# COx2/docker-nvidia-glx-desktop

Measured on AMD Instinct MI355X. Metric: encoded FPS + p50 end-to-end latency at 1080p60 H.264; concurrent sessions/node, higher is better.
Workload: dtype uint8 video (8-bit 4:2:0), H.264 Constrained Baseline

## Files before the change

### csrc/bindings/module.cpp

```cpp
#include <pybind11/numpy.h>
#include <pybind11/pybind11.h>
#include <pybind11/stl.h>

#include <cstring>

#include "../codec/h264_core.h"
#include "../codec/h264_encoder.h"
#include "../codec/vp8_encoder.h"
#include "../codec/hevc_encoder.h"
#include "../common/hip_check.h"
#include "../common/trace.h"
#include "../kernels/pixel.h"
#include "../runtime/session.h"

namespace py = pybind11;
using namespace mx;

void register_net(py::module& m);
void register_audio(py::module& m);
void register_rfb(py::module& m);

namespace {

template <class T>
T* as_ptr(uintptr_t p) {
    return reinterpret_cast<T*>(p);
}
hipStream_t as_stream(uintptr_t s) { return reinterpret_cast<hipStream_t>(s); }

py::bytes to_bytes(const std::vector<uint8_t>& v) {
    return py::bytes(reinterpret_cast<const char*>(v.data()), v.size());
}

struct PyBits {
    std::vector<uint32_t> words;
    h264::BitWriter w;
    PyBits() : words(4096) { w.init(words.data()); }
    py::tuple finish() {
        const uint32_t bits = w.bits;
        w.flush();
        std::vector<uint8_t> out;
        for (uint32_t i = 0; i < (bits + 7) / 8; ++i) out.push_back((uint8_t)(words[i / 4] >> (24 - 8 * (i % 4))));
        return py::make_tuple(to_bytes(out), bits);
    }
};

py::tuple cavlc_block_py(const std::vector<int>& coef, int nc) {
    PyBits b;
    int16_t c[16] = {0};
    const int n = (int)coef.size();
    if (n != 4 && n != 15 && n != 16) throw std::invalid_argument("block must have 4, 15 or 16 coefficients");
    for (int i = 0; i < n; ++i) c[i] = (int16_t)coef[i];
    h264::cavlc_block(b.w, c, n, nc);
    return b.finish();
}

py::array_t<int> fdct_py(py::array_t<int, py::array::c_style | py::array::forcecast> x) {
    if (x.size() != 16) throw std::invalid_argument("need 16 values");
    py::array_t<int> y(16);
    h264::fdct4x4(x.data(), y.mutable_data());
    return y;
}
py::array_t<int> idct_py(py::array_t<int, py::array::c_style | py::array::forcecast> x) {
    if (x.size() != 16) throw std::invalid_argument("need 16 values");
    py::array_t<int> y(16);
    h264::idct4x4(x.data(), y.mutable_data());
    return y;
}

py::array_t<uint8_t> copy_plane(const uint8_t* dev, int pitch, int w, int h) {
    py::array_t<uint8_t> out({h, w});
    HIP_CHECK(hipDeviceSynchronize());
    HIP_CHECK(hipMemcpy2D(out.mutable_data(), w, dev, pitch, w, h, hipMemcpyDeviceToHost));
    return out;
}

}

PYBIND11_MODULE(_native, m) {
    m.doc() = "mxdesk native runtime: HIP kernels (gfx950), H.264 encoder, session pipeline";

    m.def("device_count", []() {
        int n = 0;
        if (hipGetDeviceCount(&n) != hipSuccess) return 0;
        return n;
    });
    m.def("set_device", [](int d) { HIP_CHECK(hipSetDevice(d)); });
    m.def("device_name", [](int d) {
        hipDeviceProp_t p;
        HIP_CHECK(hipGetDeviceProperties(&p, d));
        return std::string(p.gcnArchName) + " / " + p.name;
    });
    m.def("synchronize", []() { HIP_CHECK(hipDeviceSynchronize()); });
    register_net(m);
    register_audio(m);
    register_rfb(m);
    m.def("now_us", &Session::now_us, "CLOCK_MONOTONIC microseconds (same clock as time.monotonic())");

    py::module h = m.def_submodule("h264", "H.264 building blocks (for tests)");
    h.def("hpel_planes", [](py::array_t<uint8_t, py::array::c_style> ref, int coded_w) {
        if (ref.ndim() != 2 || coded_w % 16 || ref.shape(0) % 16 || ref.shape(1) < coded_w)
            throw std::invalid_argument("ref must be (coded_h, pitch) with 16-aligned coded size");
        int hp = 0;
        auto planes = h264::hpel_planes_for_test(ref.data(), coded_w, (int)ref.shape(0), (int)ref.shape(1), &hp);
        const int rows = (int)ref.shape(0) + 2 * h264::kHpelPad;
        py::list out;
        for (auto& p : planes) {
            py::array_t<uint8_t> a({rows, hp});
            std::memcpy(a.mutable_data(), p.data(), p.size());
            out.append(a);
        }
        return out;
    });
    h.def("mc_luma_gpu", [](py::array_t<uint8_t, py::array::c_style> ref, int coded_w, int x4, int y4) {
        if (ref.ndim() != 2 || coded_w % 16 || ref.shape(0) % 16 || ref.shape(1) < coded_w)
            throw std::invalid_argument("ref must be (coded_h, pitch) with 16-aligned coded size");
        py::array_t<uint8_t> out({16, 16});
        h264::mc_luma_for_test(ref.data(), coded_w, (int)ref.shape(0), (int)ref.shape(1), x4, y4, out.mutable_data());
        return out;
    }, py::arg("ref"), py::arg("coded_w"), py::arg("x4"), py::arg("y4"),
          "16x16 luma prediction at quarter-sample position (x4, y4) by k_inter_encode's interpolation");
    h.def("cavlc_block", &cavlc_block_py, py::arg("coef"), py::arg("nc"));
    h.def("fdct4x4", &fdct_py);
    h.def("idct4x4", &idct_py);
    h.def("ue", [](uint32_t k) {
        PyBits b;
        h264::put_ue(b.w, k);
        return b.finish();
    });
    h.def("se", [](int v) {
        PyBits b;
        h264::put_se(b.w, v);
        return b.finish();
    });
    h.def("luma_qpel", [](py::array_t<uint8_t, py::array::c_style> plane, int x4, int y4) {
        if (plane.ndim() != 2) throw std::invalid_argument("2-D plane");
        const int H = (int)plane.shape(0), W = (int)plane.shape(1);
        return h264::luma_qpel(plane.data(), W, W, H, x4, y4);
    });
    h.def("level_for", &h264::pick_level);

    py::class_<h264::EncoderConfig>(m, "EncoderConfig")
        .def(py::init<>())
        .def_readwrite("width", &h264::EncoderConfig::width)
        .def_readwrite("height", &h264::EncoderConfig::height)
        .def_readwrite("fps", &h264::EncoderConfig::fps)
        .def_readwrite("bitrate_kbps", &h264::EncoderConfig::bitrate_kbps)
        .def_readwrite("qp", &h264::EncoderConfig::qp)
        .def_readwrite("qp_min", &h264::EncoderConfig::qp_min)
        .def_readwrite("qp_max", &h264::EncoderConfig::qp_max)
        .def_readwrite("keyint", &h264::EncoderConfig::keyint)
        .def_readwrite("search_range", &h264::EncoderConfig::search_range)
        .def_readwrite("me_coarse", &h264::EncoderConfig::me_coarse)
        .def_readwrite("intra4x4", &h264::EncoderConfig::intra4x4)
        .def_readwrite("subpel", &h264::EncoderConfig::subpel)
        .def_readwrite("chroma_qp_offset", &h264::EncoderConfig::chroma_qp_offset)
        .def_readwrite("pipeline_depth", &h264::EncoderConfig::pipeline_depth)
        .def_readwrite("aq", &h264::EncoderConfig::aq)
        .def_readwrite("intra_in_p", &h264::EncoderConfig::intra_in_p)
        .def_readwrite("vp8_bpred", &h264::EncoderConfig::vp8_bpred)
        .def_readwrite("vp8_intra", &h264::EncoderConfig::vp8_intra)
        .def_readwrite("mask_x0", &h264::EncoderConfig::mask_x0)
        .def_readwrite("mask_y0", &h264::EncoderConfig::mask_y0)
        .def_readwrite("mask_x1", &h264::EncoderConfig::mask_x1)
        .def_readwrite("mask_y1", &h264::EncoderConfig::mask_y1)
        .def_readwrite("deblock", &h264::EncoderConfig::deblock)
        .def_readwrite("partitions", &h264::EncoderConfig::partitions)
        .def_readwrite("tu_split", &h264::EncoderConfig::tu_split)
        .def_readwrite("hevc_slice_cost", &h264::EncoderConfig::hevc_slice_cost)
        .def_readwrite("hevc_wpp", &h264::EncoderConfig::hevc_wpp)
        .def_readwrite("hevc_wpp_rows", &h264::EncoderConfig::hevc_wpp_rows)
        .def_readwrite("sao", &h264::EncoderConfig::sao)
        .def_readwrite("hevc_chroma_keep", &h264::EncoderConfig::hevc_chroma_keep)
        .def_readwrite("hevc_intra_split", &h264::EncoderConfig::hevc_intra_split);

    py::class_<h264::FrameStats>(m, "FrameStats")
        .def_readonly("frame_index", &h264::FrameStats::frame_index)
        .def_readonly("idr", &h264::FrameStats::idr)
        .def_readonly("qp", &h264::FrameStats::qp)
        .def_readonly("bytes", &h264::FrameStats::bytes)
        .def_readonly("skipped_mbs", &h264::FrameStats::skipped_mbs)
        .def_readonly("encode_ms", &h264::FrameStats::encode_ms)
        .def_property_readonly("sse", [](const h264::FrameStats& s) { return py::make_tuple(s.sse[0], s.sse[1], s.sse[2]); })
        .def_readonly("sse_masked", &h264::FrameStats::sse_masked)
        .def_readonly("masked_pixels", &h264::FrameStats::masked_pixels)
        .def_readonly("deblocked", &h264::FrameStats::deblocked)
        .def_readonly("db_coherent", &h264::FrameStats::db_coherent)
        .def_readonly("db_changed", &h264::FrameStats::db_changed)
        .def_readonly("db_moving", &h264::FrameStats::db_moving);

    py::class_<h264::CpuH264Encoder>(m, "CpuH264Encoder")
        .def(py::init<const h264::EncoderConfig&>())
        .def(
            "encode",
            [](h264::CpuH264Encoder& e, py::array_t<uint8_t, py::array::c_style> y,
               py::array_t<uint8_t, py::array::c_style> uv, bool force_idr) {
                if (y.ndim() != 2 || uv.ndim() != 2 || y.shape(1) != uv.shape(1))
                    throw std::invalid_argument("y (H,P) and uv (H/2,P) planes with equal pitch");
                const int pitch = (int)y.shape(1);
                const int cw = e.coded_pitch();
                const auto& cfg = e.common().config();
                const int ch = e.common().mb_h() * 16;
                if (y.shape(0) < cfg.height || pitch < cfg.width || uv.shape(0) < cfg.height / 2)
                    throw std::invalid_argument("planes smaller than the encoder's configured picture");
                std::vector<uint8_t> py_, puv;
                const uint8_t* yy = y.data();
                const uint8_t* uu = uv.data();
                int p = pitch;
                if (y.shape(0) < ch || pitch < cw) {
                    h264::pad_nv12(yy, uu, cfg.width, cfg.height, pitch, cw, ch, py_, puv);
                    yy = py_.data();
                    uu = puv.data();
                    p = cw;
                }
                const auto& au = e.encode(yy, uu, p, force_idr);
                return to_bytes(au);
            },
            py::arg("y"), py::arg("uv"), py::arg("force_idr") = false)
        .def("recon",
             [](h264::CpuH264Encoder& e) {
                 const int cw = e.coded_pitch(), ch = e.common().mb_h() * 16;
                 py::array_t<uint8_t> y({ch, cw}), uv({ch / 2, cw});
                 std::memcpy(y.mutable_data(), e.recon_y().data(), (size_t)cw * ch);
                 std::memcpy(uv.mutable_data(), e.recon_uv().data(), (size_t)cw * ch / 2);
                 return py::make_tuple(y, uv);
             })
        .def("mb_bits",
             [](h264::CpuH264Encoder& e) {
                 const auto& v = e.mb_bits();
                 py::array_t<uint32_t> a((py::ssize_t)v.size());
                 std::memcpy(a.mutable_data(), v.data(), v.size() * 4);
                 return a.reshape({e.common().mb_h(), e.common().mb_w()});
             })
        .def("mb_info",
             [](h264::CpuH264Encoder& e) {
                 const auto& v = e.mb_info();
                 py::array_t<int32_t> a({(py::ssize_t)v.size(), (py::ssize_t)9});
                 int32_t* d = a.mutable_data();
                 for (size_t i = 0; i < v.size(); ++i) {
                     int nz = 0;
                     for (int k = 0; k < 16; ++k) nz += v[i].nz_luma[k];
                     const int32_t r[9] = {v[i].type, v[i].qp, v[i].cbp, v[i].skip, v[i].mvx, v[i].mvy, nz,
                                           (int32_t)v[i].cost, v[i].part};
                     std::memcpy(d + 9 * i, r, sizeof r);
                 }
                 return a.reshape({e.common().mb_h(), e.common().mb_w(), 9});
             })
        .def("request_idr", [](h264::CpuH264Encoder& e) { e.common().request_idr(); })
        .def("set_bitrate", [](h264::CpuH264Encoder& e, int k) { e.common().set_bitrate(k); })
        .def_property_readonly("stats", &h264::CpuH264Encoder::last_stats);

    py::class_<vp8::CpuVp8Encoder>(m, "CpuVp8Encoder")
        .def(py::init<const h264::EncoderConfig&>())
        .def(
            "encode",
            [](vp8::CpuVp8Encoder& e, py::array_t<uint8_t, py::array::c_style> y,
               py::array_t<uint8_t, py::array::c_style> uv, bool force_idr) {
                if (y.ndim() != 2 || uv.ndim() != 2 || y.shape(1) != uv.shape(1))
                    throw std::invalid_argument("y (H,P) and uv (H/2,P) planes with equal pitch");
                const int pitch = (int)y.shape(1);
                const int cw = e.coded_pitch();
                const auto& cfg = e.common().config();
                const int ch = e.common().mb_h() * 16;
                if (y.shape(0) < cfg.height || pitch < cfg.width || uv.shape(0) < cfg.height / 2)
                    throw std::invalid_argument("planes smaller than the encoder's configured picture");
                std::vector<uint8_t> py_, puv;
                const uint8_t* yy = y.data();
                const uint8_t* uu = uv.data();
                int p = pitch;
                if (y.shape(0) < ch || pitch < cw) {
                    h264::pad_nv12(yy, uu, cfg.width, cfg.height, pitch, cw, ch, py_, puv);
                    yy = py_.data();
                    uu = puv.data();
                    p = cw;
                }
                const auto& au = e.encode(yy, uu, p, force_idr);
                return to_bytes(au);
            },
            py::arg("y"), py::arg("uv"), py::arg("force_idr") = false)
        .def("recon",
             [](vp8::CpuVp8Encoder& e) {
                 const int cw = e.coded_pitch(), ch = e.common().mb_h() * 16;
                 py::array_t<uint8_t> y({ch, cw}), uv({ch / 2, cw});
                 std::memcpy(y.mutable_data(), e.recon_y().data(), (size_t)cw * ch);
                 std::memcpy(uv.mutable_data(), e.recon_uv().data(), (size_t)cw * ch / 2);
                 return py::make_tuple(y, uv);
             })
        .def("mb_info",
             [](vp8::CpuVp8Encoder& e) {
                 const auto& v = e.mb_info();
                 py::array_t<int32_t> a({(py::ssize_t)v.size(), (py::ssize_t)4});
                 int32_t* d = a.mutable_data();
                 for (size_t i = 0; i < v.size(); ++i) {
// ... 509 lines not shown
```

### csrc/codec/h264_encoder.cpp

```cpp
#include "h264_encoder.h"

#include <hip/hip_ext.h>

#include <algorithm>
#include <cmath>
#include <cstring>
#include <stdexcept>
#include <string>

#include "../common/hip_check.h"
#include "h264_mb.h"

namespace mx {
namespace h264 {

EncoderCommon::EncoderCommon(const EncoderConfig& c) : cfg_(c) {
    if (c.width <= 0 || c.height <= 0 || (c.width & 1) || (c.height & 1))
        throw std::invalid_argument("encoder size must be positive and even");
    mb_w_ = (c.width + 15) / 16;
    mb_h_ = (c.height + 15) / 16;
    cur_qp_ = std::clamp(c.qp, 0, 51);
}

double EncoderCommon::frame_budget_bits() const {
// ... 131 lines not shown
    words_to_bytes(words, w.bits + (w.bits % 8 ? 8 - w.bits % 8 : 0), rbsp);
    static const uint8_t sc[4] = {0, 0, 0, 1};
    out.insert(out.end(), sc, sc + 4);
    out.push_back(0x67);
    emulation_prevent(out, rbsp.data(), rbsp.size());
    w.init(words);
    write_pps(w, pic_init_qp(), cfg_.chroma_qp_offset);
    rbsp.clear();
    words_to_bytes(words, w.bits + (w.bits % 8 ? 8 - w.bits % 8 : 0), rbsp);
    out.insert(out.end(), sc, sc + 4);
    out.push_back(0x68);
    emulation_prevent(out, rbsp.data(), rbsp.size());
}

void EncoderCommon::write_slice_nal(std::vector<uint8_t>& out, const uint8_t* rbsp, size_t n, bool idr) const {
    static const uint8_t sc[4] = {0, 0, 0, 1};
    out.insert(out.end(), sc, sc + 4);
    out.push_back(idr ? 0x65 : 0x41);
    emulation_prevent(out, rbsp, n);
}

std::vector<std::vector<uint8_t>> hpel_planes_for_test(const uint8_t* ref, int coded_w, int coded_h, int pitch,
                                                       int* hp_pitch_out) {
    Geometry g{};
    g.width = coded_w;
    g.height = coded_h;
    g.mb_w = coded_w / 16;
    g.mb_h = coded_h / 16;
    g.coded_w = coded_w;
    g.coded_h = coded_h;
    g.pitch = pitch;
    const int hp_pitch = (coded_w + 2 * kHpelPad + 255) & ~255;
    const size_t hp_bytes = (size_t)hp_pitch * (coded_h + 2 * kHpelPad);
    uint8_t* dref = nullptr;
    uint8_t* planes[4];
    FrameState fs{};
    DeviceBuffers b{};
    HIP_CHECK(hipMalloc(&dref, (size_t)pitch * coded_h));
    HIP_CHECK(hipMemcpy(dref, ref, (size_t)pitch * coded_h, hipMemcpyHostToDevice));
    for (auto& p : planes) {
        HIP_CHECK(hipMalloc(&p, hp_bytes));
        HIP_CHECK(hipMemset(p, 0, hp_bytes));
    }
    fs.ref_y = dref;
    HIP_CHECK(hipMalloc(&b.fs, sizeof(FrameState)));
    HIP_CHECK(hipMemcpy(b.fs, &fs, sizeof(FrameState), hipMemcpyHostToDevice));
    launch_hpel(g, b, planes, hp_pitch, nullptr);
    HIP_CHECK(hipGetLastError());
    HIP_CHECK(hipDeviceSynchronize());
    std::vector<std::vector<uint8_t>> out(4, std::vector<uint8_t>(hp_bytes));
    for (int i = 0; i < 4; ++i) {
        HIP_CHECK(hipMemcpy(out[i].data(), planes[i], hp_bytes, hipMemcpyDeviceToHost));
        (void)hipFree(planes[i]);
    }
    (void)hipFree(dref);
    (void)hipFree(b.fs);
    *hp_pitch_out = hp_pitch;
    return out;
}

void mc_luma_for_test(const uint8_t* ref, int coded_w, int coded_h, int pitch, int x4, int y4, uint8_t* out) {
    Geometry g{};
    g.width = g.coded_w = coded_w;
    g.height = g.coded_h = coded_h;
    g.mb_w = coded_w / 16;
    g.mb_h = coded_h / 16;
    g.pitch = pitch;
    uint8_t *dref = nullptr, *dout = nullptr;
    HIP_CHECK(hipMalloc(&dref, (size_t)pitch * coded_h));
    HIP_CHECK(hipMalloc(&dout, 256));
    HIP_CHECK(hipMemcpy(dref, ref, (size_t)pitch * coded_h, hipMemcpyHostToDevice));
    launch_mc_luma_test(g, dref, x4, y4, dout, nullptr);
    const hipError_t e = hipGetLastError();
    if (e == hipSuccess) (void)hipMemcpy(out, dout, 256, hipMemcpyDeviceToHost);
    (void)hipFree(dref);
    (void)hipFree(dout);
    HIP_CHECK(e);
}

constexpr unsigned kDeviceEvent = hipEventDisableTiming | hipEventReleaseToDevice;

void GpuH264Encoder::alloc_slot(FrameSlot& sl) {
    const int nmb = geom_.mb_w * geom_.mb_h;
    DeviceBuffers& b = sl.buf;
    HIP_CHECK(hipMalloc(&b.fs, sizeof(FrameState)));
    HIP_CHECK(hipMalloc(&b.mb, sizeof(MbInfo) * nmb));
    HIP_CHECK(hipMemsetAsync(b.mb, 0, sizeof(MbInfo) * nmb, stream_));
    HIP_CHECK(hipMalloc(&b.coef, sizeof(int16_t) * kCoefStride * nmb));
    HIP_CHECK(hipMalloc(&b.slot, sizeof(uint32_t) * kSlotWords * (size_t)nmb));
    HIP_CHECK(hipMalloc(&b.slot_bits, sizeof(uint32_t) * nmb));
    HIP_CHECK(hipMalloc(&b.row_agg, sizeof(uint4) * (size_t)geom_.mb_h));
    HIP_CHECK(hipMalloc(&b.row_sse, sizeof(unsigned long long) * 4 * 512));
    HIP_CHECK(hipMalloc(&b.coded_info, sizeof(uint4) * nmb));
    HIP_CHECK(hipMalloc(&b.slice_info, sizeof(uint32_t) * kSliceInfo * kMaxSlices));
    HIP_CHECK(hipMemsetAsync(b.slice_info, 0, sizeof(uint32_t) * kSliceInfo * kMaxSlices, stream_));
    b.out_bytes = (size_t)nmb * 768;
    HIP_CHECK(hipMalloc(&b.quad_unit, sizeof(uint32_t) * (b.out_bytes / 16 + 1)));
    HIP_CHECK(hipMalloc(&b.out_hdr, sizeof(OutHeader)));
    HIP_CHECK(hipMalloc(&b.sse_part, 4 * sizeof(unsigned long long) * kSsePartStride));
    HIP_CHECK(hipMalloc(&b.wave_prog, sizeof(int) * 4));
    HIP_CHECK(hipMalloc(&b.mb_sse, sizeof(uint32_t) * 3 * (size_t)nmb));
    HIP_CHECK(hipMalloc(&b.intra_gain, sizeof(int32_t) * (size_t)nmb));
    HIP_CHECK(hipMalloc(&b.intra_cand, sizeof(int) * (size_t)nmb));
    HIP_CHECK(hipMalloc(&b.db_rec, sizeof(uint4) * (size_t)nmb));
    HIP_CHECK(hipMalloc(&b.db_rowq, sizeof(int) * (size_t)geom_.mb_h));
    HIP_CHECK(hipMalloc(&b.db_glb, sizeof(uint64_t) * 2 * 24 * (size_t)nmb));
    HIP_CHECK(hipMemsetAsync(b.db_glb, 0, sizeof(uint64_t) * 2 * 24 * (size_t)nmb, stream_));
    HIP_CHECK(hipMalloc(&b.pack_done, sizeof(uint32_t)));
    HIP_CHECK(hipMemsetAsync(b.pack_done, 0, sizeof(uint32_t), stream_));
    HIP_CHECK(hipMalloc(&b.db_cnt, sizeof(uint32_t) * 4));
    HIP_CHECK(hipMemsetAsync(b.db_cnt, 0, sizeof(uint32_t) * 4, stream_));
    HIP_CHECK(hipHostMalloc(&b.db_err, sizeof(int), hipHostMallocMapped));
    *b.db_err = 0;
    HIP_CHECK(hipHostMalloc(&sl.fs_host, sizeof(FrameState), hipHostMallocDefault));
    HIP_CHECK(hipHostMalloc(&sl.host_out, kOutPayloadOffset + b.out_bytes + 16, hipHostMallocMapped));
    std::memset(sl.host_out, 0, kOutPayloadOffset);
    HIP_CHECK(hipEventCreateWithFlags(&sl.start, hipEventDisableTiming));
    HIP_CHECK(hipEventCreateWithFlags(&sl.analysis_done, kDeviceEvent));
    HIP_CHECK(hipEventCreateWithFlags(&sl.deblock_done, kDeviceEvent));
    HIP_CHECK(hipEventCreateWithFlags(&sl.me_done, kDeviceEvent));
    HIP_CHECK(hipEventCreateWithFlags(&sl.done, hipEventDisableTiming));
}

void GpuH264Encoder::free_slot(FrameSlot& sl) {
    DeviceBuffers& b = sl.buf;
    for (void* p : {(void*)b.fs, (void*)b.mb, (void*)b.coef, (void*)b.slot, (void*)b.slot_bits, (void*)b.row_agg,
                    (void*)b.row_sse, (void*)b.coded_info, (void*)b.slice_info,
                    (void*)b.out_hdr, (void*)b.sse_part, (void*)b.wave_prog, (void*)b.mb_sse, (void*)b.intra_gain, (void*)b.intra_cand, (void*)b.quad_unit,
                    (void*)b.db_rec, (void*)b.db_rowq, (void*)b.db_glb, (void*)b.pack_done, (void*)b.db_cnt})
        if (p) (void)hipFree(p);
    if (b.db_err) (void)hipHostFree(b.db_err);
    if (sl.fs_host) (void)hipHostFree(sl.fs_host);
    if (sl.host_out) (void)hipHostFree(sl.host_out);
    for (hipEvent_t e : {sl.start, sl.analysis_done, sl.deblock_done, sl.done, sl.me_done})
        if (e) (void)hipEventDestroy(e);
}

GpuH264Encoder::GpuH264Encoder(const EncoderConfig& cfg, hipStream_t stream)
    : cfg_(cfg.with_aq_default(4)), common_(cfg), stream_(stream) {
    if (cfg.pipeline_depth < 1 || cfg.pipeline_depth > kMaxInFlight)
        throw std::invalid_argument("pipeline_depth must be 1 to 4");
    depth_ = cfg.pipeline_depth;
    db_lag_.reset(cfg_.h264_deblock_mode());
    geom_.width = cfg.width;
    geom_.height = cfg.height;
    geom_.mb_w = common_.mb_w();
    geom_.mb_h = common_.mb_h();
    geom_.coded_w = geom_.mb_w * 16;
    geom_.coded_h = geom_.mb_h * 16;
    geom_.pitch = (geom_.coded_w + 255) & ~255;
    if (geom_.mb_h > kMaxSlices) throw std::invalid_argument("picture too tall");
    if (geom_.mb_w > 512) throw std::invalid_argument("picture too wide (k_intra_wave stages <= 512 MBs per row)");
    const int nmb = geom_.mb_w * geom_.mb_h;
    if ((nmb + 3) / 4 + geom_.mb_h > kSsePartStride)
        throw std::invalid_argument("frame too large for the distortion partials");
    const size_t ysz = (size_t)geom_.pitch * geom_.coded_h, uvsz = ysz / 2;
    for (int i = 0; i < 2; ++i) {
        HIP_CHECK(hipMalloc(&rec_y_[i], ysz));
        HIP_CHECK(hipMalloc(&rec_uv_[i], uvsz));
        HIP_CHECK(hipMemsetAsync(rec_y_[i], 16, ysz, stream_));
        HIP_CHECK(hipMemsetAsync(rec_uv_[i], 128, uvsz, stream_));
        HIP_CHECK(hipMalloc(&src_keep_[i], ysz));
        HIP_CHECK(hipMemsetAsync(src_keep_[i], 16, ysz, stream_));
    }
    if (cfg.mask_x1 > cfg.mask_x0 && cfg.mask_y1 > cfg.mask_y0) {
        mask_mb_[0] = std::max(0, cfg.mask_x0) / 16;
        mask_mb_[1] = std::max(0, cfg.mask_y0) / 16;
        mask_mb_[2] = std::min(geom_.mb_w, (cfg.mask_x1 + 15) / 16);
        mask_mb_[3] = std::min(geom_.mb_h, (cfg.mask_y1 + 15) / 16);
    }
    masked_pixels_ = (int64_t)cfg.width * cfg.height;
    for (int my = mask_mb_[1]; my < mask_mb_[3]; ++my)
        for (int mx = mask_mb_[0]; mx < mask_mb_[2]; ++mx)
            masked_pixels_ -= (int64_t)std::max(0, std::min(16, cfg.width - 16 * mx)) *
                              std::max(0, std::min(16, cfg.height - 16 * my));
    if (cfg_.h264_deblock()) HIP_CHECK(hipMalloc(&rec_unf_, ysz));
    for (int i = 0; i < depth_; ++i) alloc_slot(slots_[i]);
    clock_khz_ = device_clock_khz();
    if (depth_ > 1) {
        HIP_CHECK(hipStreamCreateWithFlags(&stream_e_, hipStreamNonBlocking));
        if (cfg_.h264_deblock()) {
            HIP_CHECK(hipEventCreateWithFlags(&ev_hpu_, kDeviceEvent));
            HIP_CHECK(hipEventRecord(ev_hpu_, stream_));
        }
    }
    HIP_CHECK(hipStreamSynchronize(stream_));
    const char* et = std::getenv("MXDESK_ENTROPY_THREAD");
    if (stream_e_ && !(et && et[0] == '0')) {
        HIP_CHECK(hipGetDevice(&device_));
        launcher_ = std::thread([this]() { launcher_loop(); });
    }
}

void GpuH264Encoder::ensure_me_stream() {
    if (stream_m_) return;
    e2_retired_ = true;
    if (stream_e2_) {
        drain_launcher();
        HIP_CHECK(hipStreamSynchronize(stream_e2_));
        HIP_CHECK(hipStreamDestroy(stream_e2_));
        stream_e2_ = nullptr;
    }
    const char* rv = std::getenv("MXDESK_ME_CU_RESERVE");
    const int reserve = rv ? std::atoi(rv) : 0;
    int ncu = 0;
    HIP_CHECK(hipDeviceGetAttribute(&ncu, hipDeviceAttributeMultiprocessorCount, 0));
    if (reserve > 0 && reserve < ncu) {
        std::vector<uint32_t> mask((size_t)(ncu + 31) / 32, 0u);
        for (int c = 0; c < ncu - reserve; ++c) mask[(size_t)c / 32] |= 1u << (c % 32);
        HIP_CHECK(hipExtStreamCreateWithCUMask(&stream_m_, (uint32_t)mask.size(), mask.data()));
    } else {
        HIP_CHECK(hipStreamCreateWithFlags(&stream_m_, hipStreamNonBlocking));
    }
}

void GpuH264Encoder::launcher_loop() {
    (void)hipSetDevice(device_);
    for (;;) {
        EntropyJob j;
        {
            std::unique_lock<std::mutex> lk(lmu_);
            lcv_.wait(lk, [&] { return lstop_ || !ljobs_.empty(); });
            if (ljobs_.empty()) return;
            j = ljobs_.front();
            ljobs_.pop_front();
        }
        try {
            FrameSlot& sl = slots_[j.slot];
            HIP_CHECK(hipStreamWaitEvent(j.stream, sl.analysis_done, 0));
            launch_entropy(geom_, sl.buf, sl.host_out, j.stream, j.sse_ready);
            HIP_CHECK(hipGetLastError());
            HIP_CHECK(hipEventRecord(sl.done, j.stream));
        } catch (...) {
            std::lock_guard<std::mutex> lk(lmu_);
            lerr_ = std::current_exception();
        }
        {
            std::lock_guard<std::mutex> lk(lmu_);
            ++l_done_;
        }
        lcv_.notify_all();
    }
}

void GpuH264Encoder::drain_launcher() const {
    if (!launcher_.joinable()) return;
    std::unique_lock<std::mutex> lk(lmu_);
    lcv_.wait(lk, [&] { return l_done_ >= l_pushed_ || lerr_; });
    if (lerr_) std::rethrow_exception(lerr_);
}

void GpuH264Encoder::wait_launched(int slot) const {
    std::unique_lock<std::mutex> lk(lmu_);
    lcv_.wait(lk, [&] { return l_done_ >= slot_job_[slot] || lerr_; });
    if (lerr_) std::rethrow_exception(lerr_);
}

GpuH264Encoder::~GpuH264Encoder() {
    if (launcher_.joinable()) {
        {
            std::lock_guard<std::mutex> lk(lmu_);
            lstop_ = true;
        }
        lcv_.notify_all();
        launcher_.join();
    }
    (void)hipStreamSynchronize(stream_);
    if (stream_e_) {
        (void)hipStreamSynchronize(stream_e_);
        (void)hipStreamDestroy(stream_e_);
    }
    if (stream_e2_) {
        (void)hipStreamSynchronize(stream_e2_);
        (void)hipStreamDestroy(stream_e2_);
    }
    if (stream_m_) {
        (void)hipStreamSynchronize(stream_m_);
        (void)hipStreamDestroy(stream_m_);
    }
    if (ev_hpu_) (void)hipEventDestroy(ev_hpu_);
    if (rec_unf_) (void)hipFree(rec_unf_);
    for (int i = 0; i < 2; ++i) {
        (void)hipFree(rec_y_[i]);
        (void)hipFree(rec_uv_[i]);
        (void)hipFree(src_keep_[i]);
    }
    for (int i = 0; i < depth_; ++i) free_slot(slots_[i]);
}

void GpuH264Encoder::enqueue_analysis_kernels(bool idr, const uint8_t* src_y, const uint8_t* src_uv, bool publish) {
    FrameSlot& sl = slots_[prep_slot_];
    const FrameState* pub = publish ? sl.fs_host : nullptr;
    auto wait_input = [&]() {
        if (!in_ev_) return;
        HIP_CHECK(hipStreamWaitEvent(stream_, in_ev_, 0));
        in_ev_ = nullptr;
    };
    if (idr) {
        wait_input();
        launch_intra(geom_, sl.buf, src_y, src_uv, stream_, pub);
        if (cfg_.aq >= 3)
            launch_save_src(geom_, sl.buf, src_y, stream_);
    } else {
        if (depth_ > 1 && pub && sl.me_unf) ensure_me_stream();
        const bool side_me = stream_m_ && pub && sl.me_unf;
        if (side_me) {
            HIP_CHECK(hipStreamWaitEvent(stream_m_, ev_hpu_, 0));
            if (in_ev_) {
                HIP_CHECK(hipStreamWaitEvent(stream_m_, in_ev_, 0));
                in_ev_ = nullptr;
            }
            launch_me(geom_, sl.buf, src_y, stream_m_, pub, true);
            HIP_CHECK(hipEventRecord(sl.me_done, stream_m_));
            HIP_CHECK(hipStreamWaitEvent(stream_, sl.me_done, 0));
        } else {
            wait_input();
            launch_me(geom_, sl.buf, src_y, stream_, pub);
        }
        launch_inter(geom_, sl.buf, src_y, src_uv, stream_);
        if (cfg_.intra_in_p) launch_intra_in_p(geom_, sl.buf, src_y, src_uv, stream_);
    }
}

void GpuH264Encoder::link_entropy() {
    if (!stream_e_) return;
    drain_launcher();
    FrameSlot& sl = slots_[prep_slot_];
    HIP_CHECK(hipEventRecord(sl.analysis_done, stream_));
    HIP_CHECK(hipStreamWaitEvent(stream_e_, sl.analysis_done, 0));
}

void GpuH264Encoder::enqueue_entropy() {
    drain_launcher();
    FrameSlot& sl = slots_[prep_slot_];
    launch_entropy(geom_, sl.buf, sl.host_out, stream_e_ ? stream_e_ : stream_, nullptr);
}

void GpuH264Encoder::unfiltered_copy(FrameSlot& sl) {
    launch_copy_luma(geom_, sl.fs_host->rec_y, rec_unf_, stream_);
    if (ev_hpu_) HIP_CHECK(hipEventRecord(ev_hpu_, stream_));
}

void GpuH264Encoder::enqueue_kernels(bool idr, const uint8_t* src_y, const uint8_t* src_uv, bool publish) {
    FrameSlot& sl = slots_[prep_slot_];
    enqueue_analysis_kernels(idr, src_y, src_uv, publish);
    async_frame_ = launcher_.joinable() && publish && !sync_launch_;
    if (async_frame_) {
        HIP_CHECK(hipEventRecord(sl.analysis_done, stream_));
        hipEvent_t sse_ready = nullptr;
        if (sl.deblock) {
            unfiltered_copy(sl);
            launch_deblock(geom_, sl.buf, src_y, src_uv, stream_);
            HIP_CHECK(hipEventRecord(sl.deblock_done, stream_));
            sse_ready = sl.deblock_done;
        }
        if (depth_ >= 3 && !stream_e2_ && !e2_retired_ && !stream_m_)
            HIP_CHECK(hipStreamCreateWithFlags(&stream_e2_, hipStreamNonBlocking));
        hipStream_t es = (stream_e2_ && (seq_ & 1)) ? stream_e2_ : stream_e_;
        HIP_CHECK(hipGetLastError());
        {
            std::lock_guard<std::mutex> lk(lmu_);
            if (lerr_) std::rethrow_exception(lerr_);
            ljobs_.push_back(EntropyJob{prep_slot_, sse_ready, es});
            slot_job_[prep_slot_] = ++l_pushed_;
        }
        lcv_.notify_all();
        return;
    }
    link_entropy();
    hipStream_t es = stream_e_ ? stream_e_ : stream_;
    hipEvent_t sse_ready = nullptr;
    if (sl.deblock) {
        unfiltered_copy(sl);
        launch_deblock(geom_, sl.buf, src_y, src_uv, stream_);
        if (stream_e_) {
            HIP_CHECK(hipEventRecord(sl.deblock_done, stream_));
            sse_ready = sl.deblock_done;
        }
    }
    launch_entropy(geom_, sl.buf, sl.host_out, es, sse_ready);
    HIP_CHECK(hipGetLastError());
}

void GpuH264Encoder::fill_state(FrameSlot& sl, bool idr, int qp, int ref, int cur) {
    FrameState& f = *sl.fs_host;
    f.ref_y = rec_y_[ref];
    f.ref_uv = rec_uv_[ref];
    f.rec_y = rec_y_[cur];
    f.rec_uv = rec_uv_[cur];
    f.idr = idr ? 1 : 0;
    f.frame_num = common_.cur_frame_num();
    f.idr_pic_id = common_.cur_idr_pic_id();
    f.qp = qp;
    f.slice_rows = idr ? idr_slice_rows(geom_.mb_h) : geom_.mb_h;
    f.num_slices = (geom_.mb_h + f.slice_rows - 1) / f.slice_rows;
    f.search_range = me_range(cfg_.search_range);
    f.me_coarse = cfg_.me_coarse;
    f.intra4x4 = cfg_.intra4x4;
    f.subpel = cfg_.subpel;
    f.deblock_off = sl.deblock ? 0 : 1;
    if (++db_epoch_ == 0) db_epoch_ = 1;
    f.db_epoch = (int32_t)db_epoch_;
    f.pic_init_qp = common_.pic_init_qp();
    f.chroma_qp_offset = cfg_.chroma_qp_offset;
    f.log2_max_frame_num = common_.log2_max_frame_num();
    f.aq = cfg_.aq;
    f.intra_in_p = cfg_.intra_in_p;
    f.partitions = cfg_.partitions ? 1 : 0;
    f.mask_mx0 = mask_mb_[0];
    f.mask_my0 = mask_mb_[1];
    f.mask_mx1 = mask_mb_[2];
    f.mask_my1 = mask_mb_[3];
    f.me_ref = sl.me_unf ? rec_unf_ : nullptr;
    f.sse_part = sl.buf.sse_part;
    f.prev_src = src_keep_[ref];
    f.save_src = src_keep_[cur];
}

int GpuH264Encoder::probe_bytes(const uint8_t* src_y, const uint8_t* src_uv, int qp) {
    if (!inflight_.empty()) throw std::logic_error("GpuH264Encoder: probe with frames in flight");
    prep_slot_ = 0;
    FrameSlot& sl = slots_[0];
    sl.deblock = cfg_.deblock == 1;
    sl.me_unf = false;
    fill_state(sl, true, qp, cur_ ^ 1, cur_);
    sl.fs_host->frame_num = 0;
    sl.fs_host->idr_pic_id = 0;
    sync_launch_ = true;
    enqueue_kernels(true, src_y, src_uv, true);
    sync_launch_ = false;
    HIP_CHECK(hipStreamSynchronize(stream_));
    if (stream_e_) HIP_CHECK(hipStreamSynchronize(stream_e_));
    const OutHeader hdr = *reinterpret_cast<const OutHeader*>(sl.host_out);
    return hdr.overflow ? (int)sl.buf.out_bytes : (int)(hdr.total_bytes + hdr.num_slices * 6 + 32);
}

bool GpuH264Encoder::prepare(bool force_idr) {
    if ((int)inflight_.size() >= depth_)
        throw std::logic_error("GpuH264Encoder: collect() a frame first (pipeline full)");
    const int s = (depth_ == 1) ? 0 : next_slot_;
    next_slot_ = (next_slot_ + 1) % depth_;
    prep_slot_ = s;
    ++seq_;
    FrameSlot& sl = slots_[s];
    common_.begin_frame(force_idr || !have_ref_);
    have_ref_ = true;
    const bool idr = common_.cur_idr();
    sl.idr = idr;
    sl.qp = common_.cur_qp();
    const int ref = cur_;
    cur_ ^= 1;
    sl.fidx = seq_;
    sl.me_unf = !idr && last_deblock_;
    sl.deblock = db_lag_.decide((long long)seq_, idr);
    last_deblock_ = sl.deblock;
    fill_state(sl, idr, sl.qp, ref, cur_);
    return idr;
}

void GpuH264Encoder::enqueue_body(bool idr, const uint8_t* src_y, const uint8_t* src_uv) {
    drain_launcher();
    FrameSlot& sl = slots_[prep_slot_];
    HIP_CHECK(hipMemcpyAsync(sl.buf.fs, sl.fs_host, sizeof(FrameState), hipMemcpyHostToDevice, stream_));
    enqueue_kernels(idr, src_y, src_uv, false);
}

void GpuH264Encoder::enqueue_analysis(bool idr, const uint8_t* src_y, const uint8_t* src_uv) {
    drain_launcher();
    FrameSlot& sl = slots_[prep_slot_];
    HIP_CHECK(hipMemcpyAsync(sl.buf.fs, sl.fs_host, sizeof(FrameState), hipMemcpyHostToDevice, stream_));
    enqueue_analysis_kernels(idr, src_y, src_uv, false);
}
// ... 75 lines not shown
```

### csrc/codec/h264_gpu.h

```cpp
#pragma once
#include <vector>
#include <hip/hip_runtime.h>
#include <stdint.h>

#define MXHD_GPU __host__ __device__ __forceinline__

namespace mx {
namespace h264 {

constexpr int kSlotWords = 640;
constexpr int kCoefStride = 416;
constexpr int kCoefLuma = 0;
constexpr int kCoefLumaDc = 256;
constexpr int kCoefChromaDc = 272;
constexpr int kCoefChromaAc = 280;

enum MbType : uint8_t { kMbP16x16 = 0, kMbI16x16 = 1, kMbI4x4 = 2 };

struct MbInfo {
    int16_t mvx, mvy;
    uint8_t type;
    uint8_t cbp;
    uint8_t i16_mode;
    uint8_t chroma_mode;
    uint8_t nz_luma[16];
    uint8_t nz_cb[4];
    uint8_t nz_cr[4];
    uint8_t skip;
    uint8_t qp;
    uint8_t cbp_c;
    uint8_t itype;
    uint8_t i4[8];
    uint32_t cost;
    int16_t pmv[4];
    uint8_t part;
    uint8_t pad_[7];
};
static_assert(sizeof(MbInfo) == 64, "MbInfo layout");
enum MbPart : uint8_t { kPart16x16 = 0, kPart16x8 = 1, kPart8x16 = 2 };

MXHD_GPU bool is_intra(const MbInfo& m) { return m.type != kMbP16x16; }
template <class FS>
MXHD_GPU bool mb_unmasked(const FS* fs, int mbx, int mby) {
    return !(mbx >= fs->mask_mx0 && mbx < fs->mask_mx1 && mby >= fs->mask_my0 && mby < fs->mask_my1);
}
MXHD_GPU bool carries_dqp(const MbInfo& m) { return m.type == kMbI16x16 || m.cbp != 0; }

struct FrameState {
    const uint8_t* ref_y;
    const uint8_t* ref_uv;
    uint8_t* rec_y;
    uint8_t* rec_uv;
    int32_t idr;
    int32_t frame_num;
    int32_t idr_pic_id;
    int32_t qp;
    int32_t slice_rows;
    int32_t num_slices;
    int32_t search_range;
    int32_t subpel;
    int32_t me_coarse;
    int32_t intra4x4;
    int32_t deblock_off;
    int32_t db_epoch;
    int32_t pic_init_qp;
    int32_t chroma_qp_offset;
    int32_t log2_max_frame_num;
    int32_t aq;
    int32_t intra_in_p;
    int32_t partitions;
    int32_t mask_mx0, mask_my0, mask_mx1, mask_my1;
    const uint8_t* prev_src;
    uint8_t* save_src;
    const uint8_t* me_ref;
    unsigned long long* sse_part;
};
constexpr int kHpelPad = 48;
constexpr int kSsePartStride = 65536;

struct OutHeader {
    uint32_t total_bytes;
    uint32_t num_slices;
    uint32_t overflow;
    uint32_t deblocked;
    uint64_t sse[3];
    uint64_t sse_masked;
    uint64_t t_start;
    uint64_t t_end;
    uint32_t db_coherent, db_changed, db_moving;
    uint32_t pad;
};
static_assert(sizeof(OutHeader) % 16 == 0, "payload must stay 16-byte aligned");
constexpr int kMaxSlices = 1024;
constexpr int kSliceInfo = 8;
constexpr size_t kOutPayloadOffset = sizeof(OutHeader) + 2 * kMaxSlices * sizeof(uint32_t);

struct Geometry {
    int width, height;
    int mb_w, mb_h;
    int pitch;
    int coded_w, coded_h;
};

struct DeviceBuffers {
    FrameState* fs;
    MbInfo* mb;
    int16_t* coef;
    uint32_t* slot;
    uint32_t* slot_bits;
    uint4* row_agg;
    unsigned long long* row_sse;
    uint4* coded_info;
    uint32_t* quad_unit;
    uint32_t* slice_info;
    size_t out_bytes;
    OutHeader* out_hdr;
    unsigned long long* sse_part;
    int* wave_prog;
    int32_t* intra_gain;
    int* intra_cand;
    uint32_t* mb_sse;
    uint4* db_rec;
    int* db_rowq;
    uint64_t* db_glb;
    int* db_err;
    uint32_t* db_cnt;
    uint32_t* pack_done;
};

void launch_me(const Geometry& g, const DeviceBuffers& b, const uint8_t* src_y, hipStream_t stream,
               const FrameState* publish = nullptr, bool side = false);
void launch_copy_luma(const Geometry& g, const uint8_t* luma, uint8_t* dst, hipStream_t stream);
void launch_mc_luma_test(const Geometry& g, const uint8_t* ref, int x4, int y4, uint8_t* out, hipStream_t stream);
void launch_inter(const Geometry& g, const DeviceBuffers& b, const uint8_t* src_y, const uint8_t* src_uv,
                  hipStream_t stream);
void launch_intra(const Geometry& g, const DeviceBuffers& b, const uint8_t* src_y, const uint8_t* src_uv,
                  hipStream_t stream, const FrameState* publish = nullptr);
void launch_hpel(const Geometry& g, const DeviceBuffers& b, uint8_t* const planes[4], int hp_pitch,
                 hipStream_t stream, const FrameState* publish = nullptr);
std::vector<unsigned long long> deblock_row_stamps(int mb_h);
void launch_deblock(const Geometry& g, const DeviceBuffers& b, const uint8_t* src_y, const uint8_t* src_uv,
                    hipStream_t stream);
void launch_save_src(const Geometry& g, const DeviceBuffers& b, const uint8_t* src_y, hipStream_t stream);
void launch_entropy(const Geometry& g, const DeviceBuffers& b, uint8_t* host_out, hipStream_t stream,
                    hipEvent_t wait_for_sse = nullptr);
void launch_intra_in_p(const Geometry& g, const DeviceBuffers& b, const uint8_t* src_y, const uint8_t* src_uv,
                       hipStream_t stream);

}
}
```

### csrc/codec/h264_kernels.hip

```cpp
#include <hip/hip_runtime.h>

#include <cstddef>

#include "../common/hip_check.h"
#include "h264_core.h"
#include "h264_deblock.h"
#include "h264_gpu.h"
#include "h264_mb.h"

namespace mx {
namespace h264 {

namespace {

__device__ __forceinline__ uint32_t bswap32(uint32_t v) { return __builtin_bswap32(v); }

template <bool kSwap>
struct OrWriter {
    uint32_t* dst;
    uint32_t pos;
    uint64_t acc;
    int nacc;
    uint32_t bits;

// ... 25 lines not shown
            nacc -= 32;
        }
    }
    __device__ __forceinline__ void flush() {
        if (nacc > 0) {
            emit((uint32_t)(acc << (32 - nacc)), nacc);
            nacc = 0;
            acc = 0;
        }
    }
};

__device__ __forceinline__ uint32_t rows_sum(uint32_t v) {
    const auto r16 = __builtin_amdgcn_permlane16_swap(v, v, false, false);
    v = r16[0] + r16[1];
    const auto r32 = __builtin_amdgcn_permlane32_swap(v, v, false, false);
    return r32[0] + r32[1];
}
__device__ __forceinline__ int wave_sum(int v) {
    v += __builtin_amdgcn_mov_dpp(v, 0xB1, 0xF, 0xF, false);
    v += __builtin_amdgcn_mov_dpp(v, 0x4E, 0xF, 0xF, false);
    v += __builtin_amdgcn_mov_dpp(v, 0x124, 0xF, 0xF, false);
    v += __builtin_amdgcn_mov_dpp(v, 0x128, 0xF, 0xF, false);
    return (int)rows_sum((uint32_t)v);
}

constexpr int kHpTW = 128, kHpTH = 16;
constexpr int kHpSW = kHpTW + 8;
__device__ __forceinline__ int byte_of(uint32_t w, int k) { return (int)((w >> (8 * k)) & 0xff); }
__device__ __forceinline__ uint32_t pack4(int a, int b, int c, int d) {
    const uint32_t lo = __builtin_amdgcn_perm((uint32_t)b, (uint32_t)a, 0x0c0c0400u);
    const uint32_t hi = __builtin_amdgcn_perm((uint32_t)d, (uint32_t)c, 0x0c0c0400u);
    return __builtin_amdgcn_perm(hi, lo, 0x05040100u);
}
struct StateArg {
    FrameState v;
    FrameState* dst;
    int publish;
    uint64_t* t_start;
};
__device__ __forceinline__ void publish_state(const StateArg& a) {
    static_assert(sizeof(FrameState) % 4 == 0, "FrameState is copied as dwords");
    if (a.t_start && blockIdx.x == 0 && blockIdx.y == 0 && threadIdx.x == 0) *a.t_start = wall_clock64();
    if (a.publish && blockIdx.x == 0 && blockIdx.y == 0 && threadIdx.x < sizeof(FrameState) / 4)
        reinterpret_cast<uint32_t*>(a.dst)[threadIdx.x] = reinterpret_cast<const uint32_t*>(&a.v)[threadIdx.x];
}
__device__ __forceinline__ const FrameState& state_of(const StateArg& a) { return a.publish ? a.v : *a.dst; }

__global__ __launch_bounds__(256) void k_hpel(Geometry g, StateArg sa, uint8_t* __restrict__ pf,
                                              uint8_t* __restrict__ ph, uint8_t* __restrict__ pv,
                                              uint8_t* __restrict__ pj, int hp_pitch) {
    __shared__ uint32_t smp[kHpTH + 5][kHpSW / 4];
    __shared__ int4 b1[kHpTH + 5][kHpTW / 4];
    publish_state(sa);
    const uint8_t* __restrict__ ref = state_of(sa).ref_y;
    const int px0 = blockIdx.x * kHpTW, py0 = blockIdx.y * kHpTH;
    const int W = g.coded_w + 2 * kHpelPad, H = g.coded_h + 2 * kHpelPad;
    const int tid = threadIdx.x;
    const int xs = px0 - 4 - kHpelPad, ys = py0 - 2 - kHpelPad;
    const bool interior = xs >= 0 && xs + kHpSW <= g.coded_w && ys >= 0 && ys + kHpTH + 5 <= g.coded_h &&
                          (g.pitch & 3) == 0 && (reinterpret_cast<uintptr_t>(ref) & 3) == 0;
    for (int i = tid; i < (kHpTH + 5) * (kHpSW / 4); i += 256) {
        const int r = i / (kHpSW / 4), k4 = i - r * (kHpSW / 4);
        uint32_t w;
        if (interior) {
            w = *reinterpret_cast<const uint32_t*>(ref + (size_t)(ys + r) * g.pitch + xs + 4 * k4);
        } else {
            w = 0;
            for (int k = 0; k < 4; ++k)
                w |= (uint32_t)ref_px(ref, g.pitch, g.coded_w, g.coded_h, xs + 4 * k4 + k, ys + r) << (8 * k);
        }
        smp[r][k4] = w;
    }
    __syncthreads();
    for (int i = tid; i < (kHpTH + 5) * (kHpTW / 4); i += 256) {
        const int r = i / (kHpTW / 4), q = i - r * (kHpTW / 4);
        const uint32_t w0 = smp[r][q], w1 = smp[r][q + 1], w2 = smp[r][q + 2];
        int s[12];
#pragma unroll
        for (int k = 0; k < 4; ++k) {
            s[k] = byte_of(w0, k);
            s[4 + k] = byte_of(w1, k);
            s[8 + k] = byte_of(w2, k);
        }
        int t[4];
#pragma unroll
        for (int j = 0; j < 4; ++j) t[j] = tap6(s[j + 2], s[j + 3], s[j + 4], s[j + 5], s[j + 6], s[j + 7]);
        b1[r][q] = make_int4(t[0], t[1], t[2], t[3]);
    }
    __syncthreads();
    const int q = tid & (kHpTW / 4 - 1), r0 = (tid / (kHpTW / 4)) * 2;
    const int x = px0 + 4 * q;
    if (x >= W) return;
    int sv[7][4], bv[7][4];
#pragma unroll
    for (int k = 0; k < 7; ++k) {
        const uint32_t w = smp[r0 + k][q + 1];
        const int4 bb = b1[r0 + k][q];
#pragma unroll
        for (int j = 0; j < 4; ++j) sv[k][j] = byte_of(w, j);
        bv[k][0] = bb.x;
        bv[k][1] = bb.y;
        bv[k][2] = bb.z;
        bv[k][3] = bb.w;
    }
#pragma unroll
    for (int rr = 0; rr < 2; ++rr) {
        const int y = py0 + r0 + rr;
        if (y >= H) break;
        int Hs[4], Vs[4], Js[4];
#pragma unroll
        for (int j = 0; j < 4; ++j) {
            Hs[j] = clip255((bv[rr + 2][j] + 16) >> 5);
            const int v1 = tap6(sv[rr][j], sv[rr + 1][j], sv[rr + 2][j], sv[rr + 3][j], sv[rr + 4][j], sv[rr + 5][j]);
            Vs[j] = clip255((v1 + 16) >> 5);
            const int j1 = tap6(bv[rr][j], bv[rr + 1][j], bv[rr + 2][j], bv[rr + 3][j], bv[rr + 4][j], bv[rr + 5][j]);
            Js[j] = clip255((j1 + 512) >> 10);
        }
        const size_t o = (size_t)y * hp_pitch + x;
        *reinterpret_cast<uint32_t*>(pf + o) = smp[r0 + rr + 2][q + 1];
        *reinterpret_cast<uint32_t*>(ph + o) = pack4(Hs[0], Hs[1], Hs[2], Hs[3]);
        *reinterpret_cast<uint32_t*>(pv + o) = pack4(Vs[0], Vs[1], Vs[2], Vs[3]);
        *reinterpret_cast<uint32_t*>(pj + o) = pack4(Js[0], Js[1], Js[2], Js[3]);
    }
}

constexpr int kSpW = 20;
__device__ __forceinline__ int qpel_lds(const uint8_t (*sp)[18][kSpW], int x4, int y4) {
    const int xi = x4 >> 2, yi = y4 >> 2, xf = x4 & 3, yf = y4 & 3;
    const int G = sp[0][yi][xi];
    if ((xf | yf) == 0) return G;
    if (yf == 0) {
        const int b = sp[1][yi][xi];
        if (xf == 2) return b;
        return ((xf == 1 ? G : (int)sp[0][yi][xi + 1]) + b + 1) >> 1;
    }
    if (xf == 0) {
        const int hh = sp[2][yi][xi];
        if (yf == 2) return hh;
        return ((yf == 1 ? G : (int)sp[0][yi + 1][xi]) + hh + 1) >> 1;
    }
    if (xf == 2 && yf == 2) return sp[3][yi][xi];
    if (xf == 2) return ((yf == 1 ? (int)sp[1][yi][xi] : (int)sp[1][yi + 1][xi]) + sp[3][yi][xi] + 1) >> 1;
    if (yf == 2) return ((xf == 1 ? (int)sp[2][yi][xi] : (int)sp[2][yi][xi + 1]) + sp[3][yi][xi] + 1) >> 1;
    const int bb = (yf == 1) ? sp[1][yi][xi] : sp[1][yi + 1][xi];
    const int hh = (xf == 1) ? sp[2][yi][xi] : sp[2][yi][xi + 1];
    return (bb + hh + 1) >> 1;
}

constexpr int kMaxRange = 32;
constexpr int kWinPadX = 4, kWinPadY = 3;
constexpr int kWinStride = 16 + 2 * kMaxRange + 8;
constexpr int kWinRows = 16 + 2 * kMaxRange + 7;

constexpr int kMeThreads = 256, kMeWaves = kMeThreads / 64;
constexpr int kFpRows = 18 + 5;
__device__ __forceinline__ void build_footprints(const uint8_t* win, int org0, int org1, int n,
                                                 uint8_t (*sp)[4][18][kSpW], int16_t (*b1)[kFpRows][kSpW], int tid) {
    for (int i = tid; i < n * kFpRows * 18; i += kMeThreads) {
        const int pi = i / (kFpRows * 18), rem = i - pi * (kFpRows * 18), r = rem / 18, c = rem - r * 18;
        const uint8_t* p = win + (pi ? org1 : org0) + (r - 2) * kWinStride + c;
        b1[pi][r][c] = (int16_t)tap6(p[-2], p[-1], p[0], p[1], p[2], p[3]);
    }
    __syncthreads();
    for (int i = tid; i < n * 324; i += kMeThreads) {
        const int pi = i / 324, rem = i - pi * 324, r = rem / 18, c = rem - r * 18;
        const uint8_t* p = win + (pi ? org1 : org0) + r * kWinStride + c;
        const int16_t(*b)[kSpW] = b1[pi];
        const int v1 = tap6(p[-2 * kWinStride], p[-kWinStride], p[0], p[kWinStride], p[2 * kWinStride], p[3 * kWinStride]);
        const int j1 = tap6(b[r][c], b[r + 1][c], b[r + 2][c], b[r + 3][c], b[r + 4][c], b[r + 5][c]);
        sp[pi][0][r][c] = p[0];
        sp[pi][1][r][c] = (uint8_t)clip255((b[r + 2][c] + 16) >> 5);
        sp[pi][2][r][c] = (uint8_t)clip255((v1 + 16) >> 5);
        sp[pi][3][r][c] = (uint8_t)clip255((j1 + 512) >> 10);
    }
}

struct MeState {
    const uint8_t* ref;
    int qp, search_range, subpel, me_coarse, partitions;
};
__device__ __forceinline__ MeState me_state(const FrameState& f) {
    return MeState{f.me_ref ? f.me_ref : f.ref_y, f.qp, f.search_range, f.subpel, f.me_coarse, f.partitions};
}
__device__ __forceinline__ void me_full_body(const Geometry& g, const MeState& st, const uint8_t* __restrict__ src_y,
                                             MbInfo* __restrict__ mbs) {
    __shared__ uint32_t win_lds[kWinRows * kWinStride / 4];
    __shared__ uint8_t sp2[2][4][18][kSpW];
    __shared__ int16_t fp_b1[2][kFpRows][kSpW];
    __shared__ uint32_t srcw[64];
    __shared__ unsigned long long red[kMeWaves];
    __shared__ uint32_t cand_cost[8];
    __shared__ uint32_t s_sad0[4];

    const int mbi = blockIdx.x;
    const int mbx = mbi % g.mb_w, mby = mbi / g.mb_w;
    const int x0 = mbx * 16, y0 = mby * 16;
    const int tid = threadIdx.x, lane = tid & 63;
    const int R = me_range(st.search_range);
    const int W = 16 + 2 * R;
    const uint8_t* __restrict__ ref = st.ref;
    const int lambda = lambda_sad(st.qp);

    constexpr int kWs4 = kWinStride / 4;
    {
        if (tid < 64) {
            const int r = tid >> 2, c4 = (tid & 3) * 4;
            const uint32_t sw = *reinterpret_cast<const uint32_t*>(src_y + (y0 + r) * g.pitch + x0 + c4);
            const uint32_t rw = *reinterpret_cast<const uint32_t*>(ref + (y0 + r) * g.pitch + x0 + c4);
            const int d = wave_sum((int)__builtin_amdgcn_sad_u8(sw, rw, 0u));
            if (tid == 0) s_sad0[0] = (uint32_t)d;
        }
        __syncthreads();
        const uint32_t sad0 = s_sad0[0];
        if (sad0 <= static_sad(st.qp)) {
            if (tid == 0) {
                MbInfo& m = mbs[mbi];
                m.mvx = 0;
                m.mvy = 0;
                m.part = kPart16x16;
                m.pmv[0] = m.pmv[1] = m.pmv[2] = m.pmv[3] = 0;
            }
            return;
        }
    }
    const bool t256 = tid < 256;
    const int wrows = W + 2 * kWinPadY + 1, wx0 = x0 - R - kWinPadX, wy0 = y0 - R - kWinPadY;
    const bool dwords = (g.pitch & 3) == 0 && (reinterpret_cast<uintptr_t>(ref) & 3) == 0;
    for (int i = tid; i < wrows * kWs4; i += kMeThreads) {
        const int wy = i / kWs4, wx4 = (i - wy * kWs4) * 4;
        uint32_t w = 0u;
        if (wx4 < W + 2 * kWinPadX) {
            const int py = min(max(wy0 + wy, 0), g.coded_h - 1), px = wx0 + wx4;
            const uint8_t* row = ref + (size_t)py * g.pitch;
            if (px < 0)
                w = row[0] * 0x01010101u;
            else if (px >= g.coded_w)
                w = row[g.coded_w - 1] * 0x01010101u;
            else if (dwords)
                w = *reinterpret_cast<const uint32_t*>(row + px);
            else
                w = row[px] | ((uint32_t)row[px + 1] << 8) | ((uint32_t)row[px + 2] << 16) | ((uint32_t)row[px + 3] << 24);
        }
        win_lds[i] = w;
    }
    const uint32_t* win32 = win_lds + kWinPadY * kWs4 + kWinPadX / 4;
    auto fp_org = [&](int vx, int vy) {
        return ((vy >> 2) + R + kWinPadY - 1) * kWinStride + (vx >> 2) + R + kWinPadX - 1;
    };
    if (tid < 64) {
        const int r = tid >> 2, c = (tid & 3) * 4;
        srcw[tid] = *reinterpret_cast<const uint32_t*>(src_y + (y0 + r) * g.pitch + x0 + c);
    }
    __syncthreads();

    const int side = 2 * R + 1, gw = (side + 3) >> 2, ngroups = side * gw;
    unsigned long long best = ~0ull;
    const bool coarse = st.me_coarse != 0;
    const bool parts = st.partitions != 0;
    const int ntask = (coarse && !parts) ? (R + 1) * gw : 0;
    auto mkey = [&](uint32_t sad, int dxr, int dyr) {
        const int dx = dxr - R, dy = dyr - R;
        const uint32_t cost = me_cost(sad, lambda, 4 * dx, 4 * dy);
        const uint32_t dist = (uint32_t)(abs(dx) + abs(dy));
        return ((unsigned long long)cost << 32) | (dist << 16) | (uint32_t)(dyr * side + dxr);
    };
    unsigned long long pb[4] = {~0ull, ~0ull, ~0ull, ~0ull};
    auto kmin = [](unsigned long long a, unsigned long long c) { return c < a ? c : a; };
    auto visit_quads = [&](const uint32_t* qd, int dxr, int dyr) {
        best = kmin(best, mkey(qd[0] + qd[1] + qd[2] + qd[3], dxr, dyr));
        pb[0] = kmin(pb[0], mkey(qd[0] + qd[1], dxr, dyr));
        pb[1] = kmin(pb[1], mkey(qd[2] + qd[3], dxr, dyr));
        pb[2] = kmin(pb[2], mkey(qd[0] + qd[2], dxr, dyr));
        pb[3] = kmin(pb[3], mkey(qd[1] + qd[3], dxr, dyr));
    };
    if (parts) {
        const int nsh = coarse ? 2 : 4, ntp = coarse ? (R + 1) * gw : ngroups;
        for (int q = tid; q < ntp; q += kMeThreads) {
            const int dyr = coarse ? 2 * (q / gw) : q / gw, g = q % gw;
            uint32_t acc[4][4];
#pragma unroll
            for (int i = 0; i < 4; ++i) acc[i][0] = acc[i][1] = acc[i][2] = acc[i][3] = 0;
#pragma unroll 2
            for (int r = 0; r < 16; ++r) {
                const int a = (dyr + r) * kWs4 + g, hq = r < 8 ? 0 : 2;
                const uint32_t w0 = win32[a], w1 = win32[a + 1], w2 = win32[a + 2], w3 = win32[a + 3], w4 = win32[a + 4];
                const uint32_t s0 = srcw[r * 4 + 0], s1 = srcw[r * 4 + 1], s2 = srcw[r * 4 + 2], s3 = srcw[r * 4 + 3];
#pragma unroll
                for (int si = 0; si < 4; ++si) {
                    if (si >= nsh) break;
                    const int sh = coarse ? 2 * si : si;
                    const uint32_t a0 = sh ? __builtin_amdgcn_alignbyte(w1, w0, sh) : w0;
                    const uint32_t a1 = sh ? __builtin_amdgcn_alignbyte(w2, w1, sh) : w1;
                    const uint32_t a2 = sh ? __builtin_amdgcn_alignbyte(w3, w2, sh) : w2;
                    const uint32_t a3 = sh ? __builtin_amdgcn_alignbyte(w4, w3, sh) : w3;
                    uint32_t lft = hq ? acc[si][2] : acc[si][0], rgt = hq ? acc[si][3] : acc[si][1];
                    lft = __builtin_amdgcn_sad_u8(a1, s1, __builtin_amdgcn_sad_u8(a0, s0, lft));
                    rgt = __builtin_amdgcn_sad_u8(a3, s3, __builtin_amdgcn_sad_u8(a2, s2, rgt));
                    if (hq) {
                        acc[si][2] = lft;
                        acc[si][3] = rgt;
                    } else {
                        acc[si][0] = lft;
                        acc[si][1] = rgt;
                    }
                }
            }
#pragma unroll
            for (int si = 0; si < 4; ++si) {
                if (si >= nsh) break;
                const int dxr = 4 * g + (coarse ? 2 * si : si);
                if (dxr >= side) break;
                visit_quads(acc[si], dxr, dyr);
            }
        }
    }
    for (int q = tid; q < ntask; q += kMeThreads) {
        const int dyr = 2 * (q / gw), g = q % gw;
        uint32_t s0a = 0, s2a = 0;
#pragma unroll 4
        for (int r = 0; r < 16; ++r) {
            const int a = (dyr + r) * kWs4 + g;
            const uint32_t w0 = win32[a], w1 = win32[a + 1], w2 = win32[a + 2], w3 = win32[a + 3], w4 = win32[a + 4];
            const uint32_t s0 = srcw[r * 4 + 0], s1 = srcw[r * 4 + 1], s2 = srcw[r * 4 + 2], s3 = srcw[r * 4 + 3];
            s0a = __builtin_amdgcn_sad_u8(w0, s0, s0a);
            s0a = __builtin_amdgcn_sad_u8(w1, s1, s0a);
            s0a = __builtin_amdgcn_sad_u8(w2, s2, s0a);
            s0a = __builtin_amdgcn_sad_u8(w3, s3, s0a);
            s2a = __builtin_amdgcn_sad_u8(__builtin_amdgcn_alignbyte(w1, w0, 2), s0, s2a);
            s2a = __builtin_amdgcn_sad_u8(__builtin_amdgcn_alignbyte(w2, w1, 2), s1, s2a);
            s2a = __builtin_amdgcn_sad_u8(__builtin_amdgcn_alignbyte(w3, w2, 2), s2, s2a);
            s2a = __builtin_amdgcn_sad_u8(__builtin_amdgcn_alignbyte(w4, w3, 2), s3, s2a);
        }
#pragma unroll
        for (int h2 = 0; h2 < 2; ++h2) {
            const int dxr = 4 * g + 2 * h2;
            if (dxr >= side) break;
            const int dx = dxr - R, dy = dyr - R, c = dyr * side + dxr;
            const uint32_t cost = me_cost(h2 ? s2a : s0a, lambda, 4 * dx, 4 * dy);
            const uint32_t dist = (uint32_t)(abs(dx) + abs(dy));
            const unsigned long long key = ((unsigned long long)cost << 32) | (dist << 16) | (uint32_t)c;
            best = key < best ? key : best;
        }
    }
    for (int q = tid; q < ((coarse || parts) ? 0 : ngroups); q += kMeThreads) {
        const int dyr = q / gw, g = q - dyr * gw;
        uint32_t sad[4] = {0, 0, 0, 0};
#pragma unroll 2
        for (int r = 0; r < 16; ++r) {
            const int a = (dyr + r) * kWs4 + g;
            const uint32_t w0 = win32[a], w1 = win32[a + 1], w2 = win32[a + 2], w3 = win32[a + 3], w4 = win32[a + 4];
            const uint32_t s0 = srcw[r * 4 + 0], s1 = srcw[r * 4 + 1], s2 = srcw[r * 4 + 2], s3 = srcw[r * 4 + 3];
            sad[0] = __builtin_amdgcn_sad_u8(w0, s0, sad[0]);
            sad[0] = __builtin_amdgcn_sad_u8(w1, s1, sad[0]);
            sad[0] = __builtin_amdgcn_sad_u8(w2, s2, sad[0]);
            sad[0] = __builtin_amdgcn_sad_u8(w3, s3, sad[0]);
#pragma unroll
            for (int sh = 1; sh < 4; ++sh) {
                uint32_t t = sad[sh];
                t = __builtin_amdgcn_sad_u8(__builtin_amdgcn_alignbyte(w1, w0, sh), s0, t);
                t = __builtin_amdgcn_sad_u8(__builtin_amdgcn_alignbyte(w2, w1, sh), s1, t);
                t = __builtin_amdgcn_sad_u8(__builtin_amdgcn_alignbyte(w3, w2, sh), s2, t);
                t = __builtin_amdgcn_sad_u8(__builtin_amdgcn_alignbyte(w4, w3, sh), s3, t);
                sad[sh] = t;
            }
        }
#pragma unroll
        for (int sh = 0; sh < 4; ++sh) {
            const int dxr = 4 * g + sh;
            if (dxr >= side) break;
            const int dx = dxr - R, dy = dyr - R, c = dyr * side + dxr;
            const uint32_t cost = me_cost(sad[sh], lambda, 4 * dx, 4 * dy);
            const uint32_t dist = (uint32_t)(abs(dx) + abs(dy));
            const unsigned long long key = ((unsigned long long)cost << 32) | (dist << 16) | (uint32_t)c;
            best = key < best ? key : best;
        }
    }
    for (int o = 32; o > 0; o >>= 1) {
        unsigned long long other = __shfl_xor(best, o, 64);
        best = other < best ? other : best;
    }
    if (lane == 0) red[tid >> 6] = best;
    __shared__ unsigned long long pred4[4][kMeWaves];
    if (parts) {
#pragma unroll
        for (int sh = 0; sh < 4; ++sh) {
            unsigned long long v = pb[sh];
            for (int o = 32; o > 0; o >>= 1) {
                const unsigned long long other = __shfl_xor(v, o, 64);
                v = other < v ? other : v;
            }
            if (lane == 0) pred4[sh][tid >> 6] = v;
        }
    }
    __syncthreads();
    unsigned long long b = red[0];
    for (int i = 1; i < kMeWaves; ++i) b = red[i] < b ? red[i] : b;
    unsigned long long pbest[4] = {~0ull, ~0ull, ~0ull, ~0ull};
    if (parts)
        for (int sh = 0; sh < 4; ++sh)
            for (int i = 0; i < kMeWaves; ++i) pbest[sh] = pred4[sh][i] < pbest[sh] ? pred4[sh][i] : pbest[sh];
    if (parts && coarse) {
        __shared__ unsigned long long pnkey[4][8];
        const int ev = (tid & 255) >> 3, sub = tid & 7, sh = ev >> 3, k = ev & 7;
        const int cb0 = (int)(pbest[sh] & 0xffff), bxr = cb0 % side, byr = cb0 / side;
        int ddx, ddy;
        subpel_offset(k, &ddx, &ddy);
        const int nxr = bxr + ddx, nyr = byr + ddy;
        const bool inside = t256 && nxr >= 0 && nxr < side && nyr >= 0 && nyr < side;
        int d = 0;
        if (inside) {
            const uint8_t* wb = reinterpret_cast<const uint8_t*>(win32);
            const uint8_t* sb = reinterpret_cast<const uint8_t*>(srcw);
            for (int part_row = 0; part_row < 2; ++part_row) {
                const int rr = sh < 2 ? (sh == 0 ? sub : 8 + sub) : 2 * sub + part_row;
                const int c0 = sh < 2 ? 8 * part_row : (sh == 2 ? 0 : 8);
#pragma unroll
                for (int j = 0; j < 8; ++j)
                    d += abs((int)sb[rr * 16 + c0 + j] - (int)wb[(nyr + rr) * kWinStride + nxr + c0 + j]);
            }
        }
        for (int o = 4; o > 0; o >>= 1) d += __shfl_xor(d, o, 64);
        if (t256 && sub == 0) pnkey[sh][k] = inside ? mkey((uint32_t)d, nxr, nyr) : ~0ull;
        __syncthreads();
        for (int s2 = 0; s2 < 4; ++s2)
            for (int i = 0; i < 8; ++i) pbest[s2] = pnkey[s2][i] < pbest[s2] ? pnkey[s2][i] : pbest[s2];
    }
    if (coarse) {
        __shared__ unsigned long long nkey[8];
        const int cb0 = (int)(b & 0xffff), bxr = cb0 % side, byr = cb0 / side;
        const int k = (tid & 255) >> 5, sub = tid & 31, py = sub >> 1, px0 = (sub & 1) * 8;
        int ddx, ddy;
        subpel_offset(k, &ddx, &ddy);
        const int nxr = bxr + ddx, nyr = byr + ddy;
        const bool inside = t256 && nxr >= 0 && nxr < side && nyr >= 0 && nyr < side;
        int d = 0;
        if (inside) {
            const uint8_t* wrow = reinterpret_cast<const uint8_t*>(win32) + (nyr + py) * kWinStride + nxr + px0;
            const uint32_t s0 = srcw[py * 4 + (px0 >> 2)], s1 = srcw[py * 4 + (px0 >> 2) + 1];
#pragma unroll
            for (int j = 0; j < 8; ++j) d += abs((int)(((j < 4 ? s0 : s1) >> (8 * (j & 3))) & 0xff) - (int)wrow[j]);
        }
        for (int o = 16; o > 0; o >>= 1) d += __shfl_xor(d, o, 64);
        if (t256 && sub == 0) {
            const int dx = nxr - R, dy = nyr - R;
            const uint32_t cost = me_cost((uint32_t)d, lambda, 4 * dx, 4 * dy);
            const uint32_t dist = (uint32_t)(abs(dx) + abs(dy));
            nkey[k] = inside ? (((unsigned long long)cost << 32) | (dist << 16) | (uint32_t)(nyr * side + nxr)) : ~0ull;
        }
        __syncthreads();
        for (int i = 0; i < 8; ++i) b = nkey[i] < b ? nkey[i] : b;
    }
    const int cbest = (int)(b & 0xffff);
    int mvx = 4 * ((cbest % side) - R), mvy = 4 * ((cbest / side) - R);

    if (parts) {
        const uint32_t c16 = (uint32_t)(b >> 32);
        const uint32_t chz = (uint32_t)(pbest[0] >> 32) + (uint32_t)(pbest[1] >> 32) + 2u * (uint32_t)lambda;
        const uint32_t cvt = (uint32_t)(pbest[2] >> 32) + (uint32_t)(pbest[3] >> 32) + 2u * (uint32_t)lambda;
        const int part = (c16 <= chz && c16 <= cvt) ? kPart16x16 : (chz <= cvt ? kPart16x8 : kPart8x16);
        if (part != kPart16x16) {
            const int s0 = part == kPart16x8 ? 0 : 2;
            int pvx[2], pvy[2];
            uint32_t pcost[2];
            for (int i = 0; i < 2; ++i) {
                const int cb = (int)(pbest[s0 + i] & 0xffff);
                pvx[i] = 4 * ((cb % side) - R);
                pvy[i] = 4 * ((cb / side) - R);
                pcost[i] = (uint32_t)(pbest[s0 + i] >> 32);
            }
            if (st.subpel) {
                uint8_t(*psp)[4][18][kSpW] = sp2;
                __shared__ uint32_t pcand[2][8];
                build_footprints(reinterpret_cast<const uint8_t*>(win_lds), fp_org(pvx[0], pvy[0]),
                                 fp_org(pvx[1], pvy[1]), 2, sp2, fp_b1, tid);
                __syncthreads();
                const int pi = (tid & 255) >> 7, k = (tid >> 4) & 7, sub = tid & 15;
                const int rx = part == kPart8x16 ? 8 * pi : 0, ry = part == kPart16x8 ? 8 * pi : 0;
                const int prow = part == kPart16x8 ? (sub >> 1) : sub, pcol = part == kPart16x8 ? (sub & 1) * 8 : 0;
                const int yy = ry + prow, xx = rx + pcol;
                const uint32_t s0w = srcw[yy * 4 + (xx >> 2)], s1w = srcw[yy * 4 + (xx >> 2) + 1];
                const int ivx = pvx[pi], ivy = pvy[pi];
                const int base_x4 = xx * 4 + 4 - ivx, base_y4 = yy * 4 + 4 - ivy;
                for (int step = 2; step >= 1; step >>= 1) {
                    int ddx, ddy;
                    subpel_offset(k, &ddx, &ddy);
                    const int cx = pvx[pi] + ddx * step, cy = pvy[pi] + ddy * step;
                    int d = 0;
#pragma unroll
                    for (int j = 0; j < 8; ++j) {
                        const int sv = (int)(((j < 4 ? s0w : s1w) >> (8 * (j & 3))) & 0xff);
                        d += abs(sv - qpel_lds(psp[pi], base_x4 + 4 * j + cx, base_y4 + cy));
                    }
                    for (int o = 8; o > 0; o >>= 1) d += __shfl_xor(d, o, 64);
                    __syncthreads();
                    if (t256 && sub == 0) pcand[pi][k] = me_cost((uint32_t)d, lambda, cx, cy);
                    __syncthreads();
                    for (int q = 0; q < 2; ++q) {
                        int bdx = 0, bdy = 0;
                        uint32_t bcost = pcost[q];
                        for (int kk = 0; kk < 8; ++kk) {
                            const uint32_t cc = pcand[q][kk];
                            if (cc < bcost) {
                                int ex, ey;
                                subpel_offset(kk, &ex, &ey);
                                bcost = cc;
                                bdx = ex * step;
                                bdy = ey * step;
                            }
                        }
                        pvx[q] += bdx;
                        pvy[q] += bdy;
                        pcost[q] = bcost;
                    }
                }
            }
            if (tid == 0) {
                MbInfo& m = mbs[mbi];
                m.mvx = (int16_t)mvx;
                m.mvy = (int16_t)mvy;
                m.part = (uint8_t)part;
                m.pmv[0] = (int16_t)pvx[0];
                m.pmv[1] = (int16_t)pvy[0];
                m.pmv[2] = (int16_t)pvx[1];
                m.pmv[3] = (int16_t)pvy[1];
            }
            return;
        }
    }

    if (st.subpel) {
        uint8_t(*sp)[18][kSpW] = sp2[0];
        build_footprints(reinterpret_cast<const uint8_t*>(win_lds), fp_org(mvx, mvy), 0, 1, sp2, fp_b1, tid);
        __syncthreads();
        uint32_t cur_cost = (uint32_t)(b >> 32);
        const int k = (tid & 255) >> 5, sub = tid & 31;
        const int py = sub >> 1, px0 = (sub & 1) * 8;
        const uint32_t s0 = srcw[py * 4 + (px0 >> 2)], s1 = srcw[py * 4 + (px0 >> 2) + 1];
        const int base_x4 = px0 * 4 + 4 - mvx, base_y4 = py * 4 + 4 - mvy;
        for (int step = 2; step >= 1; step >>= 1) {
            int ddx, ddy;
            subpel_offset(k, &ddx, &ddy);
            const int cx = mvx + ddx * step, cy = mvy + ddy * step;
            int d = 0;
#pragma unroll
            for (int j = 0; j < 8; ++j) {
                const int sv = (int)(((j < 4 ? s0 : s1) >> (8 * (j & 3))) & 0xff);
                d += abs(sv - qpel_lds(sp, base_x4 + 4 * j + cx, base_y4 + cy));
            }
            for (int o = 16; o > 0; o >>= 1) d += __shfl_xor(d, o, 64);
            __syncthreads();
            if (t256 && sub == 0) cand_cost[k] = me_cost((uint32_t)d, lambda, cx, cy);
            __syncthreads();
            int bdx = 0, bdy = 0;
            uint32_t bcost = cur_cost;
            for (int kk = 0; kk < 8; ++kk) {
                const uint32_t cc = cand_cost[kk];
                if (cc < bcost) {
                    int ex, ey;
                    subpel_offset(kk, &ex, &ey);
                    bcost = cc;
                    bdx = ex * step;
                    bdy = ey * step;
                }
            }
            mvx += bdx;
            mvy += bdy;
            cur_cost = bcost;
        }
    }
    if (tid == 0) {
        MbInfo& m = mbs[mbi];
        m.mvx = (int16_t)mvx;
        m.mvy = (int16_t)mvy;
        m.part = kPart16x16;
        m.pmv[0] = m.pmv[1] = m.pmv[2] = m.pmv[3] = 0;
    }
}

__global__ __launch_bounds__(kMeThreads) void k_me_full(Geometry g, StateArg sa, const uint8_t* __restrict__ src_y,
                                                        MbInfo* __restrict__ mbs) {
    publish_state(sa);
    me_full_body(g, sa.publish ? me_state(sa.v) : me_state(*sa.dst), src_y, mbs);
}
__global__ __launch_bounds__(kMeThreads) void k_me_full_val(Geometry g, StateArg sa, const uint8_t* __restrict__ src_y,
                                                            MbInfo* __restrict__ mbs) {
    publish_state(sa);
    me_full_body(g, me_state(sa.v), src_y, mbs);
}

template <int K>
__device__ __forceinline__ int qbc(int v) {
    return __builtin_amdgcn_mov_dpp(v, K * 0x55, 0xF, 0xF, false);
}
__device__ __forceinline__ int quad_sum(int v) { return qbc<0>(v) + qbc<1>(v) + qbc<2>(v) + qbc<3>(v); }

__device__ __forceinline__ void fdct_row(const int* x, int r, int* y) {
    const int s03 = x[0] + x[3], d03 = x[0] - x[3], s12 = x[1] + x[2], d12 = x[1] - x[2];
    const int t[4] = {s03 + s12, 2 * d03 + d12, s03 - s12, d03 - 2 * d12};
#pragma unroll
    for (int c = 0; c < 4; ++c) {
        const int a0 = qbc<0>(t[c]), a1 = qbc<1>(t[c]), a2 = qbc<2>(t[c]), a3 = qbc<3>(t[c]);
        const int u03 = a0 + a3, e03 = a0 - a3, u12 = a1 + a2, e12 = a1 - a2;
        y[c] = r == 0 ? u03 + u12 : r == 1 ? 2 * e03 + e12 : r == 2 ? u03 - u12 : e03 - 2 * e12;
    }
}
__device__ __forceinline__ void idct_row(const int* d, int r, int* out) {
    const int e0 = d[0] + d[2], e1 = d[0] - d[2], e2 = (d[1] >> 1) - d[3], e3 = d[1] + (d[3] >> 1);
    const int f[4] = {e0 + e3, e1 + e2, e1 - e2, e0 - e3};
#pragma unroll
    for (int c = 0; c < 4; ++c) {
        const int b0 = qbc<0>(f[c]), b1 = qbc<1>(f[c]), b2 = qbc<2>(f[c]), b3 = qbc<3>(f[c]);
        const int g0 = b0 + b2, g1 = b0 - b2, g2 = (b1 >> 1) - b3, g3 = b1 + (b3 >> 1);
        const int v = r == 0 ? g0 + g3 : r == 1 ? g1 + g2 : r == 2 ? g1 - g2 : g0 - g3;
        out[c] = (v + 32) >> 6;
    }
}
__device__ __forceinline__ int had_row_abs(const int* x, int r) {
    const int t[4] = {x[0] + x[1] + x[2] + x[3], x[0] + x[1] - x[2] - x[3], x[0] - x[1] - x[2] + x[3],
                      x[0] - x[1] + x[2] - x[3]};
    int s = 0;
#pragma unroll
    for (int c = 0; c < 4; ++c) {
        const int a = qbc<0>(t[c]), b = qbc<1>(t[c]), cc = qbc<2>(t[c]), d = qbc<3>(t[c]);
        const int v = r == 0 ? a + b + cc + d : r == 1 ? a + b - cc - d : r == 2 ? a - b - cc + d : a - b + cc - d;
        s += v < 0 ? -v : v;
    }
    return s;
}
__device__ __forceinline__ int quant_row(const int* y, int r, int qp, bool intra, int start, int* z) {
    const int qm = qp % 6, qbits = 15 + qp / 6;
    const int f = intra ? ((1 << qbits) / 3) : ((1 << qbits) / 6);
    int nz = 0;
#pragma unroll
    for (int c = 0; c < 4; ++c) {
        const int i = r * 4 + c;
        if (i < start) {
            z[c] = 0;
            continue;
        }
        const int a = y[c] < 0 ? -y[c] : y[c];
        int q = (int)(((int64_t)a * kQuantMF[qm][kPosClass[i]] + f) >> qbits);
        q = q > kMaxLevel ? kMaxLevel : q;
        z[c] = y[c] < 0 ? -q : q;
        nz += (q != 0);
    }
    return nz;
}
__device__ __forceinline__ void dequant_row(const int* z, int r, int qp, int* d) {
    const int qm = qp % 6, qs = qp / 6;
#pragma unroll
    for (int c = 0; c < 4; ++c) d[c] = z[c] * kDequantV[qm][kPosClass[r * 4 + c]] * (1 << qs);
}

__device__ __forceinline__ void wave_sync_lds() {
    __builtin_amdgcn_fence(__ATOMIC_RELEASE, "wavefront");
    __builtin_amdgcn_wave_barrier();
    __builtin_amdgcn_fence(__ATOMIC_ACQUIRE, "wavefront");
}

constexpr int kMcStride = 24, kMcRows = 16 + 5, kMcWords = kMcRows * kMcStride / 4;
__device__ __forceinline__ void mc_luma_wave(uint32_t* __restrict__ w, const uint8_t* __restrict__ ref, int pitch,
                                             int cw, int ch, int n, int xa, int ya, int xb, int yb, int lane, int lpi,
                                             uint32_t* out) {
    const bool aligned = (pitch & 3) == 0 && (reinterpret_cast<uintptr_t>(ref) & 3) == 0;
    for (int i = lane; i < n * kMcWords; i += 64) {
        const int pi = i >= kMcWords ? 1 : 0, j = i - pi * kMcWords;
        const int wr = j / (kMcStride / 4), q = j - wr * (kMcStride / 4);
        const int xs = ((pi ? xb : xa) >> 2) - 2, ys = ((pi ? yb : ya) >> 2) - 2;
        uint32_t v;
        if (aligned && xs >= 0 && (xs & ~3) + kMcStride + 4 <= cw) {
            const int py = min(max(ys + wr, 0), ch - 1), px = xs + 4 * q;
            const uint32_t* qa = reinterpret_cast<const uint32_t*>(ref + (size_t)py * pitch + (px & ~3));
            const uint32_t sh = (uint32_t)(px & 3);
            v = sh ? __builtin_amdgcn_alignbyte(qa[1], qa[0], sh) : qa[0];
        } else {
            v = 0;
            for (int k = 0; k < 4; ++k) v |= (uint32_t)ref_px(ref, pitch, cw, ch, xs + 4 * q + k, ys + wr) << (8 * k);
        }
        w[i] = v;
    }
    wave_sync_lds();
    {
        const int xf = (lpi ? xb : xa) & 3, yf = (lpi ? yb : ya) & 3;
        w += lpi * kMcWords;
        const int r = lane >> 2, q0 = lane & 3;
        uint32_t wd[6][3];
#pragma unroll
        for (int rr = 0; rr < 6; ++rr) {
            const uint32_t* row = w + (r + rr) * (kMcStride / 4) + q0;
            wd[rr][0] = row[0];
            wd[rr][1] = row[1];
            wd[rr][2] = row[2];
        }
        auto s = [&](int rr, int c) { return byte_of(wd[rr][c >> 2], c & 3); };
        auto b1 = [&](int rr) { return tap6(s(rr, 0), s(rr, 1), s(rr, 2), s(rr, 3), s(rr, 4), s(rr, 5)); };
        auto v1 = [&](int c) { return tap6(s(0, c), s(1, c), s(2, c), s(3, c), s(4, c), s(5, c)); };
        auto b_at = [&](int rr) { return clip255((b1(rr) + 16) >> 5); };
        auto h_at = [&](int c) { return clip255((v1(c) + 16) >> 5); };
        auto j_val = [&]() { return clip255((tap6(b1(0), b1(1), b1(2), b1(3), b1(4), b1(5)) + 512) >> 10); };
        uint32_t packed = 0;
#pragma unroll 1
        for (int k = 0; k < 4; ++k) {
            const int G = s(2, 2);
            int p;
            if ((xf | yf) == 0)
                p = G;
            else if (yf == 0)
                p = xf == 2 ? b_at(2) : ((xf == 1 ? G : s(2, 3)) + b_at(2) + 1) >> 1;
            else if (xf == 0)
                p = yf == 2 ? h_at(2) : ((yf == 1 ? G : s(3, 2)) + h_at(2) + 1) >> 1;
            else if (xf == 2 && yf == 2)
                p = j_val();
            else if (xf == 2)
                p = ((yf == 1 ? b_at(2) : b_at(3)) + j_val() + 1) >> 1;
            else if (yf == 2)
                p = ((xf == 1 ? h_at(2) : h_at(3)) + j_val() + 1) >> 1;
            else
                p = ((yf == 1 ? b_at(2) : b_at(3)) + (xf == 1 ? h_at(2) : h_at(3)) + 1) >> 1;
            packed |= (uint32_t)p << (8 * k);
#pragma unroll
            for (int rr = 0; rr < 6; ++rr) {
                wd[rr][0] = __builtin_amdgcn_alignbyte(wd[rr][1], wd[rr][0], 1);
                wd[rr][1] = __builtin_amdgcn_alignbyte(wd[rr][2], wd[rr][1], 1);
                wd[rr][2] >>= 8;
            }
        }
        *out = packed;
    }
}

__global__ __launch_bounds__(64) void k_mc_luma_test(Geometry g, const uint8_t* __restrict__ ref, int x4, int y4,
                                                     uint8_t* __restrict__ out) {
    __shared__ uint32_t w[kMcWords];
    const int lane = threadIdx.x;
    uint32_t p = 0;
    mc_luma_wave(w, ref, g.pitch, g.coded_w, g.coded_h, 1, x4, y4, x4, y4, lane, 0, &p);
    reinterpret_cast<uint32_t*>(out)[lane] = p;
}

__global__ __launch_bounds__(256) void k_inter_encode(Geometry g, const FrameState* __restrict__ fs,
                                                       const uint8_t* __restrict__ src_y,
                                                       const uint8_t* __restrict__ src_uv, MbInfo* __restrict__ mbs,
                                                       int16_t* __restrict__ coef, uint32_t* __restrict__ mb_sse,
                                                       int* __restrict__ wave_prog) {
    __shared__ uint8_t pred[4][384];
    __shared__ int16_t res[4][384];
    __shared__ uint32_t mcw[4][2 * kMcWords];
    __shared__ int cdc[4][8];
    __shared__ int cdc_nz[4][2];

    const int wave = threadIdx.x >> 6, lane = threadIdx.x & 63;
    const int nmb = g.mb_w * g.mb_h;
    const int bid = blockIdx.x;
    const int mbi = bid * 4 + wave;
    if (bid == 0 && threadIdx.x == 0) wave_prog[1] = 0;
    const bool valid = mbi < nmb;
    const int mbx = valid ? mbi % g.mb_w : 0, mby = valid ? mbi / g.mb_w : 0;
    const int x0 = mbx * 16, y0 = mby * 16;
    const uint8_t* __restrict__ ref_y = fs->ref_y;
    const bool ref_dwords = (g.pitch & 3) == 0 && (reinterpret_cast<uintptr_t>(ref_y) & 3) == 0;
    const uint8_t* ref_uv = fs->ref_uv;
    const int cw = g.coded_w / 2, ch = g.coded_h / 2;
    int mvx = 0, mvy = 0;
    int lsad = 0;
    int tsad = 0;
    MbInfo mi;
    mi.part = kPart16x16;
    if (valid) {
        mi = mbs[mbi];
        const int r = lane >> 2, c0 = (lane & 3) * 4;
        const Mv lv = px_mv(mi, c0, r);
        mvx = lv.x;
        mvy = lv.y;
        const uint32_t sw = *reinterpret_cast<const uint32_t*>(src_y + (y0 + r) * g.pitch + x0 + c0);
        if (fs->aq >= 3) {
            const int ix = mvx >> 2, iy = mvy >> 2;
            const int px = x0 + c0 + ix, py = y0 + r + iy;
            if (px >= 0 && px + 4 <= g.coded_w && py >= 0 && py < g.coded_h &&
                ((px & 3) == 0 || (px & ~3) + 8 <= g.pitch)) {
                const uint32_t* qa = reinterpret_cast<const uint32_t*>(fs->prev_src + (size_t)py * g.pitch + (px & ~3));
                const uint32_t sh = (uint32_t)(px & 3);
                const uint32_t pw = sh ? __builtin_amdgcn_alignbyte(qa[1], qa[0], sh) : qa[0];
                tsad = (int)__builtin_amdgcn_sad_u8(sw, pw, 0u);
            } else {
                for (int k = 0; k < 4; ++k)
                    tsad += abs((int)((sw >> (8 * k)) & 0xff) -
                                ref_px(fs->prev_src, g.pitch, g.coded_w, g.coded_h, x0 + c0 + k + ix, y0 + r + iy));
            }
            *reinterpret_cast<uint32_t*>(fs->save_src + (y0 + r) * g.pitch + x0 + c0) = sw;
        }
        const int part = __builtin_amdgcn_readfirstlane((int)mi.part);
        const Mv va = blk_mv(mi, 0, 0), vb = blk_mv(mi, part == kPart8x16 ? 2 : 0, part == kPart16x8 ? 2 : 0);
        const int vax = __builtin_amdgcn_readfirstlane(va.x), vay = __builtin_amdgcn_readfirstlane(va.y);
        const int vbx = __builtin_amdgcn_readfirstlane(vb.x), vby = __builtin_amdgcn_readfirstlane(vb.y);
        uint32_t pw = 0;
        if ((vax | vay | vbx | vby) & 3) {
            const int lpi = part == kPart16x8 ? (r >> 3) : (part == kPart8x16 ? (c0 >> 3) : 0);
            mc_luma_wave(mcw[wave], ref_y, g.pitch, g.coded_w, g.coded_h, part == kPart16x16 ? 1 : 2, x0 * 4 + vax,
                         y0 * 4 + vay, x0 * 4 + vbx, y0 * 4 + vby, lane, lpi, &pw);
        } else {
            const int px = x0 + c0 + (mvx >> 2), py = min(max(y0 + r + (mvy >> 2), 0), g.coded_h - 1);
            if (px >= 0 && px + 4 <= g.coded_w && ((px & 3) == 0 || (px & ~3) + 8 <= g.pitch) && ref_dwords) {
                const uint32_t* qa = reinterpret_cast<const uint32_t*>(ref_y + (size_t)py * g.pitch + (px & ~3));
                const uint32_t sh = (uint32_t)(px & 3);
                pw = sh ? __builtin_amdgcn_alignbyte(qa[1], qa[0], sh) : qa[0];
            } else {
                for (int k = 0; k < 4; ++k)
                    pw |= (uint32_t)ref_px(ref_y, g.pitch, g.coded_w, g.coded_h, px + k, py) << (8 * k);
            }
        }
        for (int k = 0; k < 4; ++k) {
            const int p = (int)((pw >> (8 * k)) & 0xff);
            const int d = (int)((sw >> (8 * k)) & 0xff) - p;
            pred[wave][r * 16 + c0 + k] = (uint8_t)p;
            res[wave][r * 16 + c0 + k] = (int16_t)d;
            lsad += d < 0 ? -d : d;
        }
        const int cr_ = lane >> 3, cc = lane & 7;
        const int xc = x0 / 2 + cc, yc = y0 / 2 + cr_;
        const Mv cv = px_mv(mi, 2 * cc, 2 * cr_);
        for (int comp = 0; comp < 2; ++comp) {
            const int p = chroma_pred8(ref_uv, g.pitch, cw, ch, comp, xc * 8 + cv.x, yc * 8 + cv.y);
            const int sv = src_uv[yc * g.pitch + 2 * xc + comp];
            pred[wave][256 + comp * 64 + cr_ * 8 + cc] = (uint8_t)p;
            res[wave][256 + comp * 64 + cr_ * 8 + cc] = (int16_t)(sv - p);
        }
    }
    __syncthreads();
    const uint32_t lsad_mb = (uint32_t)wave_sum(lsad);
    const int tcls = temporal_class((uint32_t)wave_sum(tsad), __ballot((mvx | mvy) != 0) == 0ull);
    const int qp = mb_qp_for(fs->qp, lsad_mb, tcls, fs->aq);
    const int qpc = chroma_qp(qp, fs->chroma_qp_offset);
    int16_t* mc = coef + (size_t)(valid ? mbi : 0) * kCoefStride;

    const int lb = lane >> 2, rr = lane & 3, lbx = kBlkX[lb], lby = kBlkY[lb];
    int x[4], y[4], z[4], rres[4];
    const int ro = (lby * 4 + rr) * 16 + lbx * 4;
#pragma unroll
    for (int c = 0; c < 4; ++c) x[c] = res[wave][ro + c];
    const int hs = quad_sum(had_row_abs(x, rr));
    fdct_row(x, rr, y);
    const int nzb = quad_sum(quant_row(y, rr, qp, false, 0, z));
    {
        int d[4];
        dequant_row(z, rr, qp, d);
        idct_row(d, rr, rres);
    }
    int d_pred = 0, d_coded = 0;
#pragma unroll
    for (int c = 0; c < 4; ++c) {
        const int pv = pred[wave][ro + c];
        const int e = pv + x[c] - clip255(pv + rres[c]);
        d_pred += x[c] * x[c];
        d_coded += e * e;
    }
    const uint32_t bits = rr == 0 ? block_bits_est(nzb) : 0u;
    const bool drop = valid && drop_luma_for(fs->aq, lsad_mb, tcls, qp, wave_sum(d_pred), wave_sum(d_coded),
                                             (uint32_t)wave_sum((int)bits));
    const bool drop_c = drop_chroma_for(fs->aq, tcls, drop);
    const int nz_l = drop ? 0 : nzb;
    int sse_y = 0;
    if (valid) {
        uint32_t packed = 0;
        const bool vis = x0 + lbx * 4 < g.width && (y0 + lby * 4 + rr) < g.height;
#pragma unroll
        for (int c = 0; c < 4; ++c) {
            if (drop) z[c] = rres[c] = 0;
            mc[kCoefLuma + lb * 16 + kZigzagInv4x4[rr * 4 + c]] = (int16_t)z[c];
            const int pv = pred[wave][ro + c];
            const int v = clip255(pv + rres[c]);
            const int e = pv + x[c] - v;
            sse_y += vis ? e * e : 0;
            packed |= (uint32_t)v << (8 * c);
        }
        *reinterpret_cast<uint32_t*>(fs->rec_y + (y0 + lby * 4 + rr) * g.pitch + x0 + lbx * 4) = packed;
        if (rr == 0) mbs[mbi].nz_luma[lby * 4 + lbx] = (uint8_t)nz_l;
    }
    const uint32_t satd_mb = (uint32_t)wave_sum(rr == 0 ? (hs + 1) >> 1 : 0);

    const int cbk = lane >> 2, ccomp = (cbk >> 2) & 1, cblk = cbk & 3, cbx = cblk & 1, cby = cblk >> 1;
    const int co = 256 + ccomp * 64 + (cby * 4 + rr) * 8 + cbx * 4;
    const bool clane = lane < 32;
    int cz[4], nzc = 0;
    if (clane) {
        int cx[4], cy[4];
#pragma unroll
        for (int c = 0; c < 4; ++c) cx[c] = drop_c ? 0 : res[wave][co + c];
        fdct_row(cx, rr, cy);
        if (rr == 0) cdc[wave][ccomp * 4 + cblk] = cy[0];
        nzc = quant_row(cy, rr, qpc, false, 1, cz);
    }
    nzc = quad_sum(nzc);
    if (valid && clane) {
#pragma unroll
        for (int c = 0; c < 4; ++c) {
            const int i = rr * 4 + c;
            if (i > 0) mc[kCoefChromaAc + (ccomp * 4 + cblk) * 16 + kZigzagInv4x4[i]] = (int16_t)cz[c];
        }
        if (rr == 0) (ccomp ? mbs[mbi].nz_cr : mbs[mbi].nz_cb)[cblk] = (uint8_t)nzc;
    }
    __syncthreads();
    if (valid && (lane == 0 || lane == 16)) {
        const int comp = lane >> 4;
        int in[4], zd[4], dq[4];
        for (int i = 0; i < 4; ++i) in[i] = cdc[wave][comp * 4 + i];
        const int n = quant_dc_chroma(in, zd, qpc, false);
        for (int i = 0; i < 4; ++i) mc[kCoefChromaDc + comp * 4 + i] = (int16_t)zd[i];
        dequant_dc_chroma(zd, dq, qpc);
        for (int i = 0; i < 4; ++i) cdc[wave][comp * 4 + i] = dq[i];
        cdc_nz[wave][comp] = n;
    }
    __syncthreads();
    int sse_c = 0;
    if (clane) {
        int d[4], cr[4];
        dequant_row(cz, rr, qpc, d);
        if (rr == 0) d[0] = cdc[wave][ccomp * 4 + cblk];
        idct_row(d, rr, cr);
        if (valid) {
            const int xc = x0 / 2 + cbx * 4, yc = y0 / 2 + cby * 4 + rr;
#pragma unroll
            for (int c = 0; c < 4; ++c) {
                const int v = clip255(pred[wave][co + c] + cr[c]);
                const int e = pred[wave][co + c] + res[wave][co + c] - v;
                sse_c += (2 * (xc + c) < g.width && 2 * yc < g.height) ? e * e : 0;
                fs->rec_uv[yc * g.pitch + 2 * (xc + c) + ccomp] = (uint8_t)v;
            }
        }
    }
    {
        const int sy = wave_sum(sse_y);
        const int su = wave_sum(lane < 16 ? sse_c : 0);
        const int sv = wave_sum((lane >= 16 && lane < 32) ? sse_c : 0);
        if (valid && fs->intra_in_p && lane < 3)
            mb_sse[lane * nmb + mbi] = (uint32_t)(lane == 0 ? sy : (lane == 1 ? su : sv));
        __shared__ uint32_t part[4][4];
        if (lane == 0) {
            part[0][wave] = valid ? (uint32_t)sy : 0u;
            part[1][wave] = valid ? (uint32_t)su : 0u;
            part[2][wave] = valid ? (uint32_t)sv : 0u;
            part[3][wave] = (valid && mb_unmasked(fs, mbx, mby)) ? (uint32_t)sy : 0u;
        }
        __syncthreads();
        if (threadIdx.x < 4) {
            const int c = threadIdx.x;
            fs->sse_part[c * kSsePartStride + bid] =
                (unsigned long long)part[c][0] + part[c][1] + part[c][2] + part[c][3];
        }
    }
    const unsigned long long luma_mask = __ballot(valid && rr == 0 && nz_l > 0);
    const unsigned long long chroma_mask = __ballot(valid && clane && rr == 0 && nzc > 0);
    if (valid && lane == 0) {
        int cbp = 0;
        for (int b8 = 0; b8 < 4; ++b8)
            if ((luma_mask >> (16 * b8)) & 0x1111ull) cbp |= 1 << b8;
        const int cc = (chroma_mask != 0) ? 2 : ((cdc_nz[wave][0] | cdc_nz[wave][1]) ? 1 : 0);
        cbp |= cc << 4;
        MbInfo& m = mbs[mbi];
        m.type = kMbP16x16;
        m.cbp = (uint8_t)cbp;
        m.qp = (uint8_t)qp;
        m.i16_mode = 0;
        m.chroma_mode = 0;
        m.cost = inter_cost_mb(satd_mb, fs->qp, mi);
    }
}

__constant__ uint8_t kRasterToBlk[16] = {0, 1, 4, 5, 2, 3, 6, 7, 8, 9, 12, 13, 10, 11, 14, 15};

constexpr int kLT = 24;
constexpr int kCT = 10;
constexpr int kCTI = 20;

__global__ __launch_bounds__(256) void k_intra_analyze(Geometry g, StateArg sa, const uint8_t* __restrict__ src_y,
                                                       const uint8_t* __restrict__ src_uv, MbInfo* __restrict__ mbs,
                                                       int* __restrict__ wave_prog, int32_t* __restrict__ gain,
                                                       int* __restrict__ cand) {
    __shared__ IntraCosts costs[4];
    __shared__ uint8_t ltile[4][17][kLT];
    __shared__ uint8_t ctile[4][9][kCTI];
    publish_state(sa);
    const FrameState* fs = &state_of(sa);
    if (blockIdx.x == 0) {
        if (!fs->idr)
            for (int i = threadIdx.x; i < 4 * g.mb_h; i += 256)
                fs->sse_part[(i / g.mb_h) * kSsePartStride + (g.mb_w * g.mb_h + 3) / 4 + i % g.mb_h] = 0;
    }
    const int wave = threadIdx.x >> 6, lane = threadIdx.x & 63;
    const int mbi = blockIdx.x * 4 + wave;
    if (mbi >= g.mb_w * g.mb_h) return;
    if (!fs->idr && !intra_candidate(mbs[mbi].cost)) {
        if (lane == 0) gain[mbi] = 0;
        return;
    }
    const int mbx = mbi % g.mb_w, mby = mbi / g.mb_w;
    const int x0 = mbx * 16, y0 = mby * 16;
    const Avail av = mb_avail(g, mbx, mby, fs->slice_rows);
    for (int i = lane; i < 17 * 21; i += 64) {
        const int r = i / 21, cx = i - r * 21, x = x0 - 1 + cx, y = y0 - 1 + r;
        ltile[wave][r][cx] = (x >= 0 && y >= 0 && x < g.coded_w) ? src_y[y * g.pitch + x] : 0;
    }
    for (int i = lane; i < 9 * 18; i += 64) {
        const int r = i / 18, bx = i - r * 18, x = x0 - 2 + bx, y = y0 / 2 - 1 + r;
        ctile[wave][r][bx] = (x >= 0 && y >= 0) ? src_uv[y * g.pitch + x] : 0;
    }
    wave_sync_lds();
    const uint8_t* sy = &ltile[wave][1][1];
    const uint8_t* suv = &ctile[wave][1][2];
    IntraCosts& c = costs[wave];
    const int rb = lane >> 2, r = lane & 3, bx = rb & 3, by = rb >> 2;
    auto satd_quad = [&](int d0, int d1, int d2, int d3) -> uint32_t {
        int t[4] = {d0 + d1 + d2 + d3, d0 + d1 - d2 - d3, d0 - d1 - d2 + d3, d0 - d1 + d2 - d3};
        uint32_t sum = 0;
#pragma unroll
        for (int j = 0; j < 4; ++j) {
            int v = t[j];
            int o = __builtin_amdgcn_mov_dpp(v, 0xB1, 0xF, 0xF, false);
            v = (r & 1) ? o - v : v + o;
            o = __builtin_amdgcn_mov_dpp(v, 0x4E, 0xF, 0xF, false);
            v = (r & 2) ? o - v : v + o;
            sum += (uint32_t)(v < 0 ? -v : v);
        }
        sum += (uint32_t)__builtin_amdgcn_mov_dpp((int)sum, 0xB1, 0xF, 0xF, false);
        sum += (uint32_t)__builtin_amdgcn_mov_dpp((int)sum, 0x4E, 0xF, 0xF, false);
        return (sum + 1) >> 1;
    };
    {
        const Nb4 n = nb4_from_plane(sy, kLT, 0, 0, bx, by, av.left, av.top, av.topright, av.topleft);
        int sv[4];
#pragma unroll
        for (int j = 0; j < 4; ++j) sv[j] = sy[(4 * by + r) * kLT + 4 * bx + j];
        for (int m = 0; m < 9; ++m) {
            const bool ok = i4_mode_ok(m, n);
            int d[4];
#pragma unroll
            for (int j = 0; j < 4; ++j) d[j] = ok ? sv[j] - pred4x4_px(m, n, j, r) : 0;
            const uint32_t t = satd_quad(d[0], d[1], d[2], d[3]);
            if (r == 0) c.c4[kRasterToBlk[rb]][m] = ok ? t : kCostInf;
        }
    }
    {
        const NbMb n = nbmb_from_plane(sy, kLT, 0, 0, 16, 1, 0, av.left, av.top, av.topleft);
        for (int m = 0; m < 4; ++m) {
            const bool ok = i16_mode_ok(m, n);
            uint32_t t = 0;
            if (ok) {
                const PredMb p = prep_i16(m, n);
                int d[4];
#pragma unroll
                for (int j = 0; j < 4; ++j)
                    d[j] = (int)sy[(4 * by + r) * kLT + 4 * bx + j] - pred16_px(p, n, 4 * bx + j, 4 * by + r);
                t = satd_quad(d[0], d[1], d[2], d[3]);
                t = r == 0 ? t : 0u;
                t += (uint32_t)__builtin_amdgcn_mov_dpp((int)t, 0x124, 0xF, 0xF, false);
                t += (uint32_t)__builtin_amdgcn_mov_dpp((int)t, 0x128, 0xF, 0xF, false);
                t = rows_sum(t);
            }
            if (lane == 0) c.c16[m] = ok ? t : kCostInf;
        }
    }
    {
        const int comp = (lane >> 4) & 1, cb = (lane >> 2) & 3, cbx = cb & 1, cby = cb >> 1;
        const NbMb n = nbmb_from_plane(suv, kCTI, 0, 0, 8, 2, comp, av.left, av.top, av.topleft);
        for (int m = 0; m < 4; ++m) {
            const bool ok = chroma_mode_ok(m, n);
            uint32_t t = 0;
            if (ok) {
                const PredMb p = prep_chroma(m, n);
                int d[4];
#pragma unroll
                for (int j = 0; j < 4; ++j)
                    d[j] = lane < 32 ? (int)suv[(4 * cby + r) * kCTI + 2 * (4 * cbx + j) + comp] -
                                           predc_px(p, n, 4 * cbx + j, 4 * cby + r)
                                     : 0;
                t = satd_quad(d[0], d[1], d[2], d[3]);
                t = (r == 0 && lane < 32) ? t : 0u;
                t += (uint32_t)__builtin_amdgcn_mov_dpp((int)t, 0x124, 0xF, 0xF, false);
                t += (uint32_t)__builtin_amdgcn_mov_dpp((int)t, 0x128, 0xF, 0xF, false);
                t = rows_sum(t);
            }
            if (lane == 0) c.cc[m] = ok ? t : kCostInf;
        }
    }
    __builtin_amdgcn_fence(__ATOMIC_RELEASE, "wavefront");
    __builtin_amdgcn_wave_barrier();
    __builtin_amdgcn_fence(__ATOMIC_ACQUIRE, "wavefront");
    if (lane == 0) {
        const IntraDecision d = decide_intra(c, fs->qp, fs->intra4x4 != 0);
        MbInfo& m = mbs[mbi];
        const int32_t gn = fs->idr ? 1 : intra_gain(d.cost_luma, m.cost, fs->qp);
        if (!fs->idr) {
            gain[mbi] = gn;
            if (gn > 0) cand[atomicAdd(&wave_prog[1], 1)] = mbi;
        }
        if (gn > 0) {
            const int qp = fs->qp;
            if (fs->idr)
                m.type = (uint8_t)d.type;
            else
                m.itype = (uint8_t)d.type;
            m.i16_mode = (uint8_t)d.i16_mode;
            m.chroma_mode = (uint8_t)d.chroma_mode;
            uint8_t md[8];
            for (int rb = 0; rb < 16; rb += 2) md[rb >> 1] = (uint8_t)(d.i4[rb] | (d.i4[rb + 1] << 4));
            for (int k = 0; k < 8; ++k) m.i4[k] = md[k];
            if (fs->idr) {
                m.qp = (uint8_t)qp;
                m.mvx = 0;
                m.mvy = 0;
            }
        }
    }
}



struct MbFields {
    int type, qp, i16_mode, chroma_mode;
    uint32_t i4lo, i4hi;
    __device__ int i4(int rb) const { return (int)(((rb < 8 ? i4lo : i4hi) >> (4 * (rb & 7))) & 15u); }
};
__device__ __forceinline__ MbFields load_fields(const MbInfo* m) {
    const uint32_t* w = reinterpret_cast<const uint32_t*>(m);
    const uint32_t d1 = w[1], d8 = w[8], d9 = w[9], d10 = w[10];
    MbFields f;
    f.type = (int)(d1 & 0xff);
    f.i16_mode = (int)((d1 >> 16) & 0xff);
    f.chroma_mode = (int)(d1 >> 24);
    f.qp = (int)((d8 >> 8) & 0xff);
    f.i4lo = d9;
    f.i4hi = d10;
    return f;
}
static_assert(offsetof(MbInfo, type) == 4 && offsetof(MbInfo, i16_mode) == 6 && offsetof(MbInfo, chroma_mode) == 7 &&
                  offsetof(MbInfo, qp) == 33 && offsetof(MbInfo, i4) == 36,
              "load_fields() layout");


struct QpTab {
// ... 499 lines not shown
                }
            }
            if (!open && t > 4 * (started - 1) + 9) break;
            const int j = lane >> 3, grp = (lane >> 2) & 1, r = lane & 3;
            const int k = j == 0 ? sk[0] : (j == 1 ? sk[1] : sk[2]);
            const int sl = t - 4 * k;
            const bool mine = lane < 24 && k >= 0 && sl <= 9;
            const int rb = mine ? i4_step_block(sl, grp) : -1;
            int nzb = 0;
            if (rb >= 0) {
                const int x = base + k, mbi = mby * g.mb_w + x;
                const uint32_t lo = j == 0 ? mlo[0] : (j == 1 ? mlo[1] : mlo[2]);
                const uint32_t hi = j == 0 ? mhi[0] : (j == 1 ? mhi[1] : mhi[2]);
                const int mode = (int)(((rb < 8 ? lo : hi) >> (4 * (rb & 7))) & 15u);
                uint32_t e2 = 0;
                nzb = i4_code_block(g, rb, r, mode, T, P.src[j], P.lt[j], coef + (size_t)mbi * kCoefStride, x * 16, y0,
                                    mb_avail(g, x, mby, slice_rows), e2);
                sse_a += e2;
                if (j == 0 ? um[0] : (j == 1 ? um[1] : um[2])) sse_m += e2;
                if (r == 0) mbs[mbi].nz_luma[rb] = (uint8_t)nzb;
            }
            const unsigned long long any = __ballot(rb >= 0 && r == 0 && nzb > 0);
            wave_sync_lds();
#pragma unroll
            for (int s = 0; s < 3; ++s) {
                const int ks = sk[s], ss = t - 4 * ks;
                if (ks < 0 || ss > 9) continue;
#pragma unroll
                for (int gq = 0; gq < 2; ++gq)
                    if ((any >> (8 * s + 4 * gq)) & 1ull) cbp[s] |= 1 << (raster_to_blk(i4_step_block(ss, gq)) >> 2);
                if (ss >= 3 && (ss & 1)) {
                    const int by = (ss - 3) >> 1, jn = s == 2 ? 0 : s + 1;
                    if (lane < 4) P.lt[jn][1 + 4 * by + lane][0] = P.lt[s][1 + 4 * by + lane][16];
                }
                if (ss == 9) {
                    if (lane == 0) mbs[mby * g.mb_w + base + ks].cbp = (uint8_t)cbp[s];
                    finish(base + ks);
                }
            }
            wave_sync_lds();
        }
        next = base + started;
    }
#ifdef MX_IDR_TIMING
    if (lane == 0) printf("MXIDR plane 0 slice %d row %d wall_ticks %llu\n", (int)blockIdx.x, wave, wall_clock64() - t_start);
#endif
    unsigned long long a = sse_a, mm = sse_m;
    for (int o = 32; o > 0; o >>= 1) {
        a += __shfl_xor(a, o, 64);
        mm += __shfl_xor(mm, o, 64);
    }
    if (lane == 0) {
        fs->sse_part[0 * kSsePartStride + mby] = a;
        fs->sse_part[3 * kSsePartStride + mby] = mm;
    }
}

__global__ __launch_bounds__(512) void k_intra_wave(Geometry g, const FrameState* __restrict__ fs,
                                                     const uint8_t* __restrict__ src_y,
                                                     const uint8_t* __restrict__ src_uv, MbInfo* __restrict__ mbs,
                                                     int16_t* __restrict__ coef) {
    __builtin_amdgcn_s_setprio(3);
    extern __shared__ uint8_t s_line[];
    __shared__ IntraWaveTiles tiles[8];
    __shared__ LumaPipeTiles ltiles[8];
    __shared__ int prog[8];
    if ((threadIdx.x & 63) == 0) prog[threadIdx.x >> 6] = 0;
    __syncthreads();
    if (blockIdx.y == 0)
        intra_luma_rows_pl(g, fs, src_y, mbs, coef, s_line, ltiles, prog);
    else
        intra_wave_rows<true>(g, fs, src_y, src_uv, mbs, coef, s_line, tiles, prog);
}

__global__ __launch_bounds__(256) void k_intra_cbp(Geometry g, MbInfo* __restrict__ mbs) {
    const int i = blockIdx.x * 256 + threadIdx.x;
    if (i >= g.mb_w * g.mb_h) return;
    MbInfo& m = mbs[i];
    m.cbp = (uint8_t)((m.cbp & 15) | (m.cbp_c << 4));
}

__device__ void intra_p_mb(const Geometry& g, const FrameState* __restrict__ fs, const uint8_t* __restrict__ src_y,
                           const uint8_t* __restrict__ src_uv, MbInfo* __restrict__ mbs, int16_t* __restrict__ coef,
                           const int32_t* __restrict__ gain, const uint32_t* __restrict__ mb_sse, int mbi) {
    __shared__ uint8_t lt[17][kLT];
    __shared__ uint8_t ct[2][9][kCT];
    __shared__ uint32_t ls[64];
    __shared__ uint32_t cs[32];
    __shared__ int ldc[16], cdc[8];
    const int mbx = mbi % g.mb_w, mby = mbi / g.mb_w;
    if (!intra_selected(gain, g.mb_w, g.mb_h, mbx, mby)) return;
    const int wave = threadIdx.x >> 6, lane = threadIdx.x & 63;
    MbInfo& m = mbs[mbi];
    MbFields f = load_fields(&m);
    f.type = m.itype;
    f.qp = fs->qp;
    const Avail av = mb_avail(g, mbx, mby, fs->slice_rows);
    int16_t* mc = coef + (size_t)mbi * kCoefStride;
    uint32_t s0 = 0, s1 = 0;
    __syncthreads();
    if (threadIdx.x == 0) {
        m.type = (uint8_t)f.type;
        m.qp = (uint8_t)f.qp;
        m.mvx = 0;
        m.mvy = 0;
    }
    if (wave == 0) {
        const int x0 = mbx * 16, y0 = mby * 16;
        {
            const int r = lane >> 2, c4 = (lane & 3) * 4;
            ls[lane] = *reinterpret_cast<const uint32_t*>(src_y + (size_t)(y0 + r) * g.pitch + x0 + c4);
        }
        if (lane < 16) lt[1 + lane][0] = av.left ? fs->rec_y[(y0 + lane) * g.pitch + x0 - 1] : 0;
        if (lane < 21) {
            const bool ok = lane == 0 ? av.topleft : (lane <= 16 ? av.top : av.topright);
            lt[0][lane] = ok ? fs->rec_y[(y0 - 1) * g.pitch + x0 - 1 + lane] : 0;
        }
        wave_sync_lds();
        intra_luma_mb(g, f, ls, m, mc, mbx, mby, av, lt, ldc, lane, s0);
        const int r = lane >> 2, c4 = (lane & 3) * 4;
        const uint32_t v = (uint32_t)lt[1 + r][1 + c4] | ((uint32_t)lt[1 + r][2 + c4] << 8) |
                           ((uint32_t)lt[1 + r][3 + c4] << 16) | ((uint32_t)lt[1 + r][4 + c4] << 24);
        *reinterpret_cast<uint32_t*>(fs->rec_y + (y0 + r) * g.pitch + x0 + c4) = v;
    } else {
        const int xc0 = mbx * 8, yc0 = mby * 8;
        if (lane < 32) {
            const int r = lane >> 2, c4 = (lane & 3) * 4;
            cs[lane] = *reinterpret_cast<const uint32_t*>(src_uv + (size_t)(yc0 + r) * g.pitch + mbx * 16 + c4);
        }
        if (lane < 16) {
            const int comp = lane >> 3, r = lane & 7;
            ct[comp][1 + r][0] = av.left ? fs->rec_uv[(yc0 + r) * g.pitch + 2 * (xc0 - 1) + comp] : 0;
        } else if (lane < 34) {
            const int k = lane - 16, comp = k / 9, cx = k - comp * 9;
            const bool ok = cx == 0 ? av.topleft : av.top;
            ct[comp][0][cx] = ok ? fs->rec_uv[(yc0 - 1) * g.pitch + 2 * (xc0 - 1 + cx) + comp] : 0;
        }
        wave_sync_lds();
        intra_chroma_mb(g, fs->chroma_qp_offset, f, cs, m, mc, mbx, mby, av, ct, cdc, lane, s0, s1);
        if (lane < 32) {
            const int r = lane >> 2, c2 = (lane & 3) * 2;
            const uint32_t v = (uint32_t)ct[0][1 + r][1 + c2] | ((uint32_t)ct[1][1 + r][1 + c2] << 8) |
                               ((uint32_t)ct[0][1 + r][2 + c2] << 16) | ((uint32_t)ct[1][1 + r][2 + c2] << 24);
            *reinterpret_cast<uint32_t*>(fs->rec_uv + (yc0 + r) * g.pitch + 2 * (xc0 + c2)) = v;
        }
    }
    unsigned long long a = s0, b = s1;
    for (int o = 32; o > 0; o >>= 1) {
        a += __shfl_xor(a, o, 64);
        b += __shfl_xor(b, o, 64);
    }
    __syncthreads();
    const int nmb = g.mb_w * g.mb_h;
    const int slot = (nmb + 3) / 4 + mby;
    if (lane == 0) {
        if (wave == 0) {
            m.cbp = (uint8_t)((m.cbp & 15) | (m.cbp_c << 4));
            atomicAdd(&fs->sse_part[slot], a - mb_sse[mbi]);
            if (mb_unmasked(fs, mbx, mby)) atomicAdd(&fs->sse_part[3 * kSsePartStride + slot], a - mb_sse[mbi]);
        } else {
            atomicAdd(&fs->sse_part[kSsePartStride + slot], a - mb_sse[nmb + mbi]);
            atomicAdd(&fs->sse_part[2 * kSsePartStride + slot], b - mb_sse[2 * nmb + mbi]);
        }
    }
}

__global__ __launch_bounds__(128) void k_intra_p(Geometry g, const FrameState* __restrict__ fs,
                                                 const uint8_t* __restrict__ src_y, const uint8_t* __restrict__ src_uv,
                                                 MbInfo* __restrict__ mbs, int16_t* __restrict__ coef,
                                                 const int32_t* __restrict__ gain, const uint32_t* __restrict__ mb_sse,
                                                 const int* __restrict__ wave_prog, const int* __restrict__ cand) {
    const int ncand = wave_prog[1];
    for (int k = blockIdx.x; k < ncand; k += gridDim.x) intra_p_mb(g, fs, src_y, src_uv, mbs, coef, gain, mb_sse, cand[k]);
}

__device__ __forceinline__ uint32_t mask_bits(int n) { return n >= 32 ? 0xffffffffu : ((1u << n) - 1); }

template <class F>
__device__ __forceinline__ void overlap(uint32_t& acc, uint32_t W0, uint32_t s0, uint32_t len, F getbits) {
    const uint32_t lo = max(W0, s0), hi = min(W0 + 32, s0 + len);
    if (lo >= hi) return;
    const int n = (int)(hi - lo);
    const uint32_t bits = getbits(lo - s0, n) & mask_bits(n);
    acc |= bits << (W0 + 32 - hi);
}

constexpr int kRoleWords = 24;
__device__ __forceinline__ uint32_t role_get(const uint32_t* buf, uint32_t b, int n) {
    const uint32_t wi = b >> 5, sh = b & 31;
    const uint64_t hi = ((uint64_t)buf[wi] << 32) | (wi + 1 < (uint32_t)kRoleWords ? buf[wi + 1] : 0u);
    return (uint32_t)((hi << sh) >> (64 - n));
}

constexpr int kCavlcMbPerBlock = 8;
__global__ __launch_bounds__(256) void k_cavlc(Geometry g, const FrameState* __restrict__ fs, MbInfo* __restrict__ mbs,
                                               const int16_t* __restrict__ coef, uint32_t* __restrict__ slot,
                                               uint32_t* __restrict__ slot_bits) {
    static_assert(kNumRoles < 32, "the roles of one MB (plus the total slot) must fit a half-wave");
    __shared__ uint32_t rbuf[kCavlcMbPerBlock][kNumRoles][kRoleWords];
    __shared__ uint32_t roff[kCavlcMbPerBlock][kNumRoles + 1];
    __shared__ __attribute__((aligned(16))) int16_t cbuf[kCavlcMbPerBlock][kCoefStride];
    __shared__ MbInfo nbuf[kCavlcMbPerBlock][5];
    static_assert(sizeof(MbInfo) % 4 == 0, "MbInfo copied as dwords");
    const int hw = (threadIdx.x >> 5) & 1, lane = threadIdx.x & 31;
    const int wave = threadIdx.x >> 5;
    const int nmb = g.mb_w * g.mb_h;
    const int mbi = blockIdx.x * kCavlcMbPerBlock + wave;
    if (mbi >= nmb) return;
    const int mbx = mbi % g.mb_w, mby = mbi / g.mb_w;
    const Avail av = mb_avail(g, mbx, mby, fs->slice_rows);
    {
        const int src[5] = {mbi, mbi - 1, mbi - g.mb_w, mbi - g.mb_w + 1, mbi - g.mb_w - 1};
        const bool ok[5] = {true, av.left, av.top, av.topright, av.topleft};
        constexpr int kW = (int)(sizeof(MbInfo) / 4);
        for (int q = lane; q < 5 * kW; q += 32) {
            const int k = q / kW, d = q - k * kW;
            if (ok[k]) reinterpret_cast<uint32_t*>(&nbuf[wave][k])[d] = reinterpret_cast<const uint32_t*>(&mbs[src[k]])[d];
        }
        __builtin_amdgcn_fence(__ATOMIC_RELEASE, "wavefront");
        __builtin_amdgcn_wave_barrier();
        __builtin_amdgcn_fence(__ATOMIC_ACQUIRE, "wavefront");
    }
    const MbNbrs nb{&nbuf[wave][0], &nbuf[wave][1], &nbuf[wave][2], &nbuf[wave][3], &nbuf[wave][4]};
    const MbInfo& m = nbuf[wave][0];
    const int16_t* mc = coef + (size_t)mbi * kCoefStride;

    int mvd[4];
    const bool skip = decide_skip(nb, av, mvd);
    int dqp = 0;
    if (!skip && !fs->idr && carries_dqp(m)) {
        const int per_slice = fs->slice_rows * g.mb_w, first = (mbi / per_slice) * per_slice;
        int pred = fs->qp;
        bool found = false;
        constexpr int kPer = 16;
        for (int j0 = mbi - 1; j0 >= first && !found; j0 -= 32 * kPer) {
            int qv[kPer];
#pragma unroll
            for (int k = 0; k < kPer; ++k) {
                const int j = j0 - 32 * k - lane;
                qv[k] = -1;
                if (j >= first) {
                    const MbInfo& mj = mbs[j];
                    if (carries_dqp(mj)) qv[k] = mj.qp;
                }
            }
#pragma unroll
            for (int k = 0; k < kPer; ++k) {
                const unsigned long long bal = __ballot(qv[k] >= 0);
                const uint32_t hb = (uint32_t)(bal >> (32 * hw));
                const int q = __shfl(qv[k], hb ? (int)(__ffs(hb) - 1) : 0, 32);
                if (!found && hb) {
                    pred = q;
                    found = true;
                }
            }
        }
        dqp = qp_delta(m.qp, pred);
    }
    if (!skip) {
        const uint4* src = reinterpret_cast<const uint4*>(mc);
        uint4* dst = reinterpret_cast<uint4*>(cbuf[wave]);
        for (int q = lane; q < kCoefStride / 8; q += 32) dst[q] = src[q];
    }
    __builtin_amdgcn_fence(__ATOMIC_RELEASE, "wavefront");
    __builtin_amdgcn_wave_barrier();
    __builtin_amdgcn_fence(__ATOMIC_ACQUIRE, "wavefront");
    uint32_t bits = 0;
    if (!skip && lane < kNumRoles) {
        BitWriter w;
        w.init(rbuf[wave][lane]);
        code_role(w, lane, g, fs->idr, nb, cbuf[wave], av, mvd, dqp);
        w.flush();
        bits = w.bits;
    }
    uint32_t incl = bits;
    incl += (uint32_t)__builtin_amdgcn_update_dpp(0, (int)incl, 0x111, 0xF, 0xF, false);
    incl += (uint32_t)__builtin_amdgcn_update_dpp(0, (int)incl, 0x112, 0xF, 0xF, false);
    incl += (uint32_t)__builtin_amdgcn_update_dpp(0, (int)incl, 0x114, 0xF, 0xF, false);
    incl += (uint32_t)__builtin_amdgcn_update_dpp(0, (int)incl, 0x118, 0xF, 0xF, false);
    incl += (uint32_t)__builtin_amdgcn_update_dpp(0, (int)incl, 0x142, 0xA, 0xF, false);
    const uint32_t total = __shfl(incl, 31, 32);
    if (lane < kNumRoles) roff[wave][lane] = incl - bits;
    if (lane == kNumRoles) roff[wave][kNumRoles] = total;
    __builtin_amdgcn_fence(__ATOMIC_RELEASE, "wavefront");
    __builtin_amdgcn_wave_barrier();
    __builtin_amdgcn_fence(__ATOMIC_ACQUIRE, "wavefront");
    const bool fits = total <= kSlotWords * 32u;
    if (!skip && fits) {
        const uint32_t nwords = (total + 31) >> 5;
        uint32_t* dst = slot + (size_t)mbi * kSlotWords;
        for (uint32_t wi = lane; wi < nwords; wi += 32) {
            const uint32_t W0 = wi * 32;
            int r = 0;
            while (r < kNumRoles - 1 && roff[wave][r + 1] <= W0) ++r;
            uint32_t acc = 0;
            for (; r < kNumRoles; ++r) {
                const uint32_t o = roff[wave][r], len = roff[wave][r + 1] - o;
                if (o >= W0 + 32) break;
                if (len == 0) continue;
                overlap(acc, W0, o, len, [&](uint32_t x, int n) { return role_get(rbuf[wave][r], x, n); });
            }
            dst[wi] = acc;
        }
    }
    if (lane == 0) {
        slot_bits[mbi] = skip ? 0u : (fits ? total : 0xffffffffu);
        mbs[mbi].skip = skip ? 1 : 0;
    }
}

constexpr int kScanThreads = 256;
constexpr int kScanRowPer = 2;
constexpr int kScanMaxRows = 512;

template <typename T, typename Op>
__device__ __forceinline__ T blk_excl_scan(T v, T init, Op op, T* wbuf, T* total) {
    constexpr int kW = kScanThreads / 64;
    const int lane = threadIdx.x & 63, w = threadIdx.x >> 6;
    T incl = v;
    for (int o = 1; o < 64; o <<= 1) {
        const T t = __shfl_up(incl, o, 64);
        if (lane >= o) incl = op(incl, t);
    }
    T excl = __shfl_up(incl, 1, 64);
    if (lane == 0) excl = init;
    if (lane == 63) wbuf[w] = incl;
    __syncthreads();
    T before = init, all = init;
    for (int k = 0; k < kW; ++k) {
        if (k < w) before = op(before, wbuf[k]);
        all = op(all, wbuf[k]);
    }
    __syncthreads();
    *total = all;
    return op(before, excl);
}

__device__ __forceinline__ uint32_t blk_excl_sum(uint32_t v, uint32_t* wbuf, uint32_t* total) {
    return blk_excl_scan<uint32_t>(v, 0u, [](uint32_t a, uint32_t b) { return a + b; }, wbuf, total);
}
__device__ __forceinline__ int blk_excl_max(int v, int init, int* wbuf, int* total) {
    return blk_excl_scan<int>(v, init, [](int a, int b) { return max(a, b); }, wbuf, total);
}

__device__ __forceinline__ SliceParams slice_params(const FrameState* fs, int s, int mb_w) {
    return make_slice_params(s * fs->slice_rows * mb_w, fs->idr, fs->frame_num, fs->log2_max_frame_num,
                             fs->idr_pic_id, fs->qp - fs->pic_init_qp, fs->deblock_off);
}

__global__ __launch_bounds__(kScanThreads) void k_scan_rows(Geometry g, const FrameState* __restrict__ fs,
                                                            const uint32_t* __restrict__ slot_bits,
                                                            uint4* __restrict__ row_agg,
                                                            unsigned long long* __restrict__ row_sse,
                                                            const MbInfo* __restrict__ mbs, uint32_t* __restrict__ db_cnt) {
    __shared__ int wi[kScanThreads / 64];
    __shared__ uint32_t wu[kScanThreads / 64];
    const int t = threadIdx.x, r = blockIdx.x, base = r * g.mb_w;
    const bool idr = fs->idr != 0;
    const int nmb = g.mb_w * g.mb_h;
    const int nparts = (idr || !fs->deblock_off) ? g.mb_h : (nmb + 3) / 4 + (fs->intra_in_p ? g.mb_h : 0);
    const int p0 = (int)((long long)nparts * r / g.mb_h), p1 = (int)((long long)nparts * (r + 1) / g.mb_h);
    unsigned long long acc[4] = {0, 0, 0, 0};
    for (int i = p0 + t; i < p1; i += kScanThreads)
        for (int c = 0; c < 4; ++c) acc[c] += fs->sse_part[c * kSsePartStride + i];
    uint32_t b[kScanRowPer];
    int last = -1, first = 0x7fffffff;
    uint32_t ncoded = 0, over = 0;
#pragma unroll
    for (int k = 0; k < kScanRowPer; ++k) {
        const int j = t * kScanRowPer + k;
        b[k] = j < g.mb_w ? slot_bits[base + j] : 0u;
        if (b[k] == 0xffffffffu) {
            over = 1;
            b[k] = 1;
        }
        if (b[k]) {
            last = base + j;
            first = min(first, base + j);
            ++ncoded;
        }
    }
    int lastall;
    int prev = blk_excl_max(last, -1, wi, &lastall);
    uint32_t bits = 0;
#pragma unroll
    for (int k = 0; k < kScanRowPer; ++k) {
        if (!b[k]) continue;
        const int i = base + t * kScanRowPer + k;
        if (prev >= 0 && !idr) bits += (uint32_t)ue_len((uint32_t)(i - prev - 1));
        bits += b[k];
        prev = i;
    }
    uint32_t tb, tc, to;
    (void)blk_excl_sum(bits, wu, &tb);
    (void)blk_excl_sum(ncoded, wu, &tc);
    (void)blk_excl_sum(over, wu, &to);
    int firstall;
    (void)blk_excl_scan<int>(first, 0x7fffffff, [](int x, int y) { return min(x, y); }, wi, &firstall);
    if (t == 0)
        row_agg[r] = make_uint4((uint32_t)(lastall >= 0 ? firstall : -1), (uint32_t)lastall,
                                tc | (to ? 0x80000000u : 0u), tb);
    __shared__ unsigned long long red[4][kScanThreads / 64];
    for (int c = 0; c < 4; ++c) {
        unsigned long long v = acc[c];
        for (int o = 32; o > 0; o >>= 1) v += __shfl_xor(v, o);
        if ((t & 63) == 0) red[c][t >> 6] = v;
    }
    __syncthreads();
    if (t < 4) {
        unsigned long long v = 0;
        for (int w = 0; w < kScanThreads / 64; ++w) v += red[t][w];
        row_sse[t * kScanMaxRows + r] = v;
    }
    if (idr || !db_cnt) return;
    DbAutoCounts ac;
    for (int j = t; j < g.mb_w; j += kScanThreads) db_auto_count(mbs, g.mb_w, base + j, ac);
    uint32_t cv[3] = {ac.coherent, ac.changed, ac.moving};
    __shared__ uint32_t cred[3][kScanThreads / 64];
    for (int c = 0; c < 3; ++c) {
        for (int o = 32; o > 0; o >>= 1) cv[c] += __shfl_xor(cv[c], o);
        if ((t & 63) == 0) cred[c][t >> 6] = cv[c];
    }
    __syncthreads();
    if (t < 3) {
        uint32_t v = 0;
        for (int w = 0; w < kScanThreads / 64; ++w) v += cred[t][w];
        if (v) atomicAdd(&db_cnt[t], v);
    }
}

__global__ __launch_bounds__(kScanThreads) void k_scan_out(Geometry g, const FrameState* __restrict__ fs,
                                                           const uint32_t* __restrict__ slot_bits,
                                                           const uint4* __restrict__ row_agg,
                                                           const unsigned long long* __restrict__ row_sse,
                                                           uint4* __restrict__ coded_info,
                                                           uint32_t* __restrict__ slice_info, size_t out_bytes,
                                                           OutHeader* __restrict__ hdr,
                                                           uint32_t* __restrict__ quad_unit, uint32_t* __restrict__ db_cnt) {
    __shared__ int s_lbraw[kScanMaxRows + 1];
    __shared__ uint32_t s_P[kScanMaxRows + 1];
    __shared__ uint32_t s_R[kScanMaxRows + 1];
    __shared__ uint32_t s_soff[kScanThreads + 1], s_sbytes[kScanThreads], s_hbits[kScanThreads];
    __shared__ int wi[kScanThreads / 64];
    __shared__ uint32_t wu[kScanThreads / 64];
    const int t = threadIdx.x, r = blockIdx.x, mb_w = g.mb_w, mb_h = g.mb_h;
    const bool idr = fs->idr != 0;
    const int srows = fs->slice_rows, ns = fs->num_slices;
    const int base = r * mb_w;
    uint32_t b[kScanRowPer];
#pragma unroll
    for (int k = 0; k < kScanRowPer; ++k) {
        const int j = t * kScanRowPer + k;
        b[k] = j < mb_w ? slot_bits[base + j] : 0u;
    }
    unsigned long long dsum[4] = {0, 0, 0, 0};
    if (r == 0)
        for (int j = t; j < mb_h; j += kScanThreads)
            for (int c = 0; c < 4; ++c) dsum[c] += row_sse[c * kScanMaxRows + j];
    uint4 ag[2];
    int lastr = -1;
#pragma unroll
    for (int k = 0; k < 2; ++k) {
        const int j = 2 * t + k;
        ag[k] = j < mb_h ? row_agg[j] : make_uint4(0xffffffffu, 0xffffffffu, 0u, 0u);
        lastr = max(lastr, (int)ag[k].y);
    }
    int dummy, lastframe;
    int lb = blk_excl_max(lastr, -1, wi, &lastframe);
    uint32_t contrib[2], nc[2], over = 0;
#pragma unroll
    for (int k = 0; k < 2; ++k) {
        const int j = 2 * t + k;
        contrib[k] = 0;
        nc[k] = ag[k].z & 0x7fffffffu;
        over |= ag[k].z >> 31;
        if (j < mb_h) {
            s_lbraw[j] = lb;
            const int sfirst = (j / srows) * srows * mb_w;
            const int pv = max(lb, sfirst - 1);
            contrib[k] = ag[k].w;
            if ((int)ag[k].x >= 0 && !idr) contrib[k] += (uint32_t)ue_len((uint32_t)((int)ag[k].x - pv - 1));
        }
        lb = max(lb, (int)ag[k].y);
    }
    uint32_t ptot, rtot, otot;
    uint32_t pex = blk_excl_sum(contrib[0] + contrib[1], wu, &ptot);
    uint32_t rex = blk_excl_sum(nc[0] + nc[1], wu, &rtot);
    (void)blk_excl_sum(over, wu, &otot);
#pragma unroll
    for (int k = 0; k < 2; ++k) {
        const int j = 2 * t + k;
        if (j < mb_h) {
            s_P[j] = pex;
            s_R[j] = rex;
        }
        pex += contrib[k];
        rex += nc[k];
    }
    if (t == 0) {
        s_P[mb_h] = ptot;
        s_R[mb_h] = rtot;
        s_lbraw[mb_h] = lastframe;
    }
    __syncthreads();
    uint32_t sbytes = 0, hb = 0;
    if (t < ns) {
        const int fr = t * srows, er = min(fr + srows, mb_h);
        const int sfirst = fr * mb_w, slast = er * mb_w - 1;
        const uint32_t data = s_P[er] - s_P[fr];
        const int lastin = max(s_lbraw[er], sfirst - 1);
        const uint32_t trail = idr ? 0u : (uint32_t)(slast - lastin);
        BitCounter bc;
        bc.init(nullptr);
        write_slice_header(bc, slice_params(fs, t, mb_w));
        hb = bc.bits;
        const uint32_t bits = hb + data + (trail ? ue_len(trail) : 0) + 1;
        sbytes = (bits + 7) >> 3;
// ... 115 lines not shown

__global__ __launch_bounds__(256) void k_pack(Geometry g, const FrameState* __restrict__ fs,
                                              const uint32_t* __restrict__ slot,
                                              const uint4* __restrict__ coded_info,
                                              const uint32_t* __restrict__ slice_info,
                                              const OutHeader* __restrict__ hdr, uint8_t* __restrict__ host,
                                              const uint32_t* __restrict__ quad_unit, uint32_t* __restrict__ done) {
    const OutHeader h = *hdr;
    pack_body(g, fs, slot, coded_info, slice_info, h, host, quad_unit);
    __syncthreads();
    if (threadIdx.x == 0) {
        const uint32_t prev = __hip_atomic_fetch_add(done, 1u, __ATOMIC_RELAXED, __HIP_MEMORY_SCOPE_AGENT);
        if (prev == gridDim.x - 1) {
            reinterpret_cast<OutHeader*>(host)->t_end = wall_clock64();
            __hip_atomic_store(done, 0u, __ATOMIC_RELAXED, __HIP_MEMORY_SCOPE_AGENT);
        }
    }
}

__device__ void pack_body(const Geometry& g, const FrameState* __restrict__ fs, const uint32_t* __restrict__ slot,
                          const uint4* __restrict__ coded_info, const uint32_t* __restrict__ slice_info,
                          const OutHeader& h, uint8_t* __restrict__ host, const uint32_t* __restrict__ quad_unit) {
    const size_t gid = (size_t)blockIdx.x * 256 + threadIdx.x;
    const size_t stride = (size_t)gridDim.x * 256;
    if (gid == 0) *reinterpret_cast<OutHeader*>(host) = h;
    uint32_t* hs = reinterpret_cast<uint32_t*>(host + sizeof(OutHeader));
    for (size_t s = gid; s < h.num_slices; s += stride) {
        hs[s] = slice_info[kSliceInfo * s + 1];
        hs[kMaxSlices + s] = slice_info[kSliceInfo * s + 2];
    }
    if (h.overflow) return;
    const bool idr = fs->idr != 0;
    const int ns = (int)h.num_slices;
    const uint32_t nquads = (h.total_bytes + 15) / 16;
    uint4* out = reinterpret_cast<uint4*>(host + kOutPayloadOffset);
    const int sub = threadIdx.x & 3;
    for (size_t qbase = gid >> 2; qbase < ((nquads + 63) / 64) * 64; qbase += stride >> 2) {
        const bool active = qbase < nquads;
        uint32_t acc = 0;
        if (active) {
            const uint32_t W0 = (uint32_t)qbase * 128 + 32 * sub;
            const int qa = (int)quad_unit[qbase];
            int lo = 0, hi = ns - 1;
            while (lo < hi) {
                const int mid = (lo + hi + 1) >> 1;
                if (slice_info[kSliceInfo * mid + 1] * 8 <= W0) lo = mid; else hi = mid - 1;
            }
            for (int s = lo; s < ns; ++s) {
                const uint32_t sbit = slice_info[kSliceInfo * s + 1] * 8;
                if (sbit >= W0 + 32) break;
                const uint32_t hbits = slice_info[kSliceInfo * s + 0];
                const uint32_t dend = slice_info[kSliceInfo * s + 4];
                if (sbit + slice_info[kSliceInfo * s + 2] * 8 <= W0) continue;
                const uint32_t trail = idr ? 0u : slice_info[kSliceInfo * s + 3];
                if (sbit + hbits > W0) {
                    uint32_t hw[4] = {0, 0, 0, 0};
                    BitWriter bw;
                    bw.init(hw);
                    write_slice_header(bw, slice_params(fs, s, g.mb_w));
                    bw.flush();
                    overlap(acc, W0, sbit, hbits, [&](uint32_t x, int n) { return slot_get(hw, x, n); });
                }
                if (dend > W0 && sbit + hbits < W0 + 32) {
                    int a = max((int)slice_info[kSliceInfo * s + 6], qa);
                    const int rend = (int)slice_info[kSliceInfo * s + 7];
                    const int b = rend - 1;
                    while (a < b && coded_info[a + 1].x <= W0) ++a;
                    for (int r = a; r < rend; ++r) {
                        const uint4 ci = coded_info[r];
                        const uint32_t off = ci.x;
                        if (off >= W0 + 32) break;
                        if (off + ci.z <= W0) continue;
                        const int run = (int)ci.w;
                        const int plen = idr ? 0 : ue_len((uint32_t)run);
                        const uint32_t pv = (uint32_t)run + 1;
                        const uint32_t* sp = slot + (size_t)ci.y * kSlotWords;
                        overlap(acc, W0, off, ci.z, [&](uint32_t x, int n) {
                            uint32_t r2 = 0;
                            int rem = n;
                            if ((int)x < plen) {
                                const int kk = min(rem, plen - (int)x);
                                r2 = (pv >> (plen - (int)x - kk)) & mask_bits(kk);
                                rem -= kk;
                                x += kk;
                            }
                            if (rem > 0) r2 = (rem == 32 ? 0u : (r2 << rem)) | slot_get(sp, x - plen, rem);
                            return r2;
                        });
                    }
                }
                const int tl = trail ? ue_len(trail) : 0;
                const uint32_t tv = trail ? (((trail + 1) << 1) | 1u) : 1u;
                overlap(acc, W0, dend, tl + 1, [&](uint32_t x, int n) { return tv >> (tl + 1 - (int)x - n); });
            }
        }
        const uint32_t w = bswap32(acc);
        const int lane = threadIdx.x & 63, q0 = lane & ~3;
        const uint32_t w0 = __shfl(w, q0), w1 = __shfl(w, q0 + 1), w2 = __shfl(w, q0 + 2), w3 = __shfl(w, q0 + 3);
        if (active && sub == 0) out[qbase] = make_uint4(w0, w1, w2, w3);
    }
}

}

void launch_hpel(const Geometry& g, const DeviceBuffers& b, uint8_t* const planes[4], int hp_pitch,
                 hipStream_t stream, const FrameState* publish) {
    const int W = g.coded_w + 2 * kHpelPad, H = g.coded_h + 2 * kHpelPad;
    dim3 grid((W + kHpTW - 1) / kHpTW, (H + kHpTH - 1) / kHpTH);
    StateArg sa{};
    if (publish) sa.v = *publish;
    sa.dst = b.fs;
    sa.publish = publish ? 1 : 0;
    sa.t_start = b.out_hdr ? &b.out_hdr->t_start : nullptr;
    hipLaunchKernelGGL(k_hpel, grid, dim3(256), 0, stream, g, sa, planes[0], planes[1], planes[2], planes[3],
                       hp_pitch);
}

__global__ __launch_bounds__(256) void k_copy_luma(const uint4* __restrict__ src, uint4* __restrict__ dst, size_t n) {
    const size_t i = (size_t)blockIdx.x * 256 + threadIdx.x;
    if (i < n) dst[i] = src[i];
}

void launch_copy_luma(const Geometry& g, const uint8_t* luma, uint8_t* dst, hipStream_t stream) {
    const size_t n = (size_t)g.pitch * g.coded_h / 16;
    hipLaunchKernelGGL(k_copy_luma, dim3((unsigned)((n + 255) / 256)), dim3(256), 0, stream,
                       reinterpret_cast<const uint4*>(luma), reinterpret_cast<uint4*>(dst), n);
}

void launch_mc_luma_test(const Geometry& g, const uint8_t* ref, int x4, int y4, uint8_t* out, hipStream_t stream) {
    hipLaunchKernelGGL(k_mc_luma_test, dim3(1), dim3(64), 0, stream, g, ref, x4, y4, out);
}

void launch_me(const Geometry& g, const DeviceBuffers& b, const uint8_t* src_y, hipStream_t stream,
               const FrameState* publish, bool side) {
    const int nmb = g.mb_w * g.mb_h;
    StateArg sa{};
    if (publish) sa.v = *publish;
    sa.dst = b.fs;
    sa.publish = publish ? 1 : 0;
    sa.t_start = b.out_hdr ? &b.out_hdr->t_start : nullptr;
    if (side && publish)
        hipLaunchKernelGGL(k_me_full_val, dim3(nmb), dim3(kMeThreads), 0, stream, g, sa, src_y, b.mb);
    else
        hipLaunchKernelGGL(k_me_full, dim3(nmb), dim3(kMeThreads), 0, stream, g, sa, src_y, b.mb);
}

void launch_inter(const Geometry& g, const DeviceBuffers& b, const uint8_t* src_y, const uint8_t* src_uv,
                  hipStream_t stream) {
    const int nmb = g.mb_w * g.mb_h;
    hipLaunchKernelGGL(k_inter_encode, dim3((nmb + 3) / 4), dim3(256), 0, stream, g, b.fs, src_y, src_uv, b.mb,
                       b.coef, b.mb_sse, b.wave_prog);
}

static void launch_analyze(const Geometry& g, const DeviceBuffers& b, const uint8_t* src_y, const uint8_t* src_uv,
                           hipStream_t stream, const FrameState* publish, bool first) {
    const int nmb = g.mb_w * g.mb_h;
    StateArg sa{};
    if (publish) sa.v = *publish;
    sa.dst = b.fs;
    sa.publish = publish ? 1 : 0;
    sa.t_start = (b.out_hdr && first) ? &b.out_hdr->t_start : nullptr;
    hipLaunchKernelGGL(k_intra_analyze, dim3((nmb + 3) / 4), dim3(256), 0, stream, g, sa, src_y, src_uv, b.mb,
                       b.wave_prog, b.intra_gain, b.intra_cand);
}

void launch_intra_in_p(const Geometry& g, const DeviceBuffers& b, const uint8_t* src_y, const uint8_t* src_uv,
                       hipStream_t stream) {
    launch_analyze(g, b, src_y, src_uv, stream, nullptr, false);
    hipLaunchKernelGGL(k_intra_p, dim3(256), dim3(128), 0, stream, g, b.fs, src_y, src_uv, b.mb, b.coef,
                       b.intra_gain, b.mb_sse, b.wave_prog, b.intra_cand);
}

void launch_intra(const Geometry& g, const DeviceBuffers& b, const uint8_t* src_y, const uint8_t* src_uv,
                  hipStream_t stream, const FrameState* publish) {
    launch_analyze(g, b, src_y, src_uv, stream, publish, true);
    const int rows = idr_slice_rows(g.mb_h), slices = (g.mb_h + rows - 1) / rows;
    const size_t lds = (size_t)rows * g.coded_w;
    ensure_func_attr(reinterpret_cast<const void*>(&k_intra_wave), hipFuncAttributeMaxDynamicSharedMemorySize,
                     160 * 1024 - (int)(sizeof(IntraWaveTiles) + sizeof(LumaPipeTiles)) * 8 - 32);
    hipLaunchKernelGGL(k_intra_wave, dim3(slices, 2), dim3(64 * rows), lds, stream, g, b.fs, src_y, src_uv, b.mb,
                       b.coef);
    hipLaunchKernelGGL(k_intra_cbp, dim3((g.mb_w * g.mb_h + 255) / 256), dim3(256), 0, stream, g, b.mb);
}

__global__ __launch_bounds__(256) void k_save_src(Geometry g, const FrameState* __restrict__ fs,
                                                   const uint8_t* __restrict__ src_y) {
    const size_t i = (size_t)blockIdx.x * 256 + threadIdx.x;
    const size_t n = (size_t)g.pitch * g.coded_h / 16;
    if (i < n) reinterpret_cast<uint4*>(fs->save_src)[i] = reinterpret_cast<const uint4*>(src_y)[i];
}

void launch_save_src(const Geometry& g, const DeviceBuffers& b, const uint8_t* src_y, hipStream_t stream) {
    const size_t n = (size_t)g.pitch * g.coded_h / 16;
    hipLaunchKernelGGL(k_save_src, dim3((unsigned)((n + 255) / 256)), dim3(256), 0, stream, g, b.fs, src_y);
}

void launch_entropy(const Geometry& g, const DeviceBuffers& b, uint8_t* host_out, hipStream_t stream,
                    hipEvent_t wait_for_sse) {
    const int nmb = g.mb_w * g.mb_h;
    hipLaunchKernelGGL(k_cavlc, dim3((nmb + kCavlcMbPerBlock - 1) / kCavlcMbPerBlock), dim3(256), 0, stream, g, b.fs,
                       b.mb, b.coef, b.slot,
                       b.slot_bits);
    if (wait_for_sse) HIP_CHECK(hipStreamWaitEvent(stream, wait_for_sse, 0));
    if (g.mb_h > kScanMaxRows || g.mb_w > kScanThreads * kScanRowPer)
        throw std::runtime_error("launch_entropy: frame too large for the row scan");
    hipLaunchKernelGGL(k_scan_rows, dim3(g.mb_h), dim3(kScanThreads), 0, stream, g, b.fs, b.slot_bits, b.row_agg,
                       b.row_sse, b.mb, b.db_cnt);
    hipLaunchKernelGGL(k_scan_out, dim3(g.mb_h), dim3(kScanThreads), 0, stream, g, b.fs, b.slot_bits, b.row_agg,
                       b.row_sse, b.coded_info, b.slice_info, b.out_bytes, b.out_hdr, b.quad_unit, b.db_cnt);
    hipLaunchKernelGGL(k_pack, dim3(256), dim3(256), 0, stream, g, b.fs, b.slot, b.coded_info, b.slice_info,
                       b.out_hdr, host_out, b.quad_unit, b.pack_done);
}

}
}
```

### csrc/codec/h264_mb.h

```cpp
#pragma once
#include "h264_core.h"
#include "h264_gpu.h"
#include "h264_intra.h"

namespace mx {
namespace h264 {

constexpr int kNumRoles = 28;

struct Avail {
    bool left, top, topright, topleft;
};

MXHD Avail mb_avail(const Geometry& g, int mbx, int mby, int slice_rows) {
    Avail a;
    const bool top_same_slice = mby > 0 && (mby / slice_rows) == ((mby - 1) / slice_rows);
    a.left = mbx > 0;
    a.top = top_same_slice;
    a.topright = top_same_slice && mbx < g.mb_w - 1;
    a.topleft = top_same_slice && mbx > 0;
    return a;
}

MXHD int combine_nc(bool ha, int na, bool hb, int nb) {
// ... 79 lines not shown
        const Mv p1 = predict_mv_part(nb, av, m.part, 1, v0);
        mvd[0] = v0.x - p0.x;
        mvd[1] = v0.y - p0.y;
        mvd[2] = v1.x - p1.x;
        mvd[3] = v1.y - p1.y;
        return false;
    }
    const MvNb a = mv_nb_blk(nb.left, av.left, 3, 0);
    const MvNb b = mv_nb_blk(nb.top, av.top, 0, 3);
    MvNb c = mv_nb_blk(nb.topright, av.topright, 0, 3);
    if (!av.topright) c = mv_nb_blk(nb.topleft, av.topleft, 3, 3);
    const Mv pskip = predict_mv_skip(a, b, c);
    const Mv p = predict_mv16x16(a, b, c);
    mvd[0] = m.mvx - p.x;
    mvd[1] = m.mvy - p.y;
    return m.cbp == 0 && m.mvx == pskip.x && m.mvy == pskip.y;
}

template <class W>
MXHD void code_role(W& w, int role, const Geometry& g, int idr, const MbNbrs& nb, const int16_t* mc,
                    const Avail& av, const int* mvd, int dqp = 0) {
    const MbInfo& m = *nb.self;
    const bool intra = m.type == kMbI16x16;
    const int cbp = m.cbp;
    const int cbp_l = cbp & 15, cbp_c = cbp >> 4;
    const MbInfo* ml = av.left ? nb.left : nullptr;
    const MbInfo* mt = av.top ? nb.top : nullptr;
    if (role == 0) {
        if (intra) {
            const int mbtype = 1 + m.i16_mode + 4 * cbp_c + (cbp_l ? 12 : 0);
            put_ue(w, (uint32_t)(idr ? mbtype : 5 + mbtype));
            put_ue(w, m.chroma_mode);
            put_se(w, dqp);
        } else if (m.type == kMbI4x4) {
            put_ue(w, idr ? 0u : 5u);
            for (int b = 0; b < 16; ++b) {
                const int bx = kBlkX[b], by = kBlkY[b];
                const bool ha = bx > 0 || av.left, hb = by > 0 || av.top;
                int ma = -1, mb = -1;
                if (bx > 0) ma = i4_get(m.i4, by * 4 + bx - 1);
                else if (ml && ml->type == kMbI4x4) ma = i4_get(ml->i4, by * 4 + 3);
                if (by > 0) mb = i4_get(m.i4, (by - 1) * 4 + bx);
                else if (mt && mt->type == kMbI4x4) mb = i4_get(mt->i4, 12 + bx);
                const int pm = i4_pred_mode(ma, mb, ha, hb);
                const int mode = i4_get(m.i4, by * 4 + bx);
                if (mode == pm) {
                    w.put(1, 1);
                } else {
                    w.put(0, 1);
                    w.put((uint32_t)(mode < pm ? mode : mode - 1), 3);
                }
            }
            put_ue(w, m.chroma_mode);
            put_ue(w, (uint32_t)cbp_to_codenum(cbp, true));
            if (cbp) put_se(w, dqp);
        } else {
            put_ue(w, m.part);
            put_se(w, mvd[0]);
            put_se(w, mvd[1]);
            if (m.part != kPart16x16) {
                put_se(w, mvd[2]);
                put_se(w, mvd[3]);
            }
            put_ue(w, (uint32_t)cbp_to_codenum(cbp, false));
            if (cbp) put_se(w, dqp);
        }
        return;
    }
    if (role == 1) {
        if (!intra) return;
        const int nc = combine_nc(av.left, ml ? ml->nz_luma[3] : 0, av.top, mt ? mt->nz_luma[12] : 0);
        cavlc_block(w, mc + kCoefLumaDc, 16, nc);
        return;
    }
    if (role <= 17) {
        const int b = role - 2;
        if (!(cbp_l & (1 << (b >> 2)))) return;
        const int bx = kBlkX[b], by = kBlkY[b];
        const bool ha = bx > 0 || av.left, hb = by > 0 || av.top;
        const int na = bx > 0 ? m.nz_luma[by * 4 + bx - 1] : (ml ? ml->nz_luma[by * 4 + 3] : 0);
        const int nb = by > 0 ? m.nz_luma[(by - 1) * 4 + bx] : (mt ? mt->nz_luma[12 + bx] : 0);
        const int nc = combine_nc(ha, na, hb, nb);
        if (intra) {
            cavlc_block(w, mc + kCoefLuma + b * 16 + 1, 15, nc);
        } else {
            cavlc_block(w, mc + kCoefLuma + b * 16, 16, nc);
        }
        return;
    }
    if (role <= 19) {
        if (!cbp_c) return;
        const int comp = role - 18;
        cavlc_block(w, mc + kCoefChromaDc + comp * 4, 4, -1);
        return;
    }
    if (role < kNumRoles) {
        if (cbp_c != 2) return;
        const int comp = (role - 20) >> 2, cb = (role - 20) & 3, bx = cb & 1, by = cb >> 1;
        const uint8_t* own = comp ? m.nz_cr : m.nz_cb;
        const uint8_t* lft = ml ? (comp ? ml->nz_cr : ml->nz_cb) : nullptr;
        const uint8_t* top = mt ? (comp ? mt->nz_cr : mt->nz_cb) : nullptr;
        const bool ha = bx > 0 || av.left, hb = by > 0 || av.top;
        const int na = bx > 0 ? own[by * 2] : (lft ? lft[by * 2 + 1] : 0);
        const int nb = by > 0 ? own[bx] : (top ? top[2 + bx] : 0);
        const int nc = combine_nc(ha, na, hb, nb);
        cavlc_block(w, mc + kCoefChromaAc + (comp * 4 + cb) * 16 + 1, 15, nc);
    }
}

MXHD int aq_mb_qp(int frame_qp, uint32_t sad, int aq) {
    if (!aq) return frame_qp;
    const int off = sad > 256u * 48 ? 12 : (sad > 256u * 32 ? 6 : 0);
    const int q = frame_qp + off;
    return q > 51 ? 51 : q;
}

MXHD int lambda_sse(int qp) {
    constexpr int tab[52] = {0,   0,   0,   0,   0,   0,   0,   0,   0,    0,    1,    1,    1,    1,
                             1,   2,   2,   3,   3,   4,   5,   7,   9,    11,   14,   17,   22,   27,
                             34,  43,  54,  69,  86,  109, 137, 173, 218,  274,  345,  435,  548,  691,
                             870, 1097, 1382, 1741, 2193, 2763, 3482, 4387, 5527, 6963};
    return tab[qp < 0 ? 0 : (qp > 51 ? 51 : qp)];
}
MXHD uint32_t block_bits_est(int nz) { return nz ? 2u + 6u * (uint32_t)nz : 0u; }
MXHD bool drop_residual(int aq, uint32_t lsad, int qp, long long d_pred, long long d_coded, uint32_t bits) {
    if (aq < 2 || lsad <= 256u * 32) return false;
    return d_pred - d_coded < (long long)lambda_sse(qp) * (long long)bits;
}

constexpr uint32_t kTsadChanging = 256u * 24, kTsadPersistent = 256u * 2;
constexpr int kAqChangingOffset = 6, kAqPersistentOffset = -6;
MXHD int aq_static_offset(int aq) { return kAqPersistentOffset - 3 * ((aq > 6 ? 6 : aq) - 3); }
enum TClass : int { kTcNormal = 0, kTcPersistent = 1, kTcChanging = 2, kTcStatic = 3 };
MXHD int temporal_class(uint32_t tsad, bool zero_mv) {
    return tsad > kTsadChanging ? kTcChanging
                                : (tsad == 0 && zero_mv ? kTcStatic : (tsad <= kTsadPersistent ? kTcPersistent : kTcNormal));
}
MXHD int aq3_mb_qp(int frame_qp, int tclass, int aq = 3) {
    const int q = frame_qp + (tclass == kTcChanging     ? kAqChangingOffset
                              : tclass == kTcStatic     ? aq_static_offset(aq)
                              : tclass == kTcPersistent ? kAqPersistentOffset
                                                        : 0);
    return q < 0 ? 0 : (q > 51 ? 51 : q);
}
MXHD int mb_qp_for(int frame_qp, uint32_t lsad, int tclass, int aq) {
    return aq >= 3 ? aq3_mb_qp(frame_qp, tclass, aq) : aq_mb_qp(frame_qp, lsad, aq);
}
MXHD bool drop_luma_for(int aq, uint32_t lsad, int tclass, int qp, long long d_pred, long long d_coded,
                        uint32_t bits) {
    if (aq >= 3)
        return tclass == kTcChanging && d_pred - d_coded < (long long)lambda_sse(qp) * (long long)bits;
    return drop_residual(aq, lsad, qp, d_pred, d_coded, bits);
}
MXHD bool drop_chroma_for(int aq, int tclass, bool luma_dropped) {
    return luma_dropped || (aq >= 3 && tclass == kTcChanging);
}

MXHD uint32_t inter_cost(uint32_t satd, int frame_qp, int mvx, int mvy) {
    return satd + (uint32_t)(lambda_sad(frame_qp) * (mvd_bits(mvx) + mvd_bits(mvy)));
}
MXHD uint32_t inter_cost_mb(uint32_t satd, int frame_qp, const MbInfo& m) {
    if (m.part == kPart16x16) return inter_cost(satd, frame_qp, m.mvx, m.mvy);
    return satd + (uint32_t)(lambda_sad(frame_qp) *
                             (mvd_bits(m.pmv[0]) + mvd_bits(m.pmv[1]) + mvd_bits(m.pmv[2]) + mvd_bits(m.pmv[3])));
}

MXHD int idr_slice_rows(int mb_h) {
    const int ns = (mb_h + 3) / 4;
    return (mb_h + ns - 1) / ns;
}

MXHD int qp_delta(int qp, int pred) { return ((qp - pred + 26 + 52) % 52) - 26; }

MXHD SliceParams make_slice_params(int first_mb, int idr, int frame_num, int log2_max_frame_num, int idr_pic_id,
                                   int qp_delta, int deblock_off) {
    SliceParams sp;
    sp.first_mb = first_mb;
    sp.idr = idr;
    sp.frame_num = frame_num;
    sp.log2_max_frame_num = log2_max_frame_num;
    sp.idr_pic_id = idr_pic_id;
    sp.qp_delta = qp_delta;
    sp.disable_deblock = deblock_off;
    return sp;
}


MXHD int luma_block_inter(const int* res, int qp, int* zscan, int* rres) {
    int y[16], z[16], d[16];
    fdct4x4(res, y);
    const int nz = quant4x4(y, z, qp, false, 0);
    for (int k = 0; k < 16; ++k) zscan[k] = z[kZigzag4x4[k]];
    dequant4x4(z, d, qp, 0);
    idct4x4(d, rres);
    return nz;
}

MXHD uint32_t me_cost(uint32_t sad, int lambda, int mvx, int mvy) {
    return sad + (uint32_t)(lambda * (mvd_bits(mvx) + mvd_bits(mvy)));
}

MXHD int me_range(int r) {
    r = r < 4 ? 4 : (r > 32 ? 32 : r);
    return (r + 3) & ~3;
}
constexpr uint32_t kStaticSad = 128;
MXHD uint32_t static_sad(int qp) {
    const uint32_t t = 64u * (uint32_t)lambda_sad(qp);
    return t > kStaticSad ? t : kStaticSad;
}

MXHD void subpel_offset(int k, int* dx, int* dy) {
    *dx = (k < 3) ? (k - 1) : (k == 3 ? -1 : (k == 4 ? 1 : (k - 6)));
    *dy = (k < 3) ? -1 : ((k == 3 || k == 4) ? 0 : 1);
}

}
}
```

Measured before the change: 10830.

## Fuse motion estimation and inter coding into one kernel with zero-block early skip

Adds a fused P-frame kernel that runs full-pel/subpel motion search and then codes the macroblock in the same block. The coder's LDS aliases the search window, and motion vectors are passed in registers, which removes a kernel launch and the round trip of motion data through global memory. The inter coder also gains SAD-based bounds that prove a luma or chroma block quantises to zero, so it can skip residual staging for those blocks. Per-MB SSE is summed directly in the row scan instead of through partial slots. In exchange, only one wave per 256-thread block does the coding step, which may idle most of the block during that phase.

```diff
diff --git a/csrc/bindings/module.cpp b/csrc/bindings/module.cpp
--- a/csrc/bindings/module.cpp
+++ b/csrc/bindings/module.cpp
@@ -139,6 +139,28 @@
         return h264::luma_qpel(plane.data(), W, W, H, x4, y4);
     });
     h.def("level_for", &h264::pick_level);
+    h.def("zero_sum_4x4", [](int qp) { return h264::zero_sum_4x4(qp); }, py::arg("qp"));
+    h.def("zero_sum_chroma_dc", [](int qpc) { return h264::zero_sum_chroma_dc(qpc); }, py::arg("qpc"));
+    h.def("chroma_qp", [](int qp, int offset) { return h264::chroma_qp(qp, offset); }, py::arg("qp"),
+          py::arg("offset") = 0);
+    h.def("quant4x4", [](py::array_t<int, py::array::c_style | py::array::forcecast> y, int qp, bool intra, int start) {
+        if (y.size() != 16) throw std::invalid_argument("need 16 values");
+        py::array_t<int> z(16);
+        const int nz = h264::quant4x4(y.data(), z.mutable_data(), qp, intra, start);
+        return py::make_tuple(z, nz);
+    }, py::arg("y"), py::arg("qp"), py::arg("intra") = false, py::arg("start") = 0);
+    h.def("quant_dc_chroma", [](py::array_t<int, py::array::c_style | py::array::forcecast> dc, int qpc, bool intra) {
+        if (dc.size() != 4) throw std::invalid_argument("need 4 values");
+        py::array_t<int> z(4);
+        const int nz = h264::quant_dc_chroma(dc.data(), z.mutable_data(), qpc, intra);
+        return py::make_tuple(z, nz);
+    }, py::arg("dc"), py::arg("qpc"), py::arg("intra") = false);
+    h.def("luma_block_inter", [](py::array_t<int, py::array::c_style | py::array::forcecast> res, int qp) {
+        if (res.size() != 16) throw std::invalid_argument("need 16 values");
+        py::array_t<int> z(16), rr(16);
+        const int nz = h264::luma_block_inter(res.data(), qp, z.mutable_data(), rr.mutable_data());
+        return py::make_tuple(z, rr, nz);
+    }, py::arg("res"), py::arg("qp"), "inter luma block: residual (raster) -> levels (scan), reconstructed residual, nz");
 
     py::class_<h264::EncoderConfig>(m, "EncoderConfig")
         .def(py::init<>())
diff --git a/csrc/codec/h264_encoder.cpp b/csrc/codec/h264_encoder.cpp
--- a/csrc/codec/h264_encoder.cpp
+++ b/csrc/codec/h264_encoder.cpp
@@ -307,7 +307,7 @@
     if (geom_.mb_h > kMaxSlices) throw std::invalid_argument("picture too tall");
     if (geom_.mb_w > 512) throw std::invalid_argument("picture too wide (k_intra_wave stages <= 512 MBs per row)");
     const int nmb = geom_.mb_w * geom_.mb_h;
-    if ((nmb + 3) / 4 + geom_.mb_h > kSsePartStride)
+    if (geom_.mb_h > kSsePartStride)
         throw std::invalid_argument("frame too large for the distortion partials");
     const size_t ysz = (size_t)geom_.pitch * geom_.coded_h, uvsz = ysz / 2;
     for (int i = 0; i < 2; ++i) {
@@ -468,11 +468,15 @@
             launch_me(geom_, sl.buf, src_y, stream_m_, pub, true);
             HIP_CHECK(hipEventRecord(sl.me_done, stream_m_));
             HIP_CHECK(hipStreamWaitEvent(stream_, sl.me_done, 0));
+            launch_inter(geom_, sl.buf, src_y, src_uv, stream_);
+        } else if (!sl.me_unf && geom_.mb_w * geom_.mb_h <= kFusedMaxMbs) {
+            wait_input();
+            launch_p_fused(geom_, sl.buf, src_y, src_uv, stream_, pub);
         } else {
             wait_input();
             launch_me(geom_, sl.buf, src_y, stream_, pub);
-        }
-        launch_inter(geom_, sl.buf, src_y, src_uv, stream_);
+            launch_inter(geom_, sl.buf, src_y, src_uv, stream_);
+        }
         if (cfg_.intra_in_p) launch_intra_in_p(geom_, sl.buf, src_y, src_uv, stream_);
     }
 }
diff --git a/csrc/codec/h264_gpu.h b/csrc/codec/h264_gpu.h
--- a/csrc/codec/h264_gpu.h
+++ b/csrc/codec/h264_gpu.h
@@ -134,6 +134,9 @@
 void launch_mc_luma_test(const Geometry& g, const uint8_t* ref, int x4, int y4, uint8_t* out, hipStream_t stream);
 void launch_inter(const Geometry& g, const DeviceBuffers& b, const uint8_t* src_y, const uint8_t* src_uv,
                   hipStream_t stream);
+constexpr int kFusedMaxMbs = 8160;
+void launch_p_fused(const Geometry& g, const DeviceBuffers& b, const uint8_t* src_y, const uint8_t* src_uv,
+                    hipStream_t stream, const FrameState* publish = nullptr);
 void launch_intra(const Geometry& g, const DeviceBuffers& b, const uint8_t* src_y, const uint8_t* src_uv,
                   hipStream_t stream, const FrameState* publish = nullptr);
 void launch_hpel(const Geometry& g, const DeviceBuffers& b, uint8_t* const planes[4], int hp_pitch,
diff --git a/csrc/codec/h264_kernels.hip b/csrc/codec/h264_kernels.hip
--- a/csrc/codec/h264_kernels.hip
+++ b/csrc/codec/h264_kernels.hip
@@ -201,6 +201,7 @@
 constexpr int kWinPadX = 4, kWinPadY = 3;
 constexpr int kWinStride = 16 + 2 * kMaxRange + 8;
 constexpr int kWinRows = 16 + 2 * kMaxRange + 7;
+constexpr int kWinWords = kWinRows * kWinStride / 4;
 
 constexpr int kMeThreads = 256, kMeWaves = kMeThreads / 64;
 constexpr int kFpRows = 18 + 5;
@@ -232,9 +233,12 @@
 __device__ __forceinline__ MeState me_state(const FrameState& f) {
     return MeState{f.me_ref ? f.me_ref : f.ref_y, f.qp, f.search_range, f.subpel, f.me_coarse, f.partitions};
 }
-__device__ __forceinline__ void me_full_body(const Geometry& g, const MeState& st, const uint8_t* __restrict__ src_y,
-                                             MbInfo* __restrict__ mbs) {
-    __shared__ uint32_t win_lds[kWinRows * kWinStride / 4];
+__device__ __forceinline__ MbInfo me_full_body(const Geometry& g, const MeState& st, const uint8_t* __restrict__ src_y,
+                                               MbInfo* __restrict__ mbs, uint32_t* win_lds) {
+    MbInfo out;
+    out.mvx = out.mvy = 0;
+    out.part = kPart16x16;
+    out.pmv[0] = out.pmv[1] = out.pmv[2] = out.pmv[3] = 0;
     __shared__ uint8_t sp2[2][4][18][kSpW];
     __shared__ int16_t fp_b1[2][kFpRows][kSpW];
     __shared__ uint32_t srcw[64];
@@ -270,7 +274,7 @@
                 m.part = kPart16x16;
                 m.pmv[0] = m.pmv[1] = m.pmv[2] = m.pmv[3] = 0;
             }
-            return;
+            return out;
         }
     }
     const bool t256 = tid < 256;
@@ -574,7 +578,14 @@
                 m.pmv[2] = (int16_t)pvx[1];
                 m.pmv[3] = (int16_t)pvy[1];
             }
-            return;
+            out.mvx = (int16_t)mvx;
+            out.mvy = (int16_t)mvy;
+            out.part = (uint8_t)part;
+            out.pmv[0] = (int16_t)pvx[0];
+            out.pmv[1] = (int16_t)pvy[0];
+            out.pmv[2] = (int16_t)pvx[1];
+            out.pmv[3] = (int16_t)pvy[1];
+            return out;
         }
     }
 
@@ -625,17 +636,22 @@
         m.part = kPart16x16;
         m.pmv[0] = m.pmv[1] = m.pmv[2] = m.pmv[3] = 0;
     }
+    out.mvx = (int16_t)mvx;
+    out.mvy = (int16_t)mvy;
+    return out;
 }
 
 __global__ __launch_bounds__(kMeThreads) void k_me_full(Geometry g, StateArg sa, const uint8_t* __restrict__ src_y,
                                                         MbInfo* __restrict__ mbs) {
+    __shared__ uint32_t win_lds[kWinWords];
     publish_state(sa);
-    me_full_body(g, sa.publish ? me_state(sa.v) : me_state(*sa.dst), src_y, mbs);
+    me_full_body(g, sa.publish ? me_state(sa.v) : me_state(*sa.dst), src_y, mbs, win_lds);
 }
 __global__ __launch_bounds__(kMeThreads) void k_me_full_val(Geometry g, StateArg sa, const uint8_t* __restrict__ src_y,
                                                             MbInfo* __restrict__ mbs) {
+    __shared__ uint32_t win_lds[kWinWords];
     publish_state(sa);
-    me_full_body(g, me_state(sa.v), src_y, mbs);
+    me_full_body(g, me_state(sa.v), src_y, mbs, win_lds);
 }
 
 template <int K>
@@ -788,65 +804,76 @@
     reinterpret_cast<uint32_t*>(out)[lane] = p;
 }
 
-__global__ __launch_bounds__(256) void k_inter_encode(Geometry g, const FrameState* __restrict__ fs,
-                                                       const uint8_t* __restrict__ src_y,
-                                                       const uint8_t* __restrict__ src_uv, MbInfo* __restrict__ mbs,
-                                                       int16_t* __restrict__ coef, uint32_t* __restrict__ mb_sse,
-                                                       int* __restrict__ wave_prog) {
-    __shared__ uint8_t pred[4][384];
-    __shared__ int16_t res[4][384];
-    __shared__ uint32_t mcw[4][2 * kMcWords];
-    __shared__ int cdc[4][8];
-    __shared__ int cdc_nz[4][2];
-
-    const int wave = threadIdx.x >> 6, lane = threadIdx.x & 63;
+struct CodeState {
+    const uint8_t* ref_y;
+    const uint8_t* ref_uv;
+    uint8_t* rec_y;
+    uint8_t* rec_uv;
+    const uint8_t* prev_src;
+    uint8_t* save_src;
+    int qp, aq, intra_in_p, chroma_qp_offset;
+};
+__device__ __forceinline__ CodeState code_state(const FrameState& f) {
+    return CodeState{f.ref_y, f.ref_uv, f.rec_y, f.rec_uv, f.prev_src, f.save_src, f.qp, f.aq, f.intra_in_p,
+                     f.chroma_qp_offset};
+}
+struct InterLds {
+    __attribute__((aligned(4))) uint8_t pred[384];
+    int16_t res[384];
+    uint32_t mcw[2 * kMcWords];
+    int cdc[8];
+    int cdc_nz[2];
+};
+__device__ __forceinline__ void inter_code_mb(const Geometry& g, const CodeState& fs, const uint8_t* __restrict__ src_y,
+                                              const uint8_t* __restrict__ src_uv, MbInfo* __restrict__ mbs,
+                                              int16_t* __restrict__ coef, uint32_t* __restrict__ mb_sse, int mbi,
+                                              int lane, const MbInfo& motion, InterLds& L) {
+    MbInfo mi;
+    mi.mvx = (int16_t)__builtin_amdgcn_readfirstlane((int)motion.mvx);
+    mi.mvy = (int16_t)__builtin_amdgcn_readfirstlane((int)motion.mvy);
+    mi.part = (uint8_t)__builtin_amdgcn_readfirstlane((int)motion.part);
+    for (int i = 0; i < 4; ++i) mi.pmv[i] = (int16_t)__builtin_amdgcn_readfirstlane((int)motion.pmv[i]);
     const int nmb = g.mb_w * g.mb_h;
-    const int bid = blockIdx.x;
-    const int mbi = bid * 4 + wave;
-    if (bid == 0 && threadIdx.x == 0) wave_prog[1] = 0;
-    const bool valid = mbi < nmb;
-    const int mbx = valid ? mbi % g.mb_w : 0, mby = valid ? mbi / g.mb_w : 0;
+    const int mbx = mbi % g.mb_w, mby = mbi / g.mb_w;
     const int x0 = mbx * 16, y0 = mby * 16;
-    const uint8_t* __restrict__ ref_y = fs->ref_y;
+    const uint8_t* __restrict__ ref_y = fs.ref_y;
     const bool ref_dwords = (g.pitch & 3) == 0 && (reinterpret_cast<uintptr_t>(ref_y) & 3) == 0;
-    const uint8_t* ref_uv = fs->ref_uv;
+    const uint8_t* ref_uv = fs.ref_uv;
     const int cw = g.coded_w / 2, ch = g.coded_h / 2;
     int mvx = 0, mvy = 0;
     int lsad = 0;
     int tsad = 0;
-    MbInfo mi;
-    mi.part = kPart16x16;
-    if (valid) {
-        mi = mbs[mbi];
+    uint32_t sw = 0, pw = 0;
+    int cpv[2] = {0, 0}, crs[2] = {0, 0};
+    {
         const int r = lane >> 2, c0 = (lane & 3) * 4;
         const Mv lv = px_mv(mi, c0, r);
         mvx = lv.x;
         mvy = lv.y;
-        const uint32_t sw = *reinterpret_cast<const uint32_t*>(src_y + (y0 + r) * g.pitch + x0 + c0);
-        if (fs->aq >= 3) {
+        sw = *reinterpret_cast<const uint32_t*>(src_y + (y0 + r) * g.pitch + x0 + c0);
+        if (fs.aq >= 3) {
             const int ix = mvx >> 2, iy = mvy >> 2;
             const int px = x0 + c0 + ix, py = y0 + r + iy;
             if (px >= 0 && px + 4 <= g.coded_w && py >= 0 && py < g.coded_h &&
                 ((px & 3) == 0 || (px & ~3) + 8 <= g.pitch)) {
-                const uint32_t* qa = reinterpret_cast<const uint32_t*>(fs->prev_src + (size_t)py * g.pitch + (px & ~3));
+                const uint32_t* qa = reinterpret_cast<const uint32_t*>(fs.prev_src + (size_t)py * g.pitch + (px & ~3));
                 const uint32_t sh = (uint32_t)(px & 3);
-                const uint32_t pw = sh ? __builtin_amdgcn_alignbyte(qa[1], qa[0], sh) : qa[0];
-                tsad = (int)__builtin_amdgcn_sad_u8(sw, pw, 0u);
+                const uint32_t qw = sh ? __builtin_amdgcn_alignbyte(qa[1], qa[0], sh) : qa[0];
+                tsad = (int)__builtin_amdgcn_sad_u8(sw, qw, 0u);
             } else {
                 for (int k = 0; k < 4; ++k)
                     tsad += abs((int)((sw >> (8 * k)) & 0xff) -
-                                ref_px(fs->prev_src, g.pitch, g.coded_w, g.coded_h, x0 + c0 + k + ix, y0 + r + iy));
-            }
-            *reinterpret_cast<uint32_t*>(fs->save_src + (y0 + r) * g.pitch + x0 + c0) = sw;
+                                ref_px(fs.prev_src, g.pitch, g.coded_w, g.coded_h, x0 + c0 + k + ix, y0 + r + iy));
+            }
+            *reinterpret_cast<uint32_t*>(fs.save_src + (y0 + r) * g.pitch + x0 + c0) = sw;
         }
         const int part = __builtin_amdgcn_readfirstlane((int)mi.part);
         const Mv va = blk_mv(mi, 0, 0), vb = blk_mv(mi, part == kPart8x16 ? 2 : 0, part == kPart16x8 ? 2 : 0);
         const int vax = __builtin_amdgcn_readfirstlane(va.x), vay = __builtin_amdgcn_readfirstlane(va.y);
         const int vbx = __builtin_amdgcn_readfirstlane(vb.x), vby = __builtin_amdgcn_readfirstlane(vb.y);
-        uint32_t pw = 0;
         if ((vax | vay | vbx | vby) & 3) {
             const int lpi = part == kPart16x8 ? (r >> 3) : (part == kPart8x16 ? (c0 >> 3) : 0);
-            mc_luma_wave(mcw[wave], ref_y, g.pitch, g.coded_w, g.coded_h, part == kPart16x16 ? 1 : 2, x0 * 4 + vax,
+            mc_luma_wave(L.mcw, ref_y, g.pitch, g.coded_w, g.coded_h, part == kPart16x16 ? 1 : 2, x0 * 4 + vax,
                          y0 * 4 + vay, x0 * 4 + vbx, y0 * 4 + vby, lane, lpi, &pw);
         } else {
             const int px = x0 + c0 + (mvx >> 2), py = min(max(y0 + r + (mvy >> 2), 0), g.coded_h - 1);
@@ -859,152 +886,208 @@
                     pw |= (uint32_t)ref_px(ref_y, g.pitch, g.coded_w, g.coded_h, px + k, py) << (8 * k);
             }
         }
-        for (int k = 0; k < 4; ++k) {
-            const int p = (int)((pw >> (8 * k)) & 0xff);
-            const int d = (int)((sw >> (8 * k)) & 0xff) - p;
-            pred[wave][r * 16 + c0 + k] = (uint8_t)p;
-            res[wave][r * 16 + c0 + k] = (int16_t)d;
-            lsad += d < 0 ? -d : d;
-        }
+        lsad = (int)__builtin_amdgcn_sad_u8(sw, pw, 0u);
         const int cr_ = lane >> 3, cc = lane & 7;
         const int xc = x0 / 2 + cc, yc = y0 / 2 + cr_;
         const Mv cv = px_mv(mi, 2 * cc, 2 * cr_);
         for (int comp = 0; comp < 2; ++comp) {
-            const int p = chroma_pred8(ref_uv, g.pitch, cw, ch, comp, xc * 8 + cv.x, yc * 8 + cv.y);
-            const int sv = src_uv[yc * g.pitch + 2 * xc + comp];
-            pred[wave][256 + comp * 64 + cr_ * 8 + cc] = (uint8_t)p;
-            res[wave][256 + comp * 64 + cr_ * 8 + cc] = (int16_t)(sv - p);
-        }
-    }
-    __syncthreads();
+            cpv[comp] = chroma_pred8(ref_uv, g.pitch, cw, ch, comp, xc * 8 + cv.x, yc * 8 + cv.y);
+            crs[comp] = (int)src_uv[yc * g.pitch + 2 * xc + comp] - cpv[comp];
+        }
+    }
+    const int aq = fs.aq;
+    const bool want_cost = fs.intra_in_p != 0;
     const uint32_t lsad_mb = (uint32_t)wave_sum(lsad);
     const int tcls = temporal_class((uint32_t)wave_sum(tsad), __ballot((mvx | mvy) != 0) == 0ull);
-    const int qp = mb_qp_for(fs->qp, lsad_mb, tcls, fs->aq);
-    const int qpc = chroma_qp(qp, fs->chroma_qp_offset);
-    int16_t* mc = coef + (size_t)(valid ? mbi : 0) * kCoefStride;
+    const int qp = mb_qp_for(fs.qp, lsad_mb, tcls, aq);
+    const int qpc = chroma_qp(qp, fs.chroma_qp_offset);
+    int16_t* mc = coef + (size_t)mbi * kCoefStride;
+
+    int bsum = lsad;
+    bsum += __builtin_amdgcn_mov_dpp(bsum, 0x124, 0xF, 0xF, false);
+    bsum += __builtin_amdgcn_mov_dpp(bsum, 0x128, 0xF, 0xF, false);
+    const bool luma_zero = __ballot(bsum > zero_sum_4x4(qp)) == 0ull;
+    int csum = abs(crs[0]) | (abs(crs[1]) << 16);
+    csum += __builtin_amdgcn_mov_dpp(csum, 0xB1, 0xF, 0xF, false);
+    csum += __builtin_amdgcn_mov_dpp(csum, 0x4E, 0xF, 0xF, false);
+    csum += __builtin_amdgcn_mov_dpp(csum, 0x128, 0xF, 0xF, false);
+    {
+        const auto r16 = __builtin_amdgcn_permlane16_swap((uint32_t)csum, (uint32_t)csum, false, false);
+        csum = (int)(r16[0] + r16[1]);
+    }
+    int psum = csum + __builtin_amdgcn_mov_dpp(csum, 0x124, 0xF, 0xF, false);
+    {
+        const auto r32 = __builtin_amdgcn_permlane32_swap((uint32_t)psum, (uint32_t)psum, false, false);
+        psum = (int)(r32[0] + r32[1]);
+    }
+    const int zac = zero_sum_4x4(qpc), zdc = zero_sum_chroma_dc(qpc);
+    const bool chroma_bound = __ballot((csum & 0xffff) > zac || (csum >> 16) > zac || (psum & 0xffff) > zdc ||
+                                       (psum >> 16) > zdc) == 0ull;
+    const bool luma_rows = !luma_zero || want_cost;
+    if (luma_rows) {
+        const int r = lane >> 2, c0 = (lane & 3) * 4;
+        *reinterpret_cast<uint32_t*>(&L.pred[r * 16 + c0]) = pw;
+        for (int k = 0; k < 4; ++k) L.res[r * 16 + c0 + k] = (int16_t)(byte_of(sw, k) - byte_of(pw, k));
+    }
+    if (!chroma_bound) {
+        for (int comp = 0; comp < 2; ++comp) {
+            L.pred[256 + comp * 64 + lane] = (uint8_t)cpv[comp];
+            L.res[256 + comp * 64 + lane] = (int16_t)crs[comp];
+        }
+    }
+    wave_sync_lds();
 
     const int lb = lane >> 2, rr = lane & 3, lbx = kBlkX[lb], lby = kBlkY[lb];
-    int x[4], y[4], z[4], rres[4];
+    int x[4] = {0, 0, 0, 0};
     const int ro = (lby * 4 + rr) * 16 + lbx * 4;
-#pragma unroll
-    for (int c = 0; c < 4; ++c) x[c] = res[wave][ro + c];
-    const int hs = quad_sum(had_row_abs(x, rr));
-    fdct_row(x, rr, y);
-    const int nzb = quad_sum(quant_row(y, rr, qp, false, 0, z));
-    {
-        int d[4];
-        dequant_row(z, rr, qp, d);
-        idct_row(d, rr, rres);
-    }
-    int d_pred = 0, d_coded = 0;
-#pragma unroll
-    for (int c = 0; c < 4; ++c) {
-        const int pv = pred[wave][ro + c];
-        const int e = pv + x[c] - clip255(pv + rres[c]);
-        d_pred += x[c] * x[c];
-        d_coded += e * e;
-    }
-    const uint32_t bits = rr == 0 ? block_bits_est(nzb) : 0u;
-    const bool drop = valid && drop_luma_for(fs->aq, lsad_mb, tcls, qp, wave_sum(d_pred), wave_sum(d_coded),
-                                             (uint32_t)wave_sum((int)bits));
-    const bool drop_c = drop_chroma_for(fs->aq, tcls, drop);
-    const int nz_l = drop ? 0 : nzb;
-    int sse_y = 0;
-    if (valid) {
-        uint32_t packed = 0;
-        const bool vis = x0 + lbx * 4 < g.width && (y0 + lby * 4 + rr) < g.height;
-#pragma unroll
-        for (int c = 0; c < 4; ++c) {
-            if (drop) z[c] = rres[c] = 0;
-            mc[kCoefLuma + lb * 16 + kZigzagInv4x4[rr * 4 + c]] = (int16_t)z[c];
-            const int pv = pred[wave][ro + c];
-            const int v = clip255(pv + rres[c]);
-            const int e = pv + x[c] - v;
-            sse_y += vis ? e * e : 0;
-            packed |= (uint32_t)v << (8 * c);
-        }
-        *reinterpret_cast<uint32_t*>(fs->rec_y + (y0 + lby * 4 + rr) * g.pitch + x0 + lbx * 4) = packed;
-        if (rr == 0) mbs[mbi].nz_luma[lby * 4 + lbx] = (uint8_t)nz_l;
-    }
-    const uint32_t satd_mb = (uint32_t)wave_sum(rr == 0 ? (hs + 1) >> 1 : 0);
+    uint32_t satd_mb = 0;
+    if (luma_rows) {
+#pragma unroll
+        for (int c = 0; c < 4; ++c) x[c] = L.res[ro + c];
+        if (want_cost) {
+            const int hs = quad_sum(had_row_abs(x, rr));
+            satd_mb = (uint32_t)wave_sum(rr == 0 ? (hs + 1) >> 1 : 0);
+        }
+    }
+    bool drop = false;
+    int nz_l = 0, sse_y = 0;
+    if (luma_zero) {
+        {
+            const int r = lane >> 2, c0 = (lane & 3) * 4;
+            const bool vis = x0 + c0 < g.width && (y0 + r) < g.height;
+            for (int k = 0; k < 4; ++k) {
+                const int e = byte_of(sw, k) - byte_of(pw, k);
+                sse_y += vis ? e * e : 0;
+            }
+            *reinterpret_cast<uint32_t*>(fs.rec_y + (y0 + r) * g.pitch + x0 + c0) = pw;
+            if (lane < 4) reinterpret_cast<uint32_t*>(mbs[mbi].nz_luma)[lane] = 0u;
+        }
+    } else {
+        int y[4], z[4], rres[4];
+        fdct_row(x, rr, y);
+        const int nzb = quad_sum(quant_row(y, rr, qp, false, 0, z));
+        {
+            int d[4];
+            dequant_row(z, rr, qp, d);
+            idct_row(d, rr, rres);
+        }
+        if (drop_luma_possible(aq, lsad_mb, tcls)) {
+            int d_pred = 0, d_coded = 0;
+#pragma unroll
+            for (int c = 0; c < 4; ++c) {
+                const int pv = L.pred[ro + c];
+                const int e = pv + x[c] - clip255(pv + rres[c]);
+                d_pred += x[c] * x[c];
+                d_coded += e * e;
+            }
+            const uint32_t bits = rr == 0 ? block_bits_est(nzb) : 0u;
+            drop = drop_luma_for(aq, lsad_mb, tcls, qp, wave_sum(d_pred), wave_sum(d_coded),
+                                          (uint32_t)wave_sum((int)bits));
+        }
+        nz_l = drop ? 0 : nzb;
+        {
+            uint32_t packed = 0;
+            const bool vis = x0 + lbx * 4 < g.width && (y0 + lby * 4 + rr) < g.height;
+#pragma unroll
+            for (int c = 0; c < 4; ++c) {
+                if (drop) z[c] = rres[c] = 0;
+                mc[kCoefLuma + lb * 16 + kZigzagInv4x4[rr * 4 + c]] = (int16_t)z[c];
+                const int pv = L.pred[ro + c];
+                const int v = clip255(pv + rres[c]);
+                const int e = pv + x[c] - v;
+                sse_y += vis ? e * e : 0;
+                packed |= (uint32_t)v << (8 * c);
+            }
+            *reinterpret_cast<uint32_t*>(fs.rec_y + (y0 + lby * 4 + rr) * g.pitch + x0 + lbx * 4) = packed;
+            if (rr == 0) mbs[mbi].nz_luma[lby * 4 + lbx] = (uint8_t)nz_l;
+        }
+    }
+    const bool drop_c = drop_chroma_for(aq, tcls, drop);
 
     const int cbk = lane >> 2, ccomp = (cbk >> 2) & 1, cblk = cbk & 3, cbx = cblk & 1, cby = cblk >> 1;
     const int co = 256 + ccomp * 64 + (cby * 4 + rr) * 8 + cbx * 4;
     const bool clane = lane < 32;
-    int cz[4], nzc = 0;
-    if (clane) {
-        int cx[4], cy[4];
-#pragma unroll
-        for (int c = 0; c < 4; ++c) cx[c] = drop_c ? 0 : res[wave][co + c];
-        fdct_row(cx, rr, cy);
-        if (rr == 0) cdc[wave][ccomp * 4 + cblk] = cy[0];
-        nzc = quant_row(cy, rr, qpc, false, 1, cz);
-    }
-    nzc = quad_sum(nzc);
-    if (valid && clane) {
-#pragma unroll
-        for (int c = 0; c < 4; ++c) {
-            const int i = rr * 4 + c;
-            if (i > 0) mc[kCoefChromaAc + (ccomp * 4 + cblk) * 16 + kZigzagInv4x4[i]] = (int16_t)cz[c];
-        }
-        if (rr == 0) (ccomp ? mbs[mbi].nz_cr : mbs[mbi].nz_cb)[cblk] = (uint8_t)nzc;
-    }
-    __syncthreads();
-    if (valid && (lane == 0 || lane == 16)) {
-        const int comp = lane >> 4;
-        int in[4], zd[4], dq[4];
-        for (int i = 0; i < 4; ++i) in[i] = cdc[wave][comp * 4 + i];
-        const int n = quant_dc_chroma(in, zd, qpc, false);
-        for (int i = 0; i < 4; ++i) mc[kCoefChromaDc + comp * 4 + i] = (int16_t)zd[i];
-        dequant_dc_chroma(zd, dq, qpc);
-        for (int i = 0; i < 4; ++i) cdc[wave][comp * 4 + i] = dq[i];
-        cdc_nz[wave][comp] = n;
-    }
-    __syncthreads();
-    int sse_c = 0;
-    if (clane) {
-        int d[4], cr[4];
-        dequant_row(cz, rr, qpc, d);
-        if (rr == 0) d[0] = cdc[wave][ccomp * 4 + cblk];
-        idct_row(d, rr, cr);
-        if (valid) {
-            const int xc = x0 / 2 + cbx * 4, yc = y0 / 2 + cby * 4 + rr;
+    int nzc = 0, dc_any = 0;
+    int sse_u = 0, sse_v = 0;
+    if (chroma_bound || drop_c) {
+        {
+            const int xc = x0 / 2 + (lane & 7), yc = y0 / 2 + (lane >> 3);
+            const bool vis = 2 * xc < g.width && 2 * yc < g.height;
+            sse_u = vis ? crs[0] * crs[0] : 0;
+            sse_v = vis ? crs[1] * crs[1] : 0;
+            uint8_t* o = fs.rec_uv + yc * g.pitch + 2 * xc;
+            if (((reinterpret_cast<uintptr_t>(fs.rec_uv) | (uintptr_t)g.pitch) & 1) == 0) {
+                *reinterpret_cast<uint16_t*>(o) = (uint16_t)(cpv[0] | (cpv[1] << 8));
+            } else {
+                o[0] = (uint8_t)cpv[0];
+                o[1] = (uint8_t)cpv[1];
+            }
+            if (lane < 2) reinterpret_cast<uint32_t*>(mbs[mbi].nz_cb)[lane] = 0u;
+        }
+    } else {
+        int cz[4];
+        if (clane) {
+            int cx[4], cy[4];
+#pragma unroll
+            for (int c = 0; c < 4; ++c) cx[c] = L.res[co + c];
+            fdct_row(cx, rr, cy);
+            if (rr == 0) L.cdc[ccomp * 4 + cblk] = cy[0];
+            nzc = quant_row(cy, rr, qpc, false, 1, cz);
+        }
+        nzc = quad_sum(nzc);
+        if (clane) {
 #pragma unroll
             for (int c = 0; c < 4; ++c) {
-                const int v = clip255(pred[wave][co + c] + cr[c]);
-                const int e = pred[wave][co + c] + res[wave][co + c] - v;
-                sse_c += (2 * (xc + c) < g.width && 2 * yc < g.height) ? e * e : 0;
-                fs->rec_uv[yc * g.pitch + 2 * (xc + c) + ccomp] = (uint8_t)v;
-            }
-        }
+                const int i = rr * 4 + c;
+                if (i > 0) mc[kCoefChromaAc + (ccomp * 4 + cblk) * 16 + kZigzagInv4x4[i]] = (int16_t)cz[c];
+            }
+            if (rr == 0) (ccomp ? mbs[mbi].nz_cr : mbs[mbi].nz_cb)[cblk] = (uint8_t)nzc;
+        }
+        wave_sync_lds();
+        if ((lane == 0 || lane == 16)) {
+            const int comp = lane >> 4;
+            int in[4], zd[4], dq[4];
+            for (int i = 0; i < 4; ++i) in[i] = L.cdc[comp * 4 + i];
+            const int n = quant_dc_chroma(in, zd, qpc, false);
+            for (int i = 0; i < 4; ++i) mc[kCoefChromaDc + comp * 4 + i] = (int16_t)zd[i];
+            dequant_dc_chroma(zd, dq, qpc);
+            for (int i = 0; i < 4; ++i) L.cdc[comp * 4 + i] = dq[i];
+            L.cdc_nz[comp] = n;
+        }
+        wave_sync_lds();
+        if (clane) {
+            int d[4], cr[4];
+            dequant_row(cz, rr, qpc, d);
+            if (rr == 0) d[0] = L.cdc[ccomp * 4 + cblk];
+            idct_row(d, rr, cr);
+            {
+                const int xc = x0 / 2 + cbx * 4, yc = y0 / 2 + cby * 4 + rr;
+                int sse_c = 0;
+#pragma unroll
+                for (int c = 0; c < 4; ++c) {
+                    const int v = clip255(L.pred[co + c] + cr[c]);
+                    const int e = L.pred[co + c] + L.res[co + c] - v;
+                    sse_c += (2 * (xc + c) < g.width && 2 * yc < g.height) ? e * e : 0;
+                    fs.rec_uv[yc * g.pitch + 2 * (xc + c) + ccomp] = (uint8_t)v;
+                }
+                (ccomp ? sse_v : sse_u) = sse_c;
+            }
+        }
+        dc_any = L.cdc_nz[0] | L.cdc_nz[1];
     }
     {
         const int sy = wave_sum(sse_y);
-        const int su = wave_sum(lane < 16 ? sse_c : 0);
-        const int sv = wave_sum((lane >= 16 && lane < 32) ? sse_c : 0);
-        if (valid && fs->intra_in_p && lane < 3)
-            mb_sse[lane * nmb + mbi] = (uint32_t)(lane == 0 ? sy : (lane == 1 ? su : sv));
-        __shared__ uint32_t part[4][4];
-        if (lane == 0) {
-            part[0][wave] = valid ? (uint32_t)sy : 0u;
-            part[1][wave] = valid ? (uint32_t)su : 0u;
-            part[2][wave] = valid ? (uint32_t)sv : 0u;
-            part[3][wave] = (valid && mb_unmasked(fs, mbx, mby)) ? (uint32_t)sy : 0u;
-        }
-        __syncthreads();
-        if (threadIdx.x < 4) {
-            const int c = threadIdx.x;
-            fs->sse_part[c * kSsePartStride + bid] =
-                (unsigned long long)part[c][0] + part[c][1] + part[c][2] + part[c][3];
-        }
-    }
-    const unsigned long long luma_mask = __ballot(valid && rr == 0 && nz_l > 0);
-    const unsigned long long chroma_mask = __ballot(valid && clane && rr == 0 && nzc > 0);
-    if (valid && lane == 0) {
+        const int su = wave_sum(sse_u);
+        const int sv = wave_sum(sse_v);
+        if (lane < 3) mb_sse[lane * nmb + mbi] = (uint32_t)(lane == 0 ? sy : (lane == 1 ? su : sv));
+    }
+    const unsigned long long luma_mask = __ballot(rr == 0 && nz_l > 0);
+    const unsigned long long chroma_mask = __ballot(clane && rr == 0 && nzc > 0);
+    if (lane == 0) {
         int cbp = 0;
         for (int b8 = 0; b8 < 4; ++b8)
             if ((luma_mask >> (16 * b8)) & 0x1111ull) cbp |= 1 << b8;
-        const int cc = (chroma_mask != 0) ? 2 : ((cdc_nz[wave][0] | cdc_nz[wave][1]) ? 1 : 0);
+        const int cc = (chroma_mask != 0) ? 2 : (dc_any ? 1 : 0);
         cbp |= cc << 4;
         MbInfo& m = mbs[mbi];
         m.type = kMbP16x16;
@@ -1012,8 +1095,39 @@
         m.qp = (uint8_t)qp;
         m.i16_mode = 0;
         m.chroma_mode = 0;
-        m.cost = inter_cost_mb(satd_mb, fs->qp, mi);
-    }
+        m.cost = want_cost ? inter_cost_mb(satd_mb, fs.qp, mi) : 0u;
+    }
+}
+
+__global__ __launch_bounds__(256) void k_inter_encode(Geometry g, const FrameState* __restrict__ fs,
+                                                       const uint8_t* __restrict__ src_y,
+                                                       const uint8_t* __restrict__ src_uv, MbInfo* __restrict__ mbs,
+                                                       int16_t* __restrict__ coef, uint32_t* __restrict__ mb_sse,
+                                                       int* __restrict__ wave_prog) {
+    __shared__ InterLds lds[4];
+    const int wave = threadIdx.x >> 6, lane = threadIdx.x & 63;
+    const int mbi = blockIdx.x * 4 + wave;
+    if (blockIdx.x == 0 && threadIdx.x == 0) wave_prog[1] = 0;
+    if (mbi >= g.mb_w * g.mb_h) return;
+    const MbInfo mi = mbs[mbi];
+    inter_code_mb(g, code_state(*fs), src_y, src_uv, mbs, coef, mb_sse, mbi, lane, mi, lds[wave]);
+}
+
+__global__ __launch_bounds__(kMeThreads) __attribute__((amdgpu_waves_per_eu(6))) void k_p_fused(Geometry g, StateArg sa, const uint8_t* __restrict__ src_y,
+                                                        const uint8_t* __restrict__ src_uv, MbInfo* __restrict__ mbs,
+                                                        int16_t* __restrict__ coef, uint32_t* __restrict__ mb_sse,
+                                                        int* __restrict__ wave_prog) {
+    __shared__ uint32_t win_lds[kWinWords];
+    static_assert(sizeof(InterLds) <= sizeof(uint32_t) * kWinWords, "the coder's LDS aliases the search window");
+    publish_state(sa);
+    if (blockIdx.x == 0 && threadIdx.x == 0) wave_prog[1] = 0;
+    const MeState st = sa.publish ? me_state(sa.v) : me_state(*sa.dst);
+    const CodeState cs = sa.publish ? code_state(sa.v) : code_state(*sa.dst);
+    const MbInfo mi = me_full_body(g, st, src_y, mbs, win_lds);
+    __syncthreads();
+    if (threadIdx.x >= 64) return;
+    inter_code_mb(g, cs, src_y, src_uv, mbs, coef, mb_sse, blockIdx.x, threadIdx.x, mi,
+                  *reinterpret_cast<InterLds*>(win_lds));
 }
 
 __constant__ uint8_t kRasterToBlk[16] = {0, 1, 4, 5, 2, 3, 6, 7, 8, 9, 12, 13, 10, 11, 14, 15};
@@ -1034,7 +1148,7 @@
     if (blockIdx.x == 0) {
         if (!fs->idr)
             for (int i = threadIdx.x; i < 4 * g.mb_h; i += 256)
-                fs->sse_part[(i / g.mb_h) * kSsePartStride + (g.mb_w * g.mb_h + 3) / 4 + i % g.mb_h] = 0;
+                fs->sse_part[(i / g.mb_h) * kSsePartStride + i % g.mb_h] = 0;
     }
     const int wave = threadIdx.x >> 6, lane = threadIdx.x & 63;
     const int mbi = blockIdx.x * 4 + wave;
@@ -1840,7 +1954,7 @@
     }
     __syncthreads();
     const int nmb = g.mb_w * g.mb_h;
-    const int slot = (nmb + 3) / 4 + mby;
+    const int slot = mby;
     if (lane == 0) {
         if (wave == 0) {
             m.cbp = (uint8_t)((m.cbp & 15) | (m.cbp_c << 4));
@@ -2040,17 +2154,26 @@
                                                             const uint32_t* __restrict__ slot_bits,
                                                             uint4* __restrict__ row_agg,
                                                             unsigned long long* __restrict__ row_sse,
-                                                            const MbInfo* __restrict__ mbs, uint32_t* __restrict__ db_cnt) {
+                                                            const MbInfo* __restrict__ mbs, uint32_t* __restrict__ db_cnt,
+                                                            const uint32_t* __restrict__ mb_sse) {
     __shared__ int wi[kScanThreads / 64];
     __shared__ uint32_t wu[kScanThreads / 64];
     const int t = threadIdx.x, r = blockIdx.x, base = r * g.mb_w;
     const bool idr = fs->idr != 0;
     const int nmb = g.mb_w * g.mb_h;
-    const int nparts = (idr || !fs->deblock_off) ? g.mb_h : (nmb + 3) / 4 + (fs->intra_in_p ? g.mb_h : 0);
-    const int p0 = (int)((long long)nparts * r / g.mb_h), p1 = (int)((long long)nparts * (r + 1) / g.mb_h);
+    const bool per_mb = !idr && fs->deblock_off;
     unsigned long long acc[4] = {0, 0, 0, 0};
-    for (int i = p0 + t; i < p1; i += kScanThreads)
-        for (int c = 0; c < 4; ++c) acc[c] += fs->sse_part[c * kSsePartStride + i];
+    if (per_mb) {
+        for (int j = t; j < g.mb_w; j += kScanThreads) {
+            const uint32_t sy = mb_sse[base + j];
+            acc[0] += sy;
+            acc[1] += mb_sse[nmb + base + j];
+            acc[2] += mb_sse[2 * nmb + base + j];
+            acc[3] += mb_unmasked(fs, j, r) ? sy : 0u;
+        }
+    }
+    if (t == 0 && (!per_mb || fs->intra_in_p))
+        for (int c = 0; c < 4; ++c) acc[c] += fs->sse_part[c * kSsePartStride + r];
     uint32_t b[kScanRowPer];
     int last = -1, first = 0x7fffffff;
     uint32_t ncoded = 0, over = 0;
@@ -2472,6 +2595,18 @@
                        b.coef, b.mb_sse, b.wave_prog);
 }
 
+void launch_p_fused(const Geometry& g, const DeviceBuffers& b, const uint8_t* src_y, const uint8_t* src_uv,
+                    hipStream_t stream, const FrameState* publish) {
+    const int nmb = g.mb_w * g.mb_h;
+    StateArg sa{};
+    if (publish) sa.v = *publish;
+    sa.dst = b.fs;
+    sa.publish = publish ? 1 : 0;
+    sa.t_start = b.out_hdr ? &b.out_hdr->t_start : nullptr;
+    hipLaunchKernelGGL(k_p_fused, dim3(nmb), dim3(kMeThreads), 0, stream, g, sa, src_y, src_uv, b.mb, b.coef, b.mb_sse,
+                       b.wave_prog);
+}
+
 static void launch_analyze(const Geometry& g, const DeviceBuffers& b, const uint8_t* src_y, const uint8_t* src_uv,
                            hipStream_t stream, const FrameState* publish, bool first) {
     const int nmb = g.mb_w * g.mb_h;
@@ -2525,7 +2660,7 @@
     if (g.mb_h > kScanMaxRows || g.mb_w > kScanThreads * kScanRowPer)
         throw std::runtime_error("launch_entropy: frame too large for the row scan");
     hipLaunchKernelGGL(k_scan_rows, dim3(g.mb_h), dim3(kScanThreads), 0, stream, g, b.fs, b.slot_bits, b.row_agg,
-                       b.row_sse, b.mb, b.db_cnt);
+                       b.row_sse, b.mb, b.db_cnt, b.mb_sse);
     hipLaunchKernelGGL(k_scan_out, dim3(g.mb_h), dim3(kScanThreads), 0, stream, g, b.fs, b.slot_bits, b.row_agg,
                        b.row_sse, b.coded_info, b.slice_info, b.out_bytes, b.out_hdr, b.quad_unit, b.db_cnt);
     hipLaunchKernelGGL(k_pack, dim3(256), dim3(256), 0, stream, g, b.fs, b.slot, b.coded_info, b.slice_info,
diff --git a/csrc/codec/h264_mb.h b/csrc/codec/h264_mb.h
--- a/csrc/codec/h264_mb.h
+++ b/csrc/codec/h264_mb.h
@@ -255,6 +255,9 @@
         return tclass == kTcChanging && d_pred - d_coded < (long long)lambda_sse(qp) * (long long)bits;
     return drop_residual(aq, lsad, qp, d_pred, d_coded, bits);
 }
+MXHD bool drop_luma_possible(int aq, uint32_t lsad, int tclass) {
+    return aq >= 3 ? tclass == kTcChanging : (aq >= 2 && lsad > 256u * 32);
+}
 MXHD bool drop_chroma_for(int aq, int tclass, bool luma_dropped) {
     return luma_dropped || (aq >= 3 && tclass == kTcChanging);
 }
@@ -299,6 +302,41 @@
     return nz;
 }
 
+constexpr int fdct_row_gain(int i) { return (i & 1) ? 2 : 1; }
+constexpr int zero_sum_4x4_calc(int qp) {
+    const int qm = qp % 6, qbits = 15 + qp / 6;
+    const int room = (1 << qbits) - 1 - (1 << qbits) / 6;
+    int t = room;
+    for (int i = 0; i < 16; ++i) {
+        const int b = room / (fdct_row_gain(i >> 2) * fdct_row_gain(i & 3) * kQuantMF[qm][kPosClass[i]]);
+        t = b < t ? b : t;
+    }
+    return t;
+}
+constexpr int zero_sum_chroma_dc_calc(int qpc) {
+    const int qm = qpc % 6, qbits = 16 + qpc / 6;
+    const int room = (1 << qbits) - 1 - 2 * ((1 << (qbits - 1)) / 6);
+    return room / kQuantMF[qm][0];
+}
+struct ZeroSumTab {
+    uint16_t blk[52], cdc[52];
+    constexpr ZeroSumTab() : blk{}, cdc{} {
+        for (int q = 0; q < 52; ++q) {
+            const int a = zero_sum_4x4_calc(q), b = zero_sum_chroma_dc_calc(q);
+            blk[q] = (uint16_t)(a > 0xffff ? 0xffff : a);
+            cdc[q] = (uint16_t)(b > 0xffff ? 0xffff : b);
+        }
+    }
+};
+MXHD int zero_sum_4x4(int qp) {
+    constexpr ZeroSumTab tab;
+    return tab.blk[qp < 0 ? 0 : (qp > 51 ? 51 : qp)];
+}
+MXHD int zero_sum_chroma_dc(int qpc) {
+    constexpr ZeroSumTab tab;
+    return tab.cdc[qpc < 0 ? 0 : (qpc > 51 ? 51 : qpc)];
+}
+
 MXHD uint32_t me_cost(uint32_t sad, int lambda, int mvx, int mvy) {
     return sad + (uint32_t)(lambda * (mvd_bits(mvx) + mvd_bits(mvy)));
 }
```

Result: faster. 12130, median of 6 (+11.9%).
